# JeremyWesthead/deacon-server

Measured on AMD Instinct MI355X. Metric: Mbp/s filtered (k=31,w=15 vs panhuman-1-sized index), decisions bit-exact vs CPU, higher is better.
Workload: dtype u64

## Files before the change

### deacon-server_amd/_native.py

```python
import ctypes as C
import os
import re
import subprocess

_PKG = os.path.dirname(os.path.abspath(__file__))
LIB_PATH = os.environ.get("DCN_LIB_PATH") or os.path.join(_PKG, "lib", "libdeacon_hip.so")
HEADER_PATH = os.path.join(os.path.dirname(_PKG), "include", "deacon_hip.h")

DCN_OK = 0
DCN_ERR_ARG = -1
DCN_ERR_HIP = -2
DCN_ERR_NOMEM = -3
DCN_ERR_IO = -4
DCN_ERR_FORMAT = -5
DCN_ERR_CAPACITY = -6
DCN_ERR_INTERNAL = -7
N_STATS = 6
N_STAGES = 5
STAGE_NAMES = ("pack", "plan", "scan", "distinct", "finish")
STAT_NAMES = ("total_seqs", "filtered_seqs", "total_bp", "output_bp", "filtered_bp", "output_seq_counter")


class DeaconHipError(RuntimeError):
    def __init__(self, code, message):
# ... 21 lines not shown
        ("prefix_length", C.c_uint64),
    ]


class TrackParams(C.Structure):
    _fields_ = [
        ("bin_bases", C.c_uint32),
        ("member_mask", C.c_uint32),
        ("depth_cap", C.c_uint32),
        ("reserved", C.c_uint32),
        ("prefix_length", C.c_uint64),
    ]


class TrackBin(C.Structure):
    _fields_ = [
        ("n_positions", C.c_uint32),
        ("n_keys", C.c_uint32),
        ("n_observed", C.c_uint32),
        ("max_depth", C.c_uint32),
        ("sum_depth", C.c_uint64),
    ]


class PlaceParams(C.Structure):
    _fields_ = [
        ("band_bases", C.c_uint32),
        ("min_votes", C.c_uint32),
        ("prefix_length", C.c_uint64),
        ("reserved", C.c_uint32 * 2),
    ]


class Placement(C.Structure):
    _fields_ = [
        ("record", C.c_uint32),
        ("reverse", C.c_uint32),
        ("votes", C.c_uint32),
        ("n_anchors", C.c_uint32),
        ("n_positions", C.c_uint32),
        ("read_start", C.c_uint32),
        ("read_end", C.c_uint32),
        ("reserved", C.c_uint32),
        ("ref_start", C.c_uint64),
        ("ref_end", C.c_uint64),
    ]


class PlaceSplitParams(C.Structure):
    _fields_ = [
        ("band_bases", C.c_uint32),
        ("min_votes", C.c_uint32),
        ("prefix_length", C.c_uint64),
        ("max_placements", C.c_uint32),
        ("reserved", C.c_uint32 * 3),
    ]


class SplitPlacement(C.Structure):
    _fields_ = Placement._fields_ + [
        ("rank", C.c_uint32),
        ("n_placed", C.c_uint32),
        ("rival_votes", C.c_uint32),
        ("mapq", C.c_uint32),
    ]


PLACE_SPLIT_MAX = 8


class PlacePairParams(C.Structure):
    _fields_ = [
        ("band_bases", C.c_uint32),
        ("min_votes", C.c_uint32),
        ("prefix_length", C.c_uint64),
        ("max_placements", C.c_uint32),
        ("max_insert", C.c_uint32),
        ("hist_bin_bases", C.c_uint32),
        ("reserved", C.c_uint32 * 3),
    ]


class PairPlacement(C.Structure):
    _fields_ = SplitPlacement._fields_ + [
        ("flags", C.c_uint32),
        ("pair_votes", C.c_uint32),
        ("tlen", C.c_int64),
    ]


PAIR_HIST_BINS = 256


def build(force=False, jobs=6):
    csrc = os.path.join(_PKG, "csrc")
    cmd = ["make", "-C", csrc, f"-j{jobs}"]
    if force:
        cmd.append("-B")
    subprocess.check_call(cmd, stdout=subprocess.DEVNULL)
    return LIB_PATH


def declared_symbols():
    text = open(HEADER_PATH).read()
    text = re.sub(r"/\*.*?\*/", "", text, flags=re.S)
    return sorted(set(re.findall(r"\b(dcn_[a-z0-9_]+)\s*\(", text)))


_u8p, _u32p, _u64p = C.POINTER(C.c_uint8), C.POINTER(C.c_uint32), C.POINTER(C.c_uint64)
_vp = C.c_void_p

_SIGNATURES = {
    "dcn_abi_version": (C.c_int, [_u32p, _u32p]),
    "dcn_version": (C.c_char_p, []),
    "dcn_last_error": (C.c_char_p, []),
    "dcn_device_count": (C.c_int, [C.POINTER(C.c_int)]),
    "dcn_set_minimizer_variant": (C.c_int, [C.c_uint32, C.c_uint32, C.c_uint32]),
    "dcn_get_minimizer_variant": (C.c_int, [_u32p, _u32p, _u32p]),
    "dcn_index_from_keys": (C.c_int, [_vp, C.c_uint64, C.c_uint8, C.c_uint8, C.c_int, C.POINTER(_vp)]),
    "dcn_index_from_file": (C.c_int, [C.c_char_p, C.c_int, C.POINTER(_vp)]),
    "dcn_index_build": (C.c_int, [_vp, _vp, C.c_uint32, C.c_uint8, C.c_uint8, C.c_float, C.c_uint64, C.c_int,
                                  C.POINTER(_vp)]),
    "dcn_index_keys": (C.c_int, [_vp, _vp, C.c_uint64, _u64p]),
    "dcn_index_union": (C.c_int, [C.POINTER(_vp), C.c_uint32, C.POINTER(_vp)]),
    "dcn_index_diff": (C.c_int, [_vp, _vp, C.POINTER(_vp)]),
    "dcn_index_intersect": (C.c_int, [C.POINTER(_vp), C.c_uint32, C.POINTER(_vp)]),
    "dcn_index_write_file": (C.c_int, [_vp, C.c_char_p]),
    "dcn_index_header": (C.c_int, [_vp, _u8p, _u8p, _u64p]),
    "dcn_index_contains": (C.c_int, [_vp, _vp, C.c_uint64, _vp]),
    "dcn_index_contains_device": (C.c_int, [_vp, _vp, C.c_uint64, _vp, _vp]),
    "dcn_index_probe_ceiling": (C.c_int, [_vp, _vp, C.c_uint64, C.c_uint32, C.POINTER(C.c_double)]),
    "dcn_index_destroy": (None, [_vp]),
    "dcn_ctx_create": (C.c_int, [_vp, C.c_uint64, C.c_uint32, C.POINTER(_vp)]),
    "dcn_ctx_destroy": (None, [_vp]),
    "dcn_filter_batch": (C.c_int, [_vp, _vp, _vp, _vp, C.c_uint32, C.POINTER(Params), _vp, _vp, _vp]),
    "dcn_filter_batch_submit": (C.c_int, [_vp, _vp, _vp, _vp, C.c_uint32, C.POINTER(Params), _vp, _vp, _vp, _u64p]),
    "dcn_filter_batch_wait": (C.c_int, [_vp, C.c_uint64]),
    "dcn_filter_batch_packed": (C.c_int, [_vp, _vp, _vp, _vp, _vp, C.c_uint32, C.POINTER(Params), _vp, _vp, _vp]),
    "dcn_filter_batch_packed_submit": (C.c_int, [_vp, _vp, _vp, _vp, _vp, C.c_uint32, C.POINTER(Params), _vp, _vp, _vp,
                                                 _u64p]),
    "dcn_pack_ascii": (C.c_int, [_vp, C.c_uint64, _vp, _vp, _u32p]),
    "dcn_stats_allreduce": (C.c_int, [C.POINTER(_vp), C.c_int, _u64p]),
    "dcn_comm_available": (C.c_int, []),
    "dcn_comm_unique_id": (C.c_int, [_vp]),
    "dcn_comm_create": (C.c_int, [_vp, C.c_int, C.c_int, C.c_int, C.POINTER(_vp)]),
    "dcn_stats_allreduce_rccl": (C.c_int, [_vp, C.POINTER(_vp), C.c_int, _u64p]),
    "dcn_comm_destroy": (None, [_vp]),
    "dcn_index_device": (C.c_int, [_vp, C.POINTER(C.c_int)]),
    "dcn_index_memory": (C.c_int, [_vp, C.POINTER(C.c_uint64)]),
    "dcn_index_clone": (C.c_int, [_vp, C.c_int, C.POINTER(_vp)]),
    "dcn_filter_batch_device": (C.c_int, [_vp, _vp, _vp, _vp, C.c_uint32, C.c_uint64, C.c_uint32,
                                          C.POINTER(Params), _vp, _vp, _vp]),
    "dcn_ctx_synchronize": (C.c_int, [_vp]),
    "dcn_ctx_reserve_records": (C.c_int, [_vp, C.c_uint64]),
    "dcn_ctx_stream": (_vp, [_vp]),
    "dcn_host_alloc": (C.c_int, [C.c_uint64, C.POINTER(_vp)]),
    "dcn_host_free": (None, [_vp]),
    "dcn_minimizer_hashes_batch": (C.c_int, [_vp, _vp, _vp, C.c_uint32, C.c_uint64, _vp, _vp, _vp, C.c_uint64]),
    "dcn_should_keep_hashes": (C.c_int, [_vp, _vp, _vp, C.c_uint32, C.POINTER(Params), _vp, _vp, _vp]),
    "dcn_ctx_stats": (C.c_int, [_vp, _u64p]),
    "dcn_ctx_reset_stats": (C.c_int, [_vp]),
    "dcn_ctx_set_profiling": (C.c_int, [_vp, C.c_int]),
    "dcn_ctx_profile": (C.c_int, [_vp, C.POINTER(C.c_double), _u64p]),
    "dcn_index_set_create": (C.c_int, [C.POINTER(_vp), C.c_uint32, C.POINTER(_vp)]),
    "dcn_index_set_destroy": (None, [_vp]),
    "dcn_index_set_info": (C.c_int, [_vp, _u32p, _u8p, _u8p, _u64p, _u64p]),
    "dcn_classify_batch": (C.c_int, [_vp, _vp, _vp, _vp, _vp, C.c_uint32, C.POINTER(Params), _vp, _vp, _vp]),
    "dcn_classify_batch_device": (C.c_int, [_vp, _vp, _vp, _vp, _vp, C.c_uint32, C.c_uint64, C.c_uint32,
                                            C.POINTER(Params), _vp, _vp, _vp]),
    "dcn_index_set_coverage_enable": (C.c_int, [_vp, C.c_int]),
    "dcn_index_set_coverage_reset": (C.c_int, [_vp]),
    "dcn_index_set_coverage": (C.c_int, [_vp, _vp, _vp]),
    "dcn_index_set_coverage_keys": (C.c_int, [_vp, C.c_uint32, _vp, C.c_uint64, _u64p]),
    "dcn_index_set_depth_enable": (C.c_int, [_vp, C.c_int]),
    "dcn_index_set_depth_reset": (C.c_int, [_vp]),
    "dcn_index_set_depth_stats": (C.c_int, [_vp, _vp, _vp, _vp]),
    "dcn_index_set_depth_hist": (C.c_int, [_vp, C.c_uint32, C.c_uint32, _vp]),
    "dcn_index_set_depth_keys": (C.c_int, [_vp, C.c_uint32, _vp, _vp, C.c_uint64, _u64p]),
    "dcn_index_set_select": (C.c_int, [_vp, C.c_uint32, C.c_uint32, C.c_uint32, C.c_uint32, C.c_uint32, _u64p,
                                       C.POINTER(_vp)]),
    "dcn_index_set_overlap": (C.c_int, [_vp, _vp, _vp, _vp]),
    "dcn_index_builder_create": (C.c_int, [C.c_uint8, C.c_uint8, C.c_float, C.c_uint64, C.c_int, C.POINTER(_vp)]),
    "dcn_index_builder_add": (C.c_int, [_vp, _vp, _vp, C.c_uint32]),
    "dcn_index_builder_info": (C.c_int, [_vp, _u64p, _u64p, _u64p, _u64p]),
    "dcn_index_builder_hist": (C.c_int, [_vp, C.c_uint32, _vp]),
    "dcn_index_builder_counts": (C.c_int, [_vp, _vp, _vp, C.c_uint64, _u64p]),
    "dcn_index_builder_finish": (C.c_int, [_vp, C.c_uint32, C.c_uint32, _u64p, C.POINTER(_vp)]),
    "dcn_index_builder_destroy": (None, [_vp]),
    "dcn_locate_batch": (C.c_int, [_vp, _vp, _vp, _vp, C.c_uint32, _vp, _vp, _vp, C.c_uint64]),
    "dcn_depth_track_batch": (C.c_int, [_vp, _vp, _vp, _vp, C.c_uint32, _vp, _vp, _vp, C.c_uint64]),
    "dcn_anchor_map_create": (C.c_int, [_vp, C.POINTER(_vp)]),
    "dcn_anchor_map_add": (C.c_int, [_vp, _vp, _vp, _vp, C.c_uint32, _u32p]),
    "dcn_anchor_map_info": (C.c_int, [_vp, _u32p, _u64p, _u64p, _u64p]),
    "dcn_anchor_map_anchors": (C.c_int, [_vp, _vp, _vp, _vp, C.c_uint64, _u64p]),
    "dcn_place_batch": (C.c_int, [_vp, _vp, _vp, _vp, C.c_uint32, _vp, _vp]),
    "dcn_place_split_batch": (C.c_int, [_vp, _vp, _vp, _vp, C.c_uint32, _vp, _vp, _vp, C.c_uint64, _vp]),
    "dcn_place_pair_batch": (C.c_int, [_vp, _vp, _vp, _vp, C.c_uint32, _vp, _vp, _vp]),
}

_lib = None
ABI = (1, 11)


def lib():
    global _lib
    if _lib is not None:
        return _lib
    if not os.path.exists(LIB_PATH):
        raise ImportError(
            f"{LIB_PATH} is missing: build it with __graft_entry__.build() "
            "(make -C deacon-server_amd/csrc). There is no CPU fallback.")
    L = C.CDLL(LIB_PATH)
    for name, (res, args) in _SIGNATURES.items():
        f = getattr(L, name)
        f.restype = res
        f.argtypes = args
    major, minor = C.c_uint32(), C.c_uint32()
    if L.dcn_abi_version(C.byref(major), C.byref(minor)) != 0 or (major.value, minor.value >= ABI[1]) != (ABI[0], True):
        raise ImportError(f"{LIB_PATH} has ABI {major.value}.{minor.value}; these bindings were written against {ABI[0]}.{ABI[1]} "
                          "(include/deacon_hip.h: DCN_ABI_MAJOR / DCN_ABI_MINOR)")
    _lib = L
    return L


def check(rc):
    if rc != DCN_OK:
        msg = lib().dcn_last_error()
        raise DeaconHipError(rc, msg.decode("utf-8", "replace") if msg else "")
    return rc
```

### deacon-server_amd/csrc/ctx.hip

```cpp
#include "dcn_ctx.h"
#include "dcn_host_pool.h"

#include <atomic>
#include <cstdlib>
#include <cstring>
#include <mutex>
#include <new>

using dcn_host::HostPool;

uint32_t dcn_cu_count() {
    int dev = 0, cus = 256;
    if (hipGetDevice(&dev) == hipSuccess) (void)hipDeviceGetAttribute(&cus, hipDeviceAttributeMultiprocessorCount, dev);
    return (uint32_t)std::max(cus, 1);
}

namespace dcn_impl {

int alloc_records(dcn_ctx *c, uint64_t n_records) {
    n_records = (n_records + 63) / 64 * 64;
    if (n_records > (1ull << 29)) return dcn_fail(DCN_ERR_CAPACITY, "more than 2^29 hit records in global sets per batch: use smaller batches");
    if (c->d_set_slots) hipFree(c->d_set_slots);
    c->d_set_slots = nullptr;
    c->rec_capacity = 0;
// ... 5 lines not shown
void free_slot_buffers(dcn_slot &sl) {
    if (sl.owns_buffers) {
        void *dev[] = {sl.d_ascii, sl.d_packed, sl.d_invmask, sl.d_offsets, sl.d_unit_id, sl.d_keep, sl.d_hits, sl.d_total};
        for (void *p : dev)
            if (p) hipFree(p);
    }
    if (sl.d_report) hipFree(sl.d_report);
    if (sl.d_off32) hipFree(sl.d_off32);
    if (sl.d_mask_pairs) hipFree(sl.d_mask_pairs);
    void *host[] = {sl.h_keep, sl.h_hits, sl.h_total, sl.h_report, sl.h_off32, sl.h_mask_pairs};
    for (void *p : host)
        if (p) hipHostFree(p);
    if (sl.done) hipEventDestroy(sl.done);
    for (hipEvent_t e : sl.ev_h2d) hipEventDestroy(e);
    for (hipEvent_t e : sl.ev_comp) hipEventDestroy(e);
    sl = dcn_slot();
}

static void free_ctx(dcn_ctx *c) {
    if (!c) return;
    hipSetDevice(c->device);
    if (c->stream) hipStreamSynchronize(c->stream);
    if (c->copy_stream) hipStreamSynchronize(c->copy_stream);
    if (c->d2h_stream) hipStreamSynchronize(c->d2h_stream);
    if (c->pack_stream) {
        hipStreamSynchronize(c->pack_stream);
        hipStreamDestroy(c->pack_stream);
    }
    for (int i = 0; i < 2; ++i) {
        if (c->pack_done[i]) hipEventDestroy(c->pack_done[i]);
        if (c->buf_free[i]) hipEventDestroy(c->buf_free[i]);
    }
    if (c->plan_done) hipEventDestroy(c->plan_done);
    if (c->d_packed_b) hipFree(c->d_packed_b);
    if (c->d_invmask_b) hipFree(c->d_invmask_b);
    if (c->d_pack_status) hipFree(c->d_pack_status);
    for (auto &sl : c->slots) free_slot_buffers(sl);
    void *dev[] = {c->d_ascii, c->d_offsets, c->d_unit_id, c->d_packed, c->d_invmask,
                   c->d_read_tiles, c->d_read_tile_first, c->d_unit_first_read, c->d_unit_tile_first, c->d_unit_tile_count, c->d_tiles,
                   c->d_keep, c->d_unit_state, c->d_hits, c->d_total, c->d_unit_scratch, c->d_caps,
                   c->d_set_off, c->d_tile_hits, c->d_pending, c->d_big, c->d_rec_hash, c->d_set_slots, c->d_status, c->d_report, c->d_dump_hash,
                   c->d_dump_pos, c->d_dump_count, c->d_dump_valid, c->d_tile_read_pos,
                   c->d_cls_big, c->d_cls_n_big, c->d_cls_match, c->d_cls_hits, c->d_cls_total,
                   c->d_loc_bits, c->d_loc_labels, c->d_loc_counts, c->d_loc_big, c->d_loc_n_big, c->d_loc_block_sums,
                   c->d_loc_seg_offsets, c->d_loc_segs, c->d_trk_bin_offsets, c->d_trk_piece_offsets, c->d_trk_bins,
                   c->d_plc_words, c->d_plc_abits, c->d_plc_big, c->d_plc_n_big, c->d_plc_out,
                   c->d_pls_rbits, c->d_pls_n_rounds, c->d_pls_read_counts, c->d_pls_counts, c->d_pls_block_sums,
                   c->d_pls_offsets, c->d_pls_rounds, c->d_pls_out, c->d_ppr_out, c->d_ppr_hist};
    for (void *p : dev)
        if (p && !((char *)p >= c->d_slab && (char *)p < c->d_slab + c->slab_bytes)) hipFree(p);
    if (c->d_slab) hipFree(c->d_slab);
    for (int i = 0; i < dcn_ctx::N_STAGE; ++i) {
        if (c->h_stage[i]) hipHostFree(c->h_stage[i]);
        if (c->stage_free[i]) hipEventDestroy(c->stage_free[i]);
    }
    for (int i = 0; i < dcn_ctx::N_EV; ++i) {
        if (c->ev_h2d[i]) hipEventDestroy(c->ev_h2d[i]);
        if (c->ev_comp[i]) hipEventDestroy(c->ev_comp[i]);
    }
    if (c->h_report) hipHostFree(c->h_report);
    for (int i = 0; i < dcn_ctx::PROF_RING; ++i)
        for (int j = 0; j <= DCN_N_STAGES; ++j)
            if (c->prof_ev[i][j]) hipEventDestroy(c->prof_ev[i][j]);
    if (c->copy_done) hipEventDestroy(c->copy_done);
    if (c->stream) hipStreamDestroy(c->stream);
    if (c->copy_stream) hipStreamDestroy(c->copy_stream);
    if (c->d2h_stream) hipStreamDestroy(c->d2h_stream);
    delete c;
}

static int prof_harvest(dcn_ctx *c, int only_slot = -1) {
    for (int i = 0; i < dcn_ctx::PROF_RING; ++i) {
        if (!c->prof_used[i] || (only_slot >= 0 && i != only_slot)) continue;
        const int first = c->prof_scan_only[i] ? DCN_STAGE_SCAN : 0, last = c->prof_scan_only[i] ? DCN_STAGE_SCAN : DCN_N_STAGES - 1;
        DCN_HIP(hipEventSynchronize(c->prof_ev[i][last + 1]));
        for (int j = first; j <= last; ++j) {
            float ms = 0.f;
            DCN_HIP(hipEventElapsedTime(&ms, c->prof_ev[i][j], c->prof_ev[i][j + 1]));
            c->prof_ms[j] += ms;
        }
        c->prof_batches++;
        c->prof_used[i] = false;
    }
    return DCN_OK;
}

int prof_begin(dcn_ctx *c, int *slot) {
    *slot = -1;
    if (!c->profiling) return DCN_OK;
    int i = c->prof_next;
    c->prof_next = (i + 1) % dcn_ctx::PROF_RING;
    if (c->prof_used[i]) DCN_TRY(prof_harvest(c, i));
    for (int j = 0; j <= DCN_N_STAGES; ++j)
        if (!c->prof_ev[i][j]) DCN_HIP(hipEventCreate(&c->prof_ev[i][j]));
    c->prof_scan_only[i] = c->profiling == 2;
    if (c->profiling == 1) DCN_HIP(hipEventRecord(c->prof_ev[i][0], c->stream));
    *slot = i;
    return DCN_OK;
}

int check_params(const dcn_params *p) {
    if (!p) return dcn_fail(DCN_ERR_ARG, "params is NULL");
    if (p->reserved != 0) return dcn_fail(DCN_ERR_ARG, "params.reserved must be 0");
    if (p->deplete > 1) return dcn_fail(DCN_ERR_ARG, "params.deplete must be 0 or 1");
    return DCN_OK;
}

static bool ensure_pack_ahead(dcn_ctx *c) {
    if (c->pack_ahead_state != 0) return c->pack_ahead_state > 0;
    c->pack_ahead_state = -1;
    if (!getenv("DCN_PACK_AHEAD") || getenv("DCN_NO_PACK_AHEAD")) return false;
    int prio_low = 0, prio_high = 0;
    (void)hipDeviceGetStreamPriorityRange(&prio_low, &prio_high);
    bool ok = hipStreamCreateWithPriority(&c->pack_stream, hipStreamNonBlocking, prio_high) == hipSuccess;
    ok = ok && hipEventCreateWithFlags(&c->plan_done, hipEventDisableTiming) == hipSuccess;
    for (int i = 0; ok && i < 2; ++i)
        ok = hipEventCreateWithFlags(&c->pack_done[i], hipEventDisableTiming) == hipSuccess &&
             hipEventCreateWithFlags(&c->buf_free[i], hipEventDisableTiming) == hipSuccess;
    ok = ok && hipMalloc((void **)&c->d_packed_b, packed_words(c->max_bases) * sizeof(uint32_t)) == hipSuccess &&
         hipMalloc((void **)&c->d_invmask_b, mask_words(c->max_bases) * sizeof(uint32_t)) == hipSuccess &&
         hipMalloc((void **)&c->d_pack_status, 2 * sizeof(dcn_status)) == hipSuccess;
    if (ok) {
        ok = hipMemset(c->d_packed_b, 0, packed_words(c->max_bases) * sizeof(uint32_t)) == hipSuccess &&
             hipMemset(c->d_invmask_b, 0, mask_words(c->max_bases) * sizeof(uint32_t)) == hipSuccess &&
             hipDeviceSynchronize() == hipSuccess;
    }
    if (!ok) {
        (void)hipGetLastError();
        if (c->d_packed_b) hipFree(c->d_packed_b);
        if (c->d_invmask_b) hipFree(c->d_invmask_b);
        if (c->d_pack_status) hipFree(c->d_pack_status);
        c->d_packed_b = c->d_invmask_b = nullptr;
        c->d_pack_status = nullptr;
        return false;
    }
    c->pack_ahead_state = 1;
    return true;
}

static dcn_scan_args scan_args(const dcn_ctx *c, const dcn_index *index, uint32_t *packed, uint32_t *invmask, uint64_t stream_bases);

int enqueue_batch(dcn_ctx *c, const BatchView &v, const dcn_params *params, bool pack_ahead) {
    hipStream_t st = c->stream;
    const dcn_index *idx = c->index;
    if (c->scratch_dirty) DCN_HIP(hipMemsetAsync(c->d_unit_scratch, 0, (uint64_t)c->max_reads * 4 * sizeof(uint32_t), st));
    c->scratch_dirty = true;
    DCN_HIP(hipMemsetAsync(c->d_status, 0, sizeof(dcn_status), st));

    int prof_slot = -1;
    DCN_TRY(prof_begin(c, &prof_slot));
    uint32_t *packed = v.d_packed + DCN_FRONT_PAD, *invmask = v.d_invmask + DCN_FRONT_PAD;
    int ahead_buf = -1;
    const uint32_t *newline_flag = nullptr;
    if (v.d_ascii && pack_ahead && c->profiling != 1 && ensure_pack_ahead(c)) {
        ahead_buf = c->pack_buf;
        c->pack_buf ^= 1;
        if (ahead_buf == 1) {
            packed = c->d_packed_b + DCN_FRONT_PAD;
            invmask = c->d_invmask_b + DCN_FRONT_PAD;
        }
        dcn_status *ps = c->d_pack_status + ahead_buf;
        DCN_HIP(hipStreamWaitEvent(c->pack_stream, c->buf_free[ahead_buf], 0));
        if (!getenv("DCN_PACK_AHEAD_EARLY")) DCN_HIP(hipStreamWaitEvent(c->pack_stream, c->plan_done, 0));
        DCN_HIP(hipMemsetAsync(ps, 0, sizeof(dcn_status), c->pack_stream));
        DCN_TRY(dcn_launch_pack_beside(v.d_ascii, v.b0, v.b1, packed, invmask, ps, c->pack_stream));
        DCN_HIP(hipEventRecord(c->pack_done[ahead_buf], c->pack_stream));
        DCN_HIP(hipStreamWaitEvent(st, c->pack_done[ahead_buf], 0));
        newline_flag = &ps->any_newline;
    } else if (v.d_ascii) {
        DCN_TRY(dcn_launch_pack(v.d_ascii, v.b0, v.b1, packed, invmask, c->d_status, st));
    }
    DCN_PROF_MARK(DCN_STAGE_PACK);

    const uint32_t n_reads = v.n_reads, n_units = v.n_units;
    dcn_plan_args pa = plan_args(c, idx, v.d_ascii, v.d_offsets, v.d_unit_id, n_reads, n_units, params->prefix_length);
    pa.unit_base = v.unit_base;
    pa.unit_state = c->d_unit_state;
    pa.unit_scratch = c->d_unit_scratch;
    pa.scratch_stride = c->max_reads;
    pa.newline_flag = newline_flag;
    pa.stream_bases = v.stream_bases;
    pa.check_offsets = 1;
    pa.max_tiles = c->max_tiles;
    DCN_TRY(dcn_launch_plan(pa, st));
    if (pack_ahead && c->pack_ahead_state == 1) DCN_HIP(hipEventRecord(c->plan_done, st));
    DCN_PROF_MARK(DCN_STAGE_PLAN);

    const UnitScratch us = unit_scratch(c);
    dcn_scan_args sa = scan_args(c, idx, packed, invmask, v.stream_bases);
    sa.unit_tile_first = c->d_unit_tile_first;
    sa.unit_tile_count = c->d_unit_tile_count;
    sa.abs_threshold = params->abs_threshold;
    sa.rel_threshold = params->rel_threshold;
    sa.deplete = params->deplete;
    sa.early_out_max_items = 0;
    static const bool no_early_out = getenv("DCN_NO_EARLY_OUT") != nullptr, no_early_out_pairs = getenv("DCN_NO_EARLY_OUT_PAIRS") != nullptr;
    if (!v.d_hits && !v.d_total && params->abs_threshold >= 1 && params->abs_threshold <= 4 && !no_early_out) {
        uint32_t lo = 0, hi = 65535;
        while (lo < hi) {
            uint32_t mid = (lo + hi + 1) / 2;
            if (dcn_required_hits(params->abs_threshold, params->rel_threshold, mid) == params->abs_threshold) lo = mid;
            else hi = mid - 1;
        }
        sa.early_out_max_items = lo;
        sa.early_out_pairs = no_early_out_pairs ? 0u : 1u;
    }
    sa.keep = v.d_keep;
    sa.hits = v.d_hits;
    sa.total = v.d_total;
    sa.unit_state = c->d_unit_state;
    sa.g_total = us.g_total;
    sa.g_hitcnt = us.g_hitcnt;
    sa.g_zero = us.g_zero;
    sa.rec_hash = c->d_rec_hash;
    sa.rec_shift = c->rec_shift;
    sa.tile_windows = c->tile_windows;
    sa.tile_hits = c->d_tile_hits;
    sa.pending = c->d_pending;
    sa.status = c->d_status;
    DCN_TRY(dcn_launch_scan(sa, tile_bound(c, n_reads, v.b1 - v.b0), false, st));
    DCN_PROF_MARK(DCN_STAGE_SCAN);

    const bool decisions_only = !v.d_hits && !v.d_total && !getenv("DCN_NO_EARLY_OUT");
    const dcn_distinct_args da = distinct_args(c, n_units, params, c->d_rec_hash, c->rec_shift, decisions_only ? us.g_total : nullptr);
    DCN_TRY(dcn_launch_distinct(da, st));
    DCN_PROF_MARK(DCN_STAGE_DISTINCT);

    const dcn_finish_args fa = finish_args(c, n_units, params, v.d_unit_id ? c->d_unit_first_read : nullptr, v.d_offsets, v.d_keep,
                                           v.d_hits, v.d_total, v.d_report);
    DCN_TRY(dcn_launch_finish(fa, st));
    c->scratch_dirty = false;
    if (pack_ahead && c->pack_ahead_state == 1) DCN_HIP(hipEventRecord(c->buf_free[ahead_buf >= 0 ? ahead_buf : 0], st));
    DCN_PROF_MARK(DCN_STAGE_FINISH);
    if (prof_slot >= 0) c->prof_used[prof_slot] = true;
    return DCN_OK;
}

int grow_run_slots(dcn_ctx *c) {
    if (c->rec_shift == 0) return DCN_OK;
    const bool in_slab = c->d_rec_hash && (char *)c->d_rec_hash >= c->d_slab && (char *)c->d_rec_hash < c->d_slab + c->slab_bytes;
    if (c->d_rec_hash && !in_slab) hipFree(c->d_rec_hash);
    c->d_rec_hash = nullptr;
    const uint32_t old_shift = c->rec_shift;
    c->rec_shift = 0;
    int rc = dev_alloc(&c->d_rec_hash, c->max_bases + 128, "rec_hash (one slot per window)");
    if (rc != DCN_OK) {
        c->rec_shift = old_shift;
        int rc2 = dev_alloc(&c->d_rec_hash, (c->max_bases >> old_shift) + 256, "rec_hash");
        return rc2 != DCN_OK ? rc2 : rc;
    }
    static std::atomic<bool> said{false};
    if (!said.exchange(true) && getenv("DCN_QUIET") == nullptr)
        std::fprintf(stderr, "deacon-hip: a unit's hits outgrew its run of the record array; this context now keeps one slot per window "
                             "(%.2f GB instead of %.2f GB of device memory)\n", (c->max_bases + 128) * 8e-9,
                     ((c->max_bases >> old_shift) + 256) * 8e-9);
    return DCN_OK;
}

int overflow_error(const dcn_ctx *c, uint64_t need) {
    return dcn_fail(DCN_ERR_CAPACITY, "hit-record scratch overflow: need " + std::to_string(need) +
                                          " records, have " + std::to_string(c->rec_capacity) +
                                          " (dcn_ctx_reserve_records)");
}

int sync_and_check(dcn_ctx *c, uint64_t *needed_records) {
    DCN_HIP(hipStreamSynchronize(c->stream));
    if (needed_records) *needed_records = 0;
    if (c->profiling) DCN_TRY(prof_harvest(c));
    if (!c->batch_pending) return DCN_OK;
    c->batch_pending = false;
    DCN_HIP(hipMemcpy(c->h_report, c->d_report, sizeof(dcn_batch_report), hipMemcpyDeviceToHost));
    if (c->h_report->bounds) {
        DCN_HIP(hipMemsetAsync(c->d_report, 0, offsetof(dcn_batch_report, stats), c->stream));
        return dcn_fail(DCN_ERR_INTERNAL, "scan kernel: index out of range in phase B (DCN_DEBUG_BOUNDS build)");
    }
    if (c->h_report->bad_offsets) {
        DCN_HIP(hipMemsetAsync(c->d_report, 0, offsetof(dcn_batch_report, stats), c->stream));
        return dcn_fail(DCN_ERR_ARG, "d_offsets of a batch since the last synchronize were not non-decreasing within [0, n_bases] when the "
                                     "device read them (were they written, and ordered before the context's stream, when "
                                     "dcn_filter_batch_device was called?): the outputs and counters of those batches are undefined");
    }
    if (c->h_report->overflow) {
        const uint64_t need = c->h_report->need;
        const bool runs = (c->h_report->overflow & 2u) != 0, sets = (c->h_report->overflow & 1u) != 0;
        DCN_HIP(hipMemsetAsync(c->d_report, 0, offsetof(dcn_batch_report, stats), c->stream));
        if (runs) DCN_TRY(grow_run_slots(c));
        if (needed_records) *needed_records = sets ? need : 0;
        if (!sets)
            return dcn_fail(DCN_ERR_CAPACITY, "a unit had more hits in one wave than its run of the record array holds; the context "
                                              "now keeps one slot per window: enqueue the batches since the last synchronize again");
        return overflow_error(c, need);
    }
    return DCN_OK;
}

bool is_pinned_host(const void *p) {
    if (!p) return false;
    hipPointerAttribute_t attr;
    if (hipPointerGetAttributes(&attr, p) != hipSuccess) {
        (void)hipGetLastError();
        return false;
    }
    return attr.type == hipMemoryTypeHost;
}

template <typename Fill>
static int staged_h2d_fill(dcn_ctx *c, void *d_dst, uint64_t bytes, uint64_t piece_align, Fill fill) {
    uint8_t *dst = (uint8_t *)d_dst;
    const uint64_t piece = c->stage_bytes / piece_align * piece_align;
    for (uint64_t off = 0; off < bytes; off += piece) {
        const int which = c->stage_next;
        c->stage_next = (which + 1) % dcn_ctx::N_STAGE;
        const uint64_t m = std::min<uint64_t>(piece, bytes - off);
        DCN_HIP(hipEventSynchronize(c->stage_free[which]));
        fill(c->h_stage[which], off, m);
        DCN_HIP(hipMemcpyAsync(dst + off, c->h_stage[which], m, hipMemcpyHostToDevice, c->copy_stream));
        DCN_HIP(hipEventRecord(c->stage_free[which], c->copy_stream));
    }
    return DCN_OK;
}

int staged_h2d(dcn_ctx *c, void *d_dst, const void *h_src, uint64_t bytes, int pinned) {
    if (bytes == 0) return DCN_OK;
    if (pinned < 0) pinned = is_pinned_host(h_src) ? 1 : 0;
    if (pinned) {
        DCN_HIP(hipMemcpyAsync(d_dst, h_src, bytes, hipMemcpyHostToDevice, c->copy_stream));
        return DCN_OK;
    }
    const uint8_t *src = (const uint8_t *)h_src;
    return staged_h2d_fill(c, d_dst, bytes, 64, [&](uint8_t *stage, uint64_t first, uint64_t n) {
        HostPool::get().copy(stage, src + first, n);
    });
}


int slots_busy(const dcn_ctx *c) {
    int n = 0;
    for (const auto &sl : c->slots) n += sl.busy ? 1 : 0;
    return n;
}

static std::mutex g_ctx_devices_mu;
static int g_ctx_per_device[64] = {0};
static void note_ctx_device(int device, int delta) {
    int n_devices = 0;
    {
        std::lock_guard<std::mutex> g(g_ctx_devices_mu);
        if (device >= 0 && device < 64) g_ctx_per_device[device] += delta;
        for (int d = 0; d < 64; ++d) n_devices += g_ctx_per_device[d] > 0;
    }
    if (delta > 0) HostPool::get().ensure_devices(n_devices);
}

int check_idle(const dcn_ctx *c) {
    if (slots_busy(c) || c->batch_pending) return dcn_fail(DCN_ERR_ARG, "batches are in flight on this context: wait for them first");
    return DCN_OK;
}

int check_ctx_matches(const dcn_ctx *c, const dcn_index *other, const char *noun) {
    const dcn_index *ix = c->index;
    const std::string n = noun;
    if (ix->k != other->k || ix->w != other->w)
        return dcn_fail(DCN_ERR_ARG, "the context's index (k=" + std::to_string((int)ix->k) + ", w=" + std::to_string((int)ix->w) +
                                         ") and " + n + " (k=" + std::to_string((int)other->k) + ", w=" + std::to_string((int)other->w) +
                                         ") differ");
    if (ix->device != other->device) return dcn_fail(DCN_ERR_ARG, "the context and " + n + " live on different devices");
    if (ix->variant != other->variant)
        return dcn_fail(DCN_ERR_ARG, "the context's index and " + n + " were created under different minimizer rules");
    return check_idle(c);
}

int check_device_batch(const dcn_ctx *c, uint32_t n_reads, uint64_t n_bases, uint32_t n_units, const uint32_t *d_unit_id) {
    if (n_reads > c->max_reads) return dcn_fail(DCN_ERR_CAPACITY, "n_reads exceeds the context's max_batch_reads");
    if (n_bases > c->max_bases) return dcn_fail(DCN_ERR_CAPACITY, "n_bases exceeds the context's max_batch_bases");
    if (n_units == 0 || n_units > n_reads || (!d_unit_id && n_units != n_reads))
        return dcn_fail(DCN_ERR_ARG, "n_units inconsistent with n_reads / d_unit_id");
    return DCN_OK;
}

int check_offsets_walk(const uint64_t *offsets, uint32_t n, const char *noun, const char *too_long) {
    if (offsets[0] != 0) return dcn_fail(DCN_ERR_ARG, std::string(noun) + "[0] must be 0");
    for (uint32_t r = 0; r < n; ++r) {
        if (offsets[r + 1] < offsets[r]) return dcn_fail(DCN_ERR_ARG, std::string(noun) + " must be non-decreasing");
        if (offsets[r + 1] - offsets[r] > 0xFFFFFFF0ull) return dcn_fail(DCN_ERR_ARG, too_long);
    }
    return DCN_OK;
}

int validate_host_batch(const dcn_ctx *c, const uint64_t *offsets, uint32_t n_reads) {
    if (n_reads > c->max_reads) return dcn_fail(DCN_ERR_CAPACITY, "n_reads exceeds the context's max_batch_reads");
    DCN_TRY(check_idle(c));
    DCN_TRY(check_offsets_walk(offsets, n_reads, "offsets", "read longer than 2^32 bases"));
    if (offsets[n_reads] > c->max_bases) return dcn_fail(DCN_ERR_CAPACITY, "batch exceeds the context's max_batch_bases");
    return DCN_OK;
}

int ensure_dump_buffers(dcn_ctx *c) {
    if (c->d_dump_hash) return DCN_OK;
    DCN_TRY(dev_alloc(&c->d_dump_hash, c->max_bases + 2, "dump_hash"));
    DCN_TRY(dev_alloc(&c->d_dump_pos, c->max_bases + 2, "dump_pos"));
    DCN_TRY(dev_alloc(&c->d_dump_valid, c->max_bases + 2, "dump_valid"));
    DCN_TRY(dev_alloc(&c->d_dump_count, c->max_tiles, "dump_count"));
    return DCN_OK;
}

int ensure_position_bitmap(dcn_ctx *c) {
    if (c->d_loc_bits) return DCN_OK;
    return dev_alloc(&c->d_loc_bits, (c->max_bases + 31) / 32 + 1, "position bitmap");
}

int ensure_position_words(dcn_ctx *c) {
    if (c->d_loc_labels) return DCN_OK;
    return dev_alloc(&c->d_loc_labels, c->max_bases + 2, "position words");
}

UnitScratch unit_scratch(const dcn_ctx *c) {
    uint32_t *const s = c->d_unit_scratch;
    const uint64_t n = c->max_reads;
    return {s, s + n, s + 2 * n, s + 3 * n};
}

int stage_done(dcn_ctx *c) {
    DCN_HIP(hipEventRecord(c->copy_done, c->copy_stream));
    DCN_HIP(hipStreamWaitEvent(c->stream, c->copy_done, 0));
// ... 64 lines not shown
    v.n_tiles = &c->d_status->n_tiles;
    v.hash = c->d_dump_hash;
    v.valid = c->d_dump_valid;
    v.pos = c->d_dump_pos;
    v.count = c->d_dump_count;
    v.max_tiles = max_tiles;
    v.n_bases = n_bases;
    return v;
}

int dump_front_end(dcn_ctx *c, const dcn_index *index, const uint8_t *d_ascii, const uint64_t *d_offsets,
                   const uint32_t *d_unit_id, uint32_t n_reads, uint32_t n_units, uint64_t n_bases, uint64_t prefix_length,
                   bool plan_checks_offsets, int *prof_slot_out, dcn_dump_view *view) {
    hipStream_t st = c->stream;
    int prof_slot = -1;
    DCN_TRY(prof_begin(c, &prof_slot));
    *prof_slot_out = prof_slot;
    DCN_TRY(dcn_launch_pack(d_ascii, 0, n_bases, c->d_packed + DCN_FRONT_PAD, c->d_invmask + DCN_FRONT_PAD, c->d_status, st));
    DCN_PROF_MARK(DCN_STAGE_PACK);
    dcn_plan_args pa = plan_args(c, index, d_ascii, d_offsets, d_unit_id, n_reads, n_units, prefix_length);
    pa.read_tiles = c->d_read_tiles;
    pa.read_tile_first = c->d_read_tile_first;
    if (plan_checks_offsets) {
        pa.stream_bases = n_bases;
        pa.check_offsets = 1;
        pa.max_tiles = c->max_tiles;
    }
    DCN_TRY(dcn_launch_plan(pa, st));
    DCN_PROF_MARK(DCN_STAGE_PLAN);
    dcn_scan_args sa = dump_scan_args(c, index, n_bases);
    sa.dump_abs = 1;
    const uint32_t max_tiles = tile_bound(c, n_reads, n_bases);
    DCN_TRY(dcn_launch_scan(sa, max_tiles, true, st));
    DCN_PROF_MARK(DCN_STAGE_SCAN);
    *view = dump_view(c, max_tiles, n_bases);
    return DCN_OK;
}

int record_run_end(dcn_ctx *c, int prof_slot) {
    if (prof_slot >= 0) c->prof_used[prof_slot] = true;
    if (c->pack_ahead_state == 1) {
        DCN_HIP(hipEventRecord(c->plan_done, c->stream));
        for (int i = 0; i < 2; ++i) DCN_HIP(hipEventRecord(c->buf_free[i], c->stream));
    }
    return DCN_OK;
}

int finish_run(dcn_ctx *c, int prof_slot) {
    DCN_TRY(record_run_end(c, prof_slot));
    return sync_and_check(c, nullptr);
}

dcn_distinct_args distinct_args(const dcn_ctx *c, uint32_t n_units, const dcn_params *params, const uint64_t *rec_hash,
                                uint32_t rec_shift, uint32_t *g_total_or_null) {
    const UnitScratch us = unit_scratch(c);
    dcn_distinct_args da = {};
    da.tiles = c->d_tiles;
    da.n_tiles = &c->d_status->n_tiles;
    da.unit_tile_first = c->d_unit_tile_first;
    da.unit_tile_count = c->d_unit_tile_count;
    da.unit_state = c->d_unit_state;
    da.tile_hits = c->d_tile_hits;
    da.pending = c->d_pending;
    da.rec_hash = rec_hash;
    da.rec_shift = rec_shift;
    da.g_hitcnt = us.g_hitcnt;
    da.g_distinct = us.g_distinct;
    da.set_off = c->d_set_off;
    da.set_slots = c->d_set_slots;
    da.set_capacity = 4 * c->rec_capacity + 64;
    da.n_units = n_units;
    da.status = c->d_status;
    da.caps = c->d_caps;
    da.big = c->d_big;
    da.g_total = g_total_or_null;
    da.abs_threshold = params->abs_threshold;
    da.rel_threshold = params->rel_threshold;
    return da;
}

dcn_finish_args finish_args(const dcn_ctx *c, uint32_t n_units, const dcn_params *params, const uint32_t *unit_first_read,
                            const uint64_t *offsets, uint8_t *keep, uint32_t *hits, uint32_t *total, dcn_batch_report *report) {
    const UnitScratch us = unit_scratch(c);
    dcn_finish_args fa = {};
    fa.n_units = n_units;
    fa.unit_first_read = unit_first_read;
    fa.offsets = offsets;
    fa.unit_state = c->d_unit_state;
    fa.g_total = us.g_total;
    fa.g_hitcnt = us.g_hitcnt;
    fa.g_distinct = us.g_distinct;
    fa.g_zero = us.g_zero;
    fa.abs_threshold = params->abs_threshold;
    fa.rel_threshold = params->rel_threshold;
    fa.deplete = params->deplete;
    fa.keep = keep;
    fa.hits = hits;
    fa.total = total;
    fa.report = report;
    fa.status = c->d_status;
    return fa;
}

}

using namespace dcn_impl;

extern "C" int dcn_ctx_create(const dcn_index *index, uint64_t max_batch_bases, uint32_t max_batch_reads,
                              dcn_ctx **out) {
    if (!out) return dcn_fail(DCN_ERR_ARG, "out is NULL");
    *out = nullptr;
    if (!index) return dcn_fail(DCN_ERR_ARG, "index is NULL");
    if (max_batch_bases == 0 || max_batch_reads == 0) return dcn_fail(DCN_ERR_ARG, "batch limits must be > 0");
    if (max_batch_reads > 0xFFFFFF00u) return dcn_fail(DCN_ERR_ARG, "max_batch_reads too large");
    dcn_ctx *c = new (std::nothrow) dcn_ctx();
    if (!c) return dcn_fail(DCN_ERR_NOMEM, "host allocation failed");
    c->index = index;
    c->device = index->device;
    c->max_bases = max_batch_bases;
    c->max_reads = max_batch_reads;
    if (const char *tw = getenv("DCN_TILE_WINDOWS")) {
        long v = strtol(tw, nullptr, 10);
        if (v >= 16 && v <= (long)DCN_MAX_TILE_WINDOWS) c->tile_windows = (uint32_t)v;
    }
    uint64_t mt = (uint64_t)max_batch_reads + max_batch_bases / c->tile_windows + 1;
    if (mt > 0xFFFFFF00ull) {
        delete c;
        return dcn_fail(DCN_ERR_ARG, "batch limits imply more than 2^32 tiles");
    }
    c->max_tiles = (uint32_t)mt;
    c->chunk_bases = 64ull << 20;
    if (const char *cb = getenv("DCN_CHUNK_BASES")) {
        long long v = atoll(cb);
        if (v >= 1024) c->chunk_bases = (uint64_t)v;
    }
    int rc = DCN_OK;
    auto fail = [&](int code) {
        free_ctx(c);
        return code;
    };
    if (hipSetDevice(c->device) != hipSuccess) return fail(dcn_fail(DCN_ERR_HIP, "hipSetDevice failed"));
    bool ok = hipStreamCreateWithFlags(&c->stream, hipStreamNonBlocking) == hipSuccess &&
              hipStreamCreateWithFlags(&c->copy_stream, hipStreamNonBlocking) == hipSuccess &&
              hipStreamCreateWithFlags(&c->d2h_stream, hipStreamNonBlocking) == hipSuccess &&
              hipEventCreateWithFlags(&c->copy_done, hipEventDisableTiming) == hipSuccess;
    for (int i = 0; ok && i < dcn_ctx::N_STAGE; ++i)
        ok = hipEventCreateWithFlags(&c->stage_free[i], hipEventDisableTiming) == hipSuccess;
    for (int i = 0; ok && i < dcn_ctx::N_EV; ++i)
        ok = hipEventCreateWithFlags(&c->ev_h2d[i], hipEventDisableTiming) == hipSuccess &&
             hipEventCreateWithFlags(&c->ev_comp[i], hipEventDisableTiming) == hipSuccess;
    if (!ok) return fail(dcn_fail(DCN_ERR_HIP, "stream/event creation failed"));
    c->rec_shift = 2;
    if (index->w <= 7) c->rec_shift = 0;
    if (const char *rs = getenv("DCN_REC_SHIFT")) c->rec_shift = (uint32_t)std::min(3, std::max(0, atoi(rs)));
    uint64_t MR = max_batch_reads;
    const bool slab = getenv("DCN_CTX_SLAB") != nullptr;
    uint64_t slab_off = 0;
    for (int pass = slab ? 0 : 1; pass < 2; ++pass) {
        if (slab && pass == 1) {
            c->slab_bytes = slab_off;
            if (hipMalloc((void **)&c->d_slab, c->slab_bytes) != hipSuccess) {
                c->d_slab = nullptr;
                c->slab_bytes = 0;
                return fail(dcn_fail(DCN_ERR_NOMEM, "hipMalloc of the context slab failed"));
            }
            slab_off = 0;
        }
#define A(ptr, count, what)                                                                                   \
    if (slab) {                                                                                               \
        if (pass == 1) c->ptr = reinterpret_cast<decltype(c->ptr)>(c->d_slab + slab_off);                     \
        slab_off += (std::max<uint64_t>((count), 1) * sizeof(*c->ptr) + (2u << 20) - 1) / (2u << 20) * (2u << 20); \
    } else if ((rc = dev_alloc(&c->ptr, (count), what)) != DCN_OK)                                            \
        return fail(rc)
    A(d_ascii, max_batch_bases + 64, "ascii");
    A(d_offsets, MR + 1, "offsets");
    A(d_unit_id, MR, "unit_id");
    A(d_packed, packed_words(max_batch_bases), "packed");
    A(d_invmask, mask_words(max_batch_bases), "invmask");
    A(d_read_tiles, MR, "read_tiles");
    A(d_read_tile_first, MR + 1, "read_tile_first");
    A(d_unit_first_read, MR + 1, "unit_first_read");
    A(d_unit_tile_first, MR + 1, "unit_tile_first");
    A(d_unit_tile_count, MR + 1, "unit_tile_count");
    A(d_tiles, mt, "tiles");
    A(d_keep, MR, "keep");
    A(d_unit_state, MR, "unit_state");
    A(d_hits, MR, "hits");
    A(d_total, MR, "total");
    A(d_unit_scratch, MR * 4, "unit_scratch");
    A(d_caps, MR, "caps");
    A(d_set_off, MR + 1, "set_off");
    A(d_tile_hits, mt, "tile_hits");
    A(d_pending, MR, "pending");
    A(d_big, MR + mt / 64 + 1, "big");
    A(d_rec_hash, (max_batch_bases >> c->rec_shift) + 256, "rec_hash");
    A(d_status, 1, "status");
    A(d_report, 1, "report");
#undef A
    }
    uint64_t recs = std::min<uint64_t>(std::max<uint64_t>(max_batch_bases / 16, 1u << 16), 1ull << 29);
    if (const char *rc_env = getenv("DCN_RECORD_CAPACITY")) recs = std::min<uint64_t>(std::max<uint64_t>(strtoull(rc_env, nullptr, 10), 64), 1ull << 29);
    if ((rc = alloc_records(c, recs)) != DCN_OK) return fail(rc);
    c->stage_bytes = std::min<uint64_t>(std::max<uint64_t>(max_batch_bases + 64, 4096), 32ull << 20);
    if (const char *sb = getenv("DCN_STAGE_BYTES"))
        c->stage_bytes = std::min<uint64_t>(std::max<uint64_t>(strtoull(sb, nullptr, 10), 4096), 32ull << 20);
    for (int i = 0; i < dcn_ctx::N_STAGE; ++i)
        if (hipHostMalloc((void **)&c->h_stage[i], c->stage_bytes, hipHostMallocDefault) != hipSuccess)
            return fail(dcn_fail(DCN_ERR_NOMEM, "pinned staging allocation failed"));
    if (hipHostMalloc((void **)&c->h_report, sizeof(dcn_batch_report), hipHostMallocDefault) != hipSuccess)
        return fail(dcn_fail(DCN_ERR_NOMEM, "pinned status allocation failed"));
    if (hipMemset(c->d_packed, 0, packed_words(max_batch_bases) * sizeof(uint32_t)) != hipSuccess ||
        hipMemset(c->d_invmask, 0, mask_words(max_batch_bases) * sizeof(uint32_t)) != hipSuccess ||
        hipMemset(c->d_status, 0, sizeof(dcn_status)) != hipSuccess ||
        hipMemset(c->d_unit_scratch, 0, (uint64_t)max_batch_reads * 4 * sizeof(uint32_t)) != hipSuccess ||
        hipMemset(c->d_report, 0, sizeof(dcn_batch_report)) != hipSuccess ||
        hipDeviceSynchronize() != hipSuccess)
        return fail(dcn_fail(DCN_ERR_HIP, "hipMemset failed"));
    note_ctx_device(c->device, +1);
    *out = c;
    return DCN_OK;
}

extern "C" void dcn_ctx_destroy(dcn_ctx *ctx) {
    if (ctx) note_ctx_device(ctx->device, -1);
    free_ctx(ctx);
}

extern "C" void *dcn_ctx_stream(dcn_ctx *ctx) { return ctx ? (void *)ctx->stream : nullptr; }

extern "C" int dcn_ctx_reserve_records(dcn_ctx *ctx, uint64_t n_records) {
    if (!ctx) return dcn_fail(DCN_ERR_ARG, "ctx is NULL");
    if (slots_busy(ctx)) return dcn_fail(DCN_ERR_ARG, "host batches are in flight: wait for them first");
    DCN_HIP(hipSetDevice(ctx->device));
    DCN_HIP(hipStreamSynchronize(ctx->stream));
    if (n_records <= ctx->rec_capacity) return DCN_OK;
    return alloc_records(ctx, n_records);
}

extern "C" int dcn_ctx_synchronize(dcn_ctx *ctx) {
    if (!ctx) return dcn_fail(DCN_ERR_ARG, "ctx is NULL");
    DCN_HIP(hipSetDevice(ctx->device));
    return sync_and_check(ctx, nullptr);
}

extern "C" int dcn_filter_batch_device(dcn_ctx *ctx, const uint8_t *d_bases, const uint64_t *d_offsets,
                                       const uint32_t *d_unit_id, uint32_t n_reads, uint64_t n_bases,
                                       uint32_t n_units, const dcn_params *params, uint8_t *d_keep, uint32_t *d_hits,
                                       uint32_t *d_total) {
    if (!ctx) return dcn_fail(DCN_ERR_ARG, "ctx is NULL");
    DCN_TRY(check_params(params));
    if (n_reads == 0) return DCN_OK;
    if (!d_bases || !d_offsets || !d_keep) return dcn_fail(DCN_ERR_ARG, "d_bases/d_offsets/d_keep is NULL");
    DCN_TRY(check_device_batch(ctx, n_reads, n_bases, n_units, d_unit_id));
    if (ctx->slots[0].busy) return dcn_fail(DCN_ERR_ARG, "a host batch is in flight on this context: wait for it first");
    DCN_HIP(hipSetDevice(ctx->device));
    BatchView v;
    v.d_ascii = d_bases;
    v.d_packed = ctx->d_packed;
    v.d_invmask = ctx->d_invmask;
    v.d_offsets = d_offsets;
    v.d_unit_id = d_unit_id;
    v.n_reads = n_reads;
    v.n_units = n_units;
    v.b0 = 0;
    v.b1 = n_bases;
    v.stream_bases = n_bases;
    v.d_keep = d_keep;
    v.d_hits = d_hits;
    v.d_total = d_total;
    v.d_report = ctx->d_report;
    DCN_TRY(enqueue_batch(ctx, v, params, true));
    ctx->batch_pending = true;
    return DCN_OK;
}

extern "C" int dcn_ctx_set_profiling(dcn_ctx *ctx, int enable) {
    if (!ctx) return dcn_fail(DCN_ERR_ARG, "ctx is NULL");
    DCN_HIP(hipSetDevice(ctx->device));
    DCN_HIP(hipStreamSynchronize(ctx->stream));
    for (int i = 0; i < dcn_ctx::PROF_RING; ++i) ctx->prof_used[i] = false;
    for (int j = 0; j < DCN_N_STAGES; ++j) ctx->prof_ms[j] = 0.0;
    ctx->prof_batches = 0;
    ctx->profiling = enable == 2 ? 2 : (enable != 0 ? 1 : 0);
    return DCN_OK;
}

extern "C" int dcn_ctx_profile(dcn_ctx *ctx, double stage_ms[DCN_N_STAGES], uint64_t *n_batches) {
    if (!ctx || !stage_ms) return dcn_fail(DCN_ERR_ARG, "ctx/stage_ms is NULL");
    if (ctx->profiling) {
        DCN_HIP(hipSetDevice(ctx->device));
        DCN_TRY(prof_harvest(ctx));
    }
    for (int j = 0; j < DCN_N_STAGES; ++j) stage_ms[j] = ctx->prof_ms[j];
    if (n_batches) *n_batches = ctx->prof_batches;
    return DCN_OK;
}

extern "C" int dcn_ctx_stats(dcn_ctx *ctx, uint64_t counters[DCN_N_STATS]) {
    if (!ctx || !counters) return dcn_fail(DCN_ERR_ARG, "ctx/counters is NULL");
    DCN_HIP(hipSetDevice(ctx->device));
    DCN_HIP(hipStreamSynchronize(ctx->stream));
    DCN_HIP(hipMemcpy(ctx->h_report, ctx->d_report, sizeof(dcn_batch_report), hipMemcpyDeviceToHost));
    for (int i = 0; i < DCN_N_STATS; ++i) counters[i] = ctx->h_report->stats[i] + ctx->host_stats[i];
    return DCN_OK;
}

extern "C" int dcn_ctx_reset_stats(dcn_ctx *ctx) {
    if (!ctx) return dcn_fail(DCN_ERR_ARG, "ctx is NULL");
    DCN_HIP(hipSetDevice(ctx->device));
    DCN_HIP(hipStreamSynchronize(ctx->stream));
    DCN_HIP(hipMemsetAsync(ctx->d_report->stats, 0, sizeof(unsigned long long) * DCN_N_STATS, ctx->stream));
    DCN_HIP(hipStreamSynchronize(ctx->stream));
    for (int i = 0; i < DCN_N_STATS; ++i) ctx->host_stats[i] = 0;
    return DCN_OK;
}

extern "C" int dcn_stats_allreduce(dcn_ctx *const *ctxs, int n_ctx, uint64_t counters[DCN_N_STATS]) {
    if (!counters || (n_ctx > 0 && !ctxs) || n_ctx < 0) return dcn_fail(DCN_ERR_ARG, "ctxs/counters is NULL");
    for (int i = 0; i < DCN_N_STATS; ++i) counters[i] = 0;
    for (int j = 0; j < n_ctx; ++j) {
        uint64_t one[DCN_N_STATS];
        DCN_TRY(dcn_ctx_stats(ctxs[j], one));
        for (int i = 0; i < DCN_N_STATS; ++i) counters[i] += one[i];
    }
    return DCN_OK;
}
```

### deacon-server_amd/csrc/dcn_ctx.h

```cpp
#pragma once

#include "dcn_dump_sweep.h"
#include "dcn_internal.h"
#include "dcn_plan.h"

#include <algorithm>
#include <functional>
#include <vector>

struct dcn_split_round;

struct dcn_mask_range {
    uint64_t g0 = 0, g1 = 0, pairs_off = 0;
    uint32_t n = 0;
};

struct dcn_chunk {
    uint32_t r0 = 0, r1 = 0, u0 = 0, u1 = 0;
    uint64_t b0 = 0, b1 = 0;
    uint64_t max_len = 0;
    std::vector<dcn_mask_range> mask_ranges;
};

struct dcn_slot {
    bool allocated = false, busy = false, owns_buffers = false;
    uint64_t ticket = 0;
    uint8_t *d_ascii = nullptr;
    uint32_t *d_packed = nullptr, *d_invmask = nullptr;
    uint64_t *d_offsets = nullptr;
    uint32_t *d_off32 = nullptr, *h_off32 = nullptr;
    bool off32 = false;
    bool lean = false;
    uint2 *d_mask_pairs = nullptr, *h_mask_pairs = nullptr;
    uint64_t mask_pairs_cap = 0, mask_pairs_used = 0;
    uint32_t *d_unit_id = nullptr;
    uint8_t *d_keep = nullptr;
    uint32_t *d_hits = nullptr, *d_total = nullptr;
    dcn_batch_report *d_report = nullptr;
    uint8_t *h_keep = nullptr;
    uint32_t *h_hits = nullptr, *h_total = nullptr;
    dcn_batch_report *h_report = nullptr;
    hipEvent_t done = nullptr;
    std::vector<hipEvent_t> ev_h2d, ev_comp;
    dcn_params params = {};
    bool device_pack = false;
    bool has_units = false, counts = false;
    uint32_t n_reads = 0, n_units = 0;
    uint64_t n_bases = 0;
    uint8_t *u_keep = nullptr;
    uint32_t *u_hits = nullptr, *u_total = nullptr;
    bool keep_direct = false, hits_direct = false, total_direct = false;
    std::vector<dcn_chunk> chunks;
};

struct dcn_ctx {
    const dcn_index *index = nullptr;
    int device = 0;
    hipStream_t stream = nullptr, copy_stream = nullptr, d2h_stream = nullptr;
    hipStream_t pack_stream = nullptr;
    uint32_t *d_packed_b = nullptr, *d_invmask_b = nullptr;
    dcn_status *d_pack_status = nullptr;
    hipEvent_t pack_done[2] = {}, buf_free[2] = {}, plan_done = nullptr;
    int pack_buf = 0, pack_ahead_state = 0;
    static constexpr int N_STAGE = 3, N_EV = 8, N_SLOTS = 2;
    hipEvent_t copy_done = nullptr, stage_free[N_STAGE] = {};
    hipEvent_t ev_h2d[N_EV] = {}, ev_comp[N_EV] = {};
    int ev_next = 0, stage_next = 0;
    uint64_t max_bases = 0;
    uint32_t max_reads = 0;
    uint32_t tile_windows = 256;
    uint32_t max_tiles = 0;
    uint64_t chunk_bases = 0;
    uint8_t *d_ascii = nullptr;
    uint64_t *d_offsets = nullptr;
    uint32_t *d_unit_id = nullptr;
    uint32_t *d_packed = nullptr, *d_invmask = nullptr;
    uint32_t *d_read_tiles = nullptr, *d_read_tile_first = nullptr;
    uint32_t *d_unit_first_read = nullptr, *d_unit_tile_first = nullptr, *d_unit_tile_count = nullptr;
    dcn_tile *d_tiles = nullptr;
    uint8_t *d_keep = nullptr, *d_unit_state = nullptr;
    uint32_t *d_hits = nullptr, *d_total = nullptr;
    uint32_t *d_unit_scratch = nullptr;
    bool scratch_dirty = false;
    uint32_t *d_caps = nullptr, *d_set_off = nullptr;
    uint64_t *d_rec_hash = nullptr;
    uint32_t rec_shift = 0;
    char *d_slab = nullptr;
    uint64_t slab_bytes = 0;
    uint32_t *d_tile_hits = nullptr, *d_pending = nullptr;
    uint2 *d_big = nullptr;
    uint64_t rec_capacity = 0;
    uint64_t *d_set_slots = nullptr;
    dcn_status *d_status = nullptr;
    dcn_batch_report *d_report = nullptr;
    dcn_batch_report *h_report = nullptr;
    uint64_t host_stats[DCN_N_STATS] = {};
    uint8_t *h_stage[N_STAGE] = {};
    uint64_t stage_bytes = 0;
    dcn_slot slots[N_SLOTS];
    uint64_t next_ticket = 1;
    uint64_t *d_dump_hash = nullptr;
    uint32_t *d_dump_pos = nullptr, *d_dump_count = nullptr, *d_tile_read_pos = nullptr;
    uint8_t *d_dump_valid = nullptr;
    uint32_t *d_cls_big = nullptr, *d_cls_n_big = nullptr;
    uint32_t *d_cls_match = nullptr, *d_cls_hits = nullptr, *d_cls_total = nullptr;
    uint32_t cls_hits_members = 0;
    uint32_t *d_loc_bits = nullptr, *d_loc_labels = nullptr;
    uint32_t *d_loc_counts = nullptr, *d_loc_big = nullptr, *d_loc_n_big = nullptr;
    unsigned long long *d_loc_block_sums = nullptr;
    uint64_t *d_loc_seg_offsets = nullptr;
    dcn_segment *d_loc_segs = nullptr;
    uint64_t loc_seg_cap = 0;
    uint64_t *d_trk_bin_offsets = nullptr, *d_trk_piece_offsets = nullptr;
    dcn_track_bin *d_trk_bins = nullptr;
    uint64_t trk_bin_cap = 0;
    uint64_t *d_plc_words = nullptr;
    uint32_t *d_plc_abits = nullptr, *d_plc_big = nullptr, *d_plc_n_big = nullptr;
    dcn_placement *d_plc_out = nullptr;
    uint32_t *d_pls_rbits = nullptr, *d_pls_n_rounds = nullptr, *d_pls_read_counts = nullptr, *d_pls_counts = nullptr;
    unsigned long long *d_pls_block_sums = nullptr;
    uint64_t *d_pls_offsets = nullptr;
    dcn_split_round *d_pls_rounds = nullptr;
    dcn_split_placement *d_pls_out = nullptr;
    uint64_t pls_round_cap = 0, pls_out_cap = 0;
    dcn_pair_placement *d_ppr_out = nullptr;
    unsigned long long *d_ppr_hist = nullptr;
    bool batch_pending = false;
    bool lean = false;
    static constexpr int PROF_RING = 64;
    int profiling = 0;
    hipEvent_t prof_ev[PROF_RING][DCN_N_STAGES + 1] = {};
    bool prof_used[PROF_RING] = {}, prof_scan_only[PROF_RING] = {};
    int prof_next = 0;
    double prof_ms[DCN_N_STAGES] = {};
    uint64_t prof_batches = 0;
};

bool dcn_host_pack_is_wide();
bool dcn_host_pack_groups(const uint8_t *ascii, uint64_t n_bases, uint64_t g0, uint64_t g1, uint32_t *packed,
                          uint32_t *mask);

#define DCN_TRY(expr)              \
    do {                           \
        int _rc = (expr);          \
        if (_rc != DCN_OK) return _rc; \
    } while (0)

#define DCN_PROF_MARK(stage)                                                                                      \
    do {                                                                                                          \
        if (prof_slot >= 0 && (c->profiling == 1 || (stage) == DCN_STAGE_PLAN || (stage) == DCN_STAGE_SCAN))      \
            DCN_HIP(hipEventRecord(c->prof_ev[prof_slot][(stage) + 1], st));                                      \
    } while (0)

#pragma GCC visibility push(hidden)
namespace dcn_impl {

template <typename T>
int dev_alloc(T **p, uint64_t count, const char *what) {
    hipError_t e = hipMalloc((void **)p, std::max<uint64_t>(count, 1) * sizeof(T));
    if (e != hipSuccess) {
        *p = nullptr;
        return dcn_fail(DCN_ERR_NOMEM, std::string("hipMalloc ") + what + ": " + hipGetErrorString(e));
    }
    return DCN_OK;
}

template <typename T>
int dev_alloc_zeroed(T **p, uint64_t count, const char *what) {
    *p = nullptr;
    T *d = nullptr;
    hipError_t e = hipMalloc((void **)&d, count * sizeof(T));
    if (e == hipSuccess) e = hipMemset(d, 0, count * sizeof(T));
    if (e == hipSuccess) e = hipDeviceSynchronize();
    if (e != hipSuccess) {
        if (d) hipFree(d);
        return dcn_hip_fail(e, what);
    }
    *p = d;
    return DCN_OK;
}

struct DevMem {
    void *p = nullptr;
    ~DevMem() {
        if (p) hipFree(p);
    }
    int alloc(uint64_t bytes, bool zero, const char *what) {
        hipError_t e = hipMalloc(&p, std::max<uint64_t>(bytes, 8));
        if (e == hipSuccess && zero) e = hipMemset(p, 0, std::max<uint64_t>(bytes, 8));
        return e == hipSuccess ? DCN_OK : dcn_hip_fail(e, what);
    }
    int clear(const char *what) {
        const hipError_t e = hipMemset(p, 0, 8);
        return e == hipSuccess ? DCN_OK : dcn_hip_fail(e, what);
    }
    int read(void *h, uint64_t bytes, const char *what) const {
        const hipError_t e = hipMemcpy(h, p, bytes, hipMemcpyDeviceToHost);
        return e == hipSuccess ? DCN_OK : dcn_hip_fail(e, what);
    }
    template <typename T>
    T *as() const {
        return (T *)p;
    }
};

inline int read_count(const DevMem &d_n, const char *what, unsigned long long *n) { return d_n.read(n, sizeof(*n), what); }

inline uint64_t packed_words(uint64_t max_bases) { return DCN_FRONT_PAD + 2 * ((max_bases + 31) / 32) + DCN_TAIL_PAD; }
inline uint64_t mask_words(uint64_t max_bases) { return DCN_FRONT_PAD + (max_bases + 31) / 32 + DCN_TAIL_PAD; }

struct BatchView {
    const uint8_t *d_ascii = nullptr;
    uint32_t *d_packed = nullptr, *d_invmask = nullptr;
    const uint64_t *d_offsets = nullptr;
    const uint32_t *d_unit_id = nullptr;
    uint32_t unit_base = 0;
    uint32_t n_reads = 0, n_units = 0;
    uint64_t b0 = 0, b1 = 0;
    uint64_t stream_bases = 0;
    uint8_t *d_keep = nullptr;
    uint32_t *d_hits = nullptr, *d_total = nullptr;
    dcn_batch_report *d_report = nullptr;
};

int same_params(const dcn_index *a, const dcn_index *b);
int check_kw(uint8_t k, uint8_t w);

constexpr uint32_t DCN_BUILD_MAX_PIECES = 1u << 16;
uint64_t build_chunk_bases();
using build_sweep_fn = std::function<int(uint64_t nb, bool continues)>;
struct build_times {
    double front_end_s = 0, staging_s = 0, growth_s = 0, finish_s = 0, finish_table_s = 0;
};
double build_now();
int build_timing_begin(dcn_ctx *c);
int build_times_print(const char *which, dcn_ctx *c, const build_times &t);
int build_run_chunks(dcn_ctx *c, const dcn_index *idx, const uint8_t *bases, const uint64_t *offsets, uint32_t n_seqs,
                     uint64_t chunk_bases, const build_sweep_fn &sweep, build_times *times = nullptr);

int check_set(const dcn_index *set);

int alloc_records(dcn_ctx *c, uint64_t n_records);
void free_slot_buffers(dcn_slot &sl);
int prof_begin(dcn_ctx *c, int *slot);
int check_params(const dcn_params *p);
int enqueue_batch(dcn_ctx *c, const BatchView &v, const dcn_params *params, bool pack_ahead = false);
// ... 42 lines not shown
```

### deacon-server_amd/csrc/dcn_internal.h

```cpp
#pragma once

#include <hip/hip_runtime.h>
#include <stdint.h>

#include <string>

#include "../../include/deacon_hip.h"

void dcn_set_error(const std::string &msg);
int dcn_fail(int code, const std::string &msg);

#define DCN_HIP(expr)                                                                              \
    do {                                                                                           \
        hipError_t _e = (expr);                                                                    \
        if (_e != hipSuccess)                                                                      \
            return dcn_fail(_e == hipErrorOutOfMemory ? DCN_ERR_NOMEM : DCN_ERR_HIP,               \
                            std::string(#expr) + ": " + hipGetErrorString(_e));                    \
    } while (0)

inline int dcn_hip_fail(hipError_t e, const char *what) {
    return dcn_fail(e == hipErrorOutOfMemory ? DCN_ERR_NOMEM : DCN_ERR_HIP, std::string(what) + ": " + hipGetErrorString(e));
}

template <typename F>
int dcn_device_tally(uint64_t count, unsigned long long *h, const char *what, F sweep) {
    unsigned long long *d = nullptr;
    hipError_t e = hipMalloc((void **)&d, count * sizeof(unsigned long long));
    if (e != hipSuccess) return dcn_hip_fail(e, what);
    int rc = DCN_OK;
    e = hipMemset(d, 0, count * sizeof(unsigned long long));
    if (e == hipSuccess) rc = sweep(d);
    if (e == hipSuccess && rc == DCN_OK) e = hipMemcpy(h, d, count * sizeof(unsigned long long), hipMemcpyDeviceToHost);
    hipFree(d);
    if (rc != DCN_OK) return rc;
    return e == hipSuccess ? DCN_OK : dcn_hip_fail(e, what);
}

uint32_t dcn_cu_count();

void dcn_host_parallel_copy(void *dst, const void *src, size_t n);

#ifndef DCN_GROUP_SLOTS
#define DCN_GROUP_SLOTS 2
#endif
constexpr int DCN_SLOTS_PER_KEY = DCN_GROUP_SLOTS == 2 ? 4 : 2;
constexpr int DCN_SLOTS_PER_KEY_ROOMY = 2 * DCN_SLOTS_PER_KEY;
constexpr uint64_t DCN_ROOMY_MAX_GROUPS = 1ull << 31;

struct dcn_table_view {
    const uint64_t *slots;
    uint32_t group_shift;
    uint32_t group_mask;
    uint32_t has_zero;
};

constexpr uint32_t DCN_VARIANT_DEFAULT = (1u << 16) | (16u << 8) | 0u;
uint32_t dcn_current_variant();

struct dcn_index {
    uint32_t variant = dcn_current_variant();
    int device = 0;
    uint8_t k = 0, w = 0;
    uint64_t n_keys = 0;
    uint64_t n_groups = 0;
    uint64_t *d_slots = nullptr;
    bool has_zero = false;
    uint32_t *d_labels = nullptr;
    uint32_t n_members = 0;
    uint32_t zero_label = 0;
    uint32_t *d_cov = nullptr;
    uint64_t cov_words = 0;
    uint64_t cov_keys[32] = {};
    uint32_t *d_depth = nullptr;
    uint64_t depth_words = 0;
    uint64_t *d_anchor = nullptr;
    uint32_t anchor_records = 0;
    dcn_table_view view() const {
        dcn_table_view v;
        v.slots = d_slots;
        uint32_t bits = 0;
        while ((1ull << bits) < n_groups) ++bits;
        v.group_shift = 32 - bits;
        v.group_mask = (uint32_t)(n_groups - 1);
        v.has_zero = has_zero ? 1u : 0u;
        return v;
    }
};

__host__ __device__ inline uint32_t dcn_group_of(uint64_t key, uint32_t group_shift, uint32_t group_mask) {
    uint32_t lo = (uint32_t)key, hi = (uint32_t)(key >> 32);
    uint32_t x = (lo ^ ((hi << 15) | (hi >> 17))) * 0x9E3779B1u;
    return group_shift >= 32 ? 0u : ((x >> group_shift) & group_mask);
}

constexpr int DCN_WAVE = 64;
constexpr int DCN_LCAP = 40;
constexpr uint32_t DCN_FRONT_PAD = 64;
constexpr uint32_t DCN_TAIL_PAD = 256;
constexpr uint32_t DCN_MAX_TILE_WINDOWS = 2048;

struct dcn_tile {
    uint64_t scan_start;
    uint32_t unit;
    uint32_t nwf;
    __host__ __device__ uint32_t n_windows() const { return nwf & 0x3FFFFFFFu; }
    __host__ __device__ uint32_t carry() const { return nwf >> 31; }
    __host__ __device__ bool whole_unit() const { return (nwf >> 30) & 1u; }
};
static_assert(sizeof(dcn_tile) == 16, "tile descriptor");

struct dcn_status {
    uint32_t rec_overflow;
    uint32_t n_tiles;
    uint32_t any_records;
    uint32_t n_big;
    uint32_t any_scattered;
    uint32_t n_pending;
    uint32_t any_newline;
    uint32_t bounds;
    uint32_t run_overflow;
    uint32_t bad_offsets;
    unsigned long long set_cursor;
};

struct dcn_batch_report {
    uint32_t overflow;
    uint32_t bounds;
    uint32_t bad_offsets;
    uint32_t reserved_;
    unsigned long long need;
    unsigned long long stats[DCN_N_STATS];
};

struct dcn_scan_args {
    const uint32_t *packed;
    const uint32_t *invmask;
    const dcn_tile *tiles;
    const uint32_t *tile_read_pos;
    const uint32_t *n_tiles;
    uint32_t *unit_tile_first;
    uint32_t *unit_tile_count;
    dcn_table_view table;
    uint32_t k, w;
    uint64_t stream_bases;
    uint64_t abs_threshold;
    double rel_threshold;
    uint32_t deplete;
    uint32_t early_out_max_items;
    uint32_t early_out_pairs;
    uint8_t *keep;
    uint32_t *hits, *total;
    uint8_t *unit_state;
    uint32_t *g_total;
    uint32_t *g_hitcnt;
    uint32_t *g_zero;
    uint64_t *rec_hash;
    uint32_t rec_shift;
    uint32_t tile_windows;
    uint32_t *tile_hits;
    uint32_t *pending;
    dcn_status *status;
    uint64_t *dump_hash;
    uint32_t *dump_pos;
    uint8_t *dump_valid;
    uint32_t *dump_count;
    uint32_t dump_abs;
    uint32_t variant;
    uint32_t nt_rot;
    uint32_t cmp_mask;
    uint32_t nt_combine_xor;
};

int dcn_launch_pack(const uint8_t *d_ascii, uint64_t base_begin, uint64_t base_end, uint32_t *d_packed,
                    uint32_t *d_invmask, dcn_status *status, hipStream_t stream, bool index_side = false,
                    uint32_t block_threads = 256);
int dcn_launch_pack_beside(const uint8_t *d_ascii, uint64_t base_begin, uint64_t base_end, uint32_t *d_packed, uint32_t *d_invmask,
                           dcn_status *status, hipStream_t stream);
int dcn_launch_scan(const dcn_scan_args &args, uint32_t max_tiles, bool dump, hipStream_t stream);

int dcn_table_build(dcn_index *idx, const uint64_t *host_keys, uint64_t n);
int dcn_table_contains(const dcn_index *idx, const uint64_t *host_keys, uint64_t n, uint8_t *out);
int dcn_table_contains_device(const dcn_index *idx, const uint64_t *d_keys, uint64_t n, uint8_t *d_out,
                              hipStream_t stream);
int dcn_table_probe_ceiling(const dcn_index *idx, const uint64_t *d_keys, uint64_t n, uint32_t reps, double *best,
                            hipStream_t stream);
int dcn_table_insert_varint9(dcn_index *idx, const uint64_t *d_raw, uint64_t n, unsigned long long *d_new,
                             uint32_t *d_zero, uint32_t *d_bad, hipStream_t stream);
uint64_t dcn_table_groups_for(uint64_t n_keys);
int dcn_table_alloc(dcn_index *idx, uint64_t n_keys_capacity);
int dcn_table_reserve(dcn_index *idx, uint64_t n_keys_capacity);
int dcn_table_insert_dump(dcn_index *idx, const uint64_t *d_hash, const uint8_t *d_valid, const uint32_t *d_abs_pos,
                          uint64_t n_slots, const uint8_t *d_ascii, float entropy_threshold, hipStream_t stream);
int dcn_table_count_valid(const uint8_t *d_valid, uint64_t n, uint64_t *count, hipStream_t stream);
int dcn_table_export(const dcn_index *idx, uint64_t *host_out, uint64_t capacity, uint64_t *n_out);
int dcn_table_merge(dcn_index *dst, const dcn_index *src, const dcn_index *minus);
hipError_t dcn_table_malloc(uint64_t **p, uint64_t bytes);
int dcn_table_clone_by_keys(const dcn_index *src, dcn_index *dst);


__host__ __device__ inline uint64_t dcn_required_hits(uint64_t abs_threshold, double rel_threshold,
                                                      uint64_t total) {
    uint64_t rel_required = 0;
    if (total != 0) {
        double r = round(rel_threshold * (double)total);
        if (!(r > 0.0)) rel_required = 0;
        else if (r >= 18446744073709551616.0) rel_required = ~0ull;
        else rel_required = (uint64_t)r;
        if (rel_required < 1) rel_required = 1;
    }
    return abs_threshold > rel_required ? abs_threshold : rel_required;
}

__host__ __device__ inline bool dcn_decide(uint64_t hits, uint64_t total, uint64_t abs_threshold,
                                           double rel_threshold, uint32_t deplete) {
    uint64_t required = dcn_required_hits(abs_threshold, rel_threshold, total);
    return deplete ? (hits < required) : (hits >= required);
}
```

### deacon-server_amd/csrc/pack.hip

```cpp
#include "dcn_internal.h"

#include <algorithm>

namespace {

__device__ inline uint32_t pack4(uint32_t x) {
    uint32_t y = (x >> 1) & 0x03030303u;
    return (y * ((1u << 24) | (1u << 18) | (1u << 12) | (1u << 6))) >> 24;
}

__device__ inline uint32_t pack4_index_side(uint32_t x) {
    uint32_t out = 0;
#pragma unroll
    for (int j = 0; j < 4; ++j) {
        uint32_t c = ((x >> (8 * j)) & 0xFFu) | 0x20u;
        bool is_a = (c == 'a') | (c == 'w');
        bool is_t = (c == 't');
        bool is_g = (c == 'g') | (c == 'r') | (c == 's') | (c == 'k') | (c == 'd') | (c == 'v');
        uint32_t code = is_a ? 0u : is_t ? 2u : is_g ? 3u : 1u;
        out |= code << (2 * j);
    }
    return out;
}

__device__ inline uint32_t invalid4(uint32_t x) {
    const uint32_t y = x | 0x20202020u;
    const uint32_t T = (y >> 2) & ~(y >> 1) & 0x01010101u;
    const uint32_t expect = 0x60606060u | (T << 4) | (T ^ 0x01010101u);
    const uint32_t diff = (y & 0xF9F9F9F9u) ^ expect;
    const uint32_t nz = ((diff & 0x7F7F7F7Fu) + 0x7F7F7F7Fu) | diff;
    return (((nz >> 7) & 0x01010101u) * 0x01020408u) >> 24;
}

template <bool ALIGNED, bool INDEX_SIDE>
__global__ __launch_bounds__(256) void pack_kernel(const uint8_t *__restrict__ ascii, uint64_t n_bases,
                                                   uint32_t *__restrict__ packed,
                                                   uint32_t *__restrict__ invmask, uint64_t g_first, uint64_t n_chunks,
                                                   dcn_status *status) {
    uint64_t stride = (uint64_t)gridDim.x * blockDim.x;
    uint32_t nl = 0;
    for (uint64_t t = g_first + (uint64_t)blockIdx.x * blockDim.x + threadIdx.x; t < g_first + n_chunks; t += stride) {
        uint64_t base = t * 32;
        uint32_t w[8];
        if (ALIGNED && base + 32 <= n_bases) {
            const uint4 *p = reinterpret_cast<const uint4 *>(ascii + base);
            uint4 a = p[0], b = p[1];
            w[0] = a.x; w[1] = a.y; w[2] = a.z; w[3] = a.w;
            w[4] = b.x; w[5] = b.y; w[6] = b.z; w[7] = b.w;
        } else {
#pragma unroll
            for (int q = 0; q < 8; ++q) {
                uint32_t v = 0;
#pragma unroll
                for (int j = 0; j < 4; ++j) {
                    uint64_t i = base + 4 * q + j;
                    uint32_t c = i < n_bases ? ascii[i] : (uint32_t)'A';
                    v |= c << (8 * j);
                }
                w[q] = v;
            }
        }
        uint32_t p0 = 0, p1 = 0, m = 0;
#pragma unroll
        for (int q = 0; q < 4; ++q) {
            p0 |= (INDEX_SIDE ? pack4_index_side(w[q]) : pack4(w[q])) << (8 * q);
            p1 |= (INDEX_SIDE ? pack4_index_side(w[q + 4]) : pack4(w[q + 4])) << (8 * q);
        }
#pragma unroll
        for (int q = 0; q < 8; ++q) m |= invalid4(w[q]) << (4 * q);
        if (!INDEX_SIDE && m) {
#pragma unroll
            for (int q = 0; q < 8; ++q) {
                uint32_t z = w[q] ^ 0x0A0A0A0Au;
                nl |= (z - 0x01010101u) & ~z & 0x80808080u;
            }
        }
        packed[2 * t] = p0;
        packed[2 * t + 1] = p1;
        invmask[t] = m;
    }
    if (!INDEX_SIDE && nl && status) status->any_newline = 1;
}


__global__ __launch_bounds__(64) __attribute__((amdgpu_num_vgpr(32))) void pack16_kernel(
    const uint8_t *__restrict__ ascii, uint32_t *__restrict__ packed, uint32_t *__restrict__ invmask, uint32_t h_first,
    uint32_t h_end, dcn_status *status) {
    const uint32_t stride = gridDim.x * 64u;
    uint32_t nl = 0;
    uint16_t *mask16 = reinterpret_cast<uint16_t *>(invmask);
    for (uint32_t t = h_first + blockIdx.x * 64u + threadIdx.x; t < h_end; t += stride) {
        const uint4 a = *reinterpret_cast<const uint4 *>(ascii + (uint64_t)t * 16);
        const uint32_t p = pack4(a.x) | (pack4(a.y) << 8) | (pack4(a.z) << 16) | (pack4(a.w) << 24);
        const uint32_t m = invalid4(a.x) | (invalid4(a.y) << 4) | (invalid4(a.z) << 8) | (invalid4(a.w) << 12);
        if (m) {
            uint32_t z = a.x ^ 0x0A0A0A0Au;
            nl |= (z - 0x01010101u) & ~z & 0x80808080u;
            z = a.y ^ 0x0A0A0A0Au;
            nl |= (z - 0x01010101u) & ~z & 0x80808080u;
            z = a.z ^ 0x0A0A0A0Au;
            nl |= (z - 0x01010101u) & ~z & 0x80808080u;
            z = a.w ^ 0x0A0A0A0Au;
            nl |= (z - 0x01010101u) & ~z & 0x80808080u;
        }
        packed[t] = p;
        mask16[t] = (uint16_t)m;
    }
    if (nl && status) status->any_newline = 1;
}

}

int dcn_launch_pack_beside(const uint8_t *d_ascii, uint64_t base_begin, uint64_t base_end, uint32_t *d_packed, uint32_t *d_invmask,
                           dcn_status *status, hipStream_t stream) {
    if (base_end <= base_begin) return DCN_OK;
    const uint64_t whole_end = base_end / 32 * 32;
    if ((reinterpret_cast<uintptr_t>(d_ascii) & 15) != 0 || (base_begin & 31) != 0 || whole_end / 16 > 0xFFFFFFFFull || whole_end <= base_begin)
        return dcn_launch_pack(d_ascii, base_begin, base_end, d_packed, d_invmask, status, stream, false, 64);
    const uint32_t h_first = (uint32_t)(base_begin / 16), h_end = (uint32_t)(whole_end / 16);
    const uint32_t blocks = (uint32_t)std::min<uint64_t>(((uint64_t)(h_end - h_first) + 63) / 64, 256ull * 4 * 16);
    hipLaunchKernelGGL(pack16_kernel, dim3(blocks), dim3(64), 0, stream, d_ascii, d_packed, d_invmask, h_first, h_end, status);
    DCN_HIP(hipGetLastError());
    if (whole_end < base_end) return dcn_launch_pack(d_ascii, whole_end, base_end, d_packed, d_invmask, status, stream, false, 64);
    return DCN_OK;
}

int dcn_launch_pack(const uint8_t *d_ascii, uint64_t base_begin, uint64_t base_end, uint32_t *d_packed,
                    uint32_t *d_invmask, dcn_status *status, hipStream_t stream, bool index_side, uint32_t block_threads) {
    if (base_end <= base_begin) return DCN_OK;
    const uint64_t g_first = base_begin / 32, n_bases = base_end;
    uint64_t n_chunks = (base_end + 31) / 32 - g_first;
    const uint32_t bt = block_threads == 64 ? 64u : 256u;
    uint32_t blocks = (uint32_t)((n_chunks + bt - 1) / bt);
    if (blocks > 256 * 32 * (256 / bt)) blocks = 256 * 32 * (256 / bt);
    bool aligned = (reinterpret_cast<uintptr_t>(d_ascii) & 15) == 0;
#define DCN_PACK(AL, IX) \
    hipLaunchKernelGGL((pack_kernel<AL, IX>), dim3(blocks), dim3(bt), 0, stream, d_ascii, n_bases, d_packed, d_invmask, g_first, n_chunks, status)
    if (index_side) {
        if (aligned) DCN_PACK(true, true);
        else DCN_PACK(false, true);
    } else {
        if (aligned) DCN_PACK(true, false);
        else DCN_PACK(false, false);
    }
#undef DCN_PACK
    DCN_HIP(hipGetLastError());
    return DCN_OK;
}
```

### deacon-server_amd/csrc/plan.hip

```cpp
#include "dcn_internal.h"
#include "dcn_plan.h"
#include "dcn_probe.h"

#include <algorithm>

namespace {

__device__ inline uint32_t effective_windows(const uint8_t *ascii, uint64_t off, uint64_t len, uint64_t prefix,
                                             uint32_t k, uint32_t l) {
    if (len < k) return 0;
    uint64_t n = (prefix > 0 && len > prefix) ? prefix : len;
    if (ascii && n > 0 && ascii[off + n - 1] == '\n') n -= 1;
    return n >= l ? (uint32_t)(n - l + 1) : 0;
}

__device__ inline void write_tile(const dcn_plan_args &a, uint32_t first, uint32_t j, uint64_t off, uint32_t nwin,
                                  uint32_t unit, bool whole_unit = false) {
    uint32_t wstart = j * a.tile_windows;
    uint32_t carry = j > 0 ? 1u : 0u;
    if (a.check_offsets && first + j >= a.max_tiles) {
        a.status->bad_offsets = 1;
        return;
    }
    dcn_tile t;
    t.scan_start = off + wstart - carry;
    t.unit = unit;
    t.nwf = min(a.tile_windows, nwin - wstart) | (carry << 31) | (whole_unit ? 1u << 30 : 0u);
    a.tiles[first + j] = t;
    if (a.tile_read_pos) a.tile_read_pos[first + j] = wstart - carry;
}

template <uint32_t PLAN_CH>
__global__ __launch_bounds__(256) void plan_kernel(dcn_plan_args a) {
    constexpr uint32_t PLAN_READS = 256 * PLAN_CH;
    constexpr uint32_t OWN = 4;
    __shared__ uint32_t s_tiles[PLAN_READS];
    __shared__ uint32_t s_first[PLAN_READS];
    __shared__ uint32_t s_wave[4], s_wave1[4];
    __shared__ uint32_t s_base;
    __shared__ uint32_t long_reads[PLAN_READS];
    __shared__ uint32_t n_long;
    const uint32_t tid = threadIdx.x;
    const uint32_t block_first = blockIdx.x * PLAN_READS;
    const uint32_t block_end = min(a.n_reads, block_first + PLAN_READS);
    if (tid == 0) n_long = 0;
    const uint8_t *ascii = (a.ascii && (a.newline_flag ? *a.newline_flag : a.status->any_newline)) ? a.ascii : nullptr;
    uint32_t nwin[PLAN_CH], nt[PLAN_CH], loc[PLAN_CH];
    const bool two_classes = a.unit_id == nullptr;
    uint32_t carry = 0;
    uint32_t carry1 = 0;
#pragma unroll
    for (uint32_t c = 0; c < PLAN_CH; ++c) {
        const uint32_t r = block_first + c * 256 + tid;
        nwin[c] = 0;
        nt[c] = 0;
        if (r < a.n_reads) {
            uint64_t off = a.offsets[r], end = a.offsets[r + 1];
            if (a.check_offsets && (end < off || end > a.stream_bases)) {
                a.status->bad_offsets = 1;
                end = off = 0;
            }
            nwin[c] = effective_windows(ascii, off, end - off, a.prefix_length, a.k, a.k + a.w - 1);
            nt[c] = (nwin[c] + a.tile_windows - 1) / a.tile_windows;
        }
        const bool single = two_classes && nt[c] == 1;
        const uint32_t own = single ? 0u : nt[c], own1 = single ? 1u : 0u;
        uint32_t inc = own, inc1 = own1;
#pragma unroll
        for (int d = 1; d < 64; d <<= 1) {
            uint32_t o = __shfl_up(inc, d, 64), o1 = __shfl_up(inc1, d, 64);
            if ((int)(tid & 63) >= d) {
                inc += o;
                inc1 += o1;
            }
        }
        __syncthreads();
        if ((tid & 63) == 63) {
            s_wave[tid >> 6] = inc;
            s_wave1[tid >> 6] = inc1;
        }
        __syncthreads();
        uint32_t wave_base = 0, chunk_total = 0, wave_base1 = 0, chunk_total1 = 0;
#pragma unroll
        for (uint32_t i = 0; i < 4; ++i) {
            if (i < (tid >> 6)) {
                wave_base += s_wave[i];
                wave_base1 += s_wave1[i];
            }
            chunk_total += s_wave[i];
            chunk_total1 += s_wave1[i];
        }
        loc[c] = single ? (0x80000000u | (carry1 + wave_base1 + inc1 - 1u)) : (carry + wave_base + inc - own);
        carry += chunk_total;
        carry1 += chunk_total1;
        s_tiles[c * 256 + tid] = nt[c];
    }
    if (tid == 0) s_base = (carry + carry1) ? atomicAdd(a.tile_cursor, carry + carry1) : 0u;
    __syncthreads();
#pragma unroll
    for (uint32_t c = 0; c < PLAN_CH; ++c) {
        if (loc[c] & 0x80000000u) loc[c] = carry + (loc[c] & 0x7FFFFFFFu);
        s_first[c * 256 + tid] = s_base + loc[c];
    }
    __syncthreads();
#pragma unroll
    for (uint32_t c = 0; c < PLAN_CH; ++c) {
        const uint32_t r = block_first + c * 256 + tid;
        if (r >= a.n_reads) continue;
        const uint32_t first = s_base + loc[c];
        if (a.read_tiles) {
            a.read_tiles[r] = nt[c];
            a.read_tile_first[r] = first;
        }
        uint32_t u = r;
        bool unit_head = true;
        if (a.unit_id) {
            u = a.unit_id[r] - a.unit_base;
            if (a.check_offsets) {
                const uint32_t prev = r ? a.unit_id[r - 1] : a.unit_base - 1u;
                if (u >= a.n_units || a.unit_id[r] - prev > 1u || (r == a.n_reads - 1 && u != a.n_units - 1)) {
                    a.status->bad_offsets = 1;
                    if (u >= a.n_units) u = 0;
                }
            }
            unit_head = r == 0 || a.unit_id[r - 1] != a.unit_id[r];
            if (unit_head) a.unit_first_read[u] = r;
            if (r == a.n_reads - 1) a.unit_first_read[a.n_units] = a.n_reads;
        }
        if (unit_head) {
            uint32_t count = nt[c];
            if (a.unit_id) {
                uint32_t q = r + 1;
                while (q < a.n_reads && a.unit_id[q] - a.unit_base == u) {
                    if (q >= block_end) {
                        count = 0xFFFFFFFFu;
                        break;
                    }
                    count += s_tiles[q - block_first];
                    ++q;
                }
            }
            if (a.unit_id || nt[c] != 1) {
                a.unit_tile_first[u] = first;
                a.unit_tile_count[u] = count;
            }
            if (a.unit_state) a.unit_state[u] = 0;
        }
        const uint64_t off = a.offsets[r];
        for (uint32_t j = 0; j < min(nt[c], OWN); ++j) write_tile(a, first, j, off, nwin[c], u, !a.unit_id && nt[c] == 1);
        if (nt[c] > OWN) long_reads[atomicAdd(&n_long, 1u)] = c * 256 + tid;
    }
    __syncthreads();
    for (uint32_t q = 0; q < n_long; ++q) {
        const uint32_t li = long_reads[q], lr = block_first + li;
        const uint32_t lnt = s_tiles[li], lfirst = s_first[li];
        uint32_t lu = a.unit_id ? a.unit_id[lr] - a.unit_base : lr;
        if (a.check_offsets && lu >= a.n_units) lu = 0;
        const uint64_t loff = a.offsets[lr];
        const uint32_t lnwin = effective_windows(ascii, loff, a.offsets[lr + 1] - loff, a.prefix_length, a.k, a.k + a.w - 1);
        for (uint32_t j = OWN + tid; j < lnt; j += blockDim.x) write_tile(a, lfirst, j, loff, lnwin, lu);
    }
}

#ifndef DCN_LDS_SET_LOG2
#define DCN_LDS_SET_LOG2 11
#endif
constexpr uint32_t DCN_LDS_SET_SLOTS = 1u << DCN_LDS_SET_LOG2;
constexpr uint32_t DCN_LDS_SET_MAX = DCN_LDS_SET_SLOTS * 7 / 10 - 33;
constexpr uint32_t DCN_LDS_WALK_MAX_TILES = 1024;

__device__ inline uint32_t set_slot_of(uint64_t h, uint32_t cap) {
    uint32_t lo = (uint32_t)h, hi = (uint32_t)(h >> 32);
    return ((lo ^ ((hi << 13) | (hi >> 19))) * 0x85EBCA6Bu) & (cap - 1);
}

__global__ __launch_bounds__(64) void unit_distinct_kernel(dcn_distinct_args a) {
    __shared__ unsigned long long set[DCN_LDS_SET_SLOTS];
    if (a.status->run_overflow) return;
    const uint32_t NP = a.status->n_pending;
    const uint32_t lane = threadIdx.x;
    uint32_t nu = 0, nfirst = 0, ncount = 0, nH = 0, ntot = 0;
    auto fetch = [&](uint32_t i) {
        if (i < NP) {
            nu = a.pending[i];
            nfirst = a.unit_tile_first[nu];
            ncount = a.unit_tile_count[nu];
            nH = a.g_hitcnt[nu];
            ntot = a.g_total ? a.g_total[nu] : 0u;
        }
    };
    fetch(blockIdx.x);
    for (uint32_t i = blockIdx.x; i < NP; i += gridDim.x) {
        const uint32_t u = nu, first = nfirst, count = ncount, H = nH, tot = ntot;
        fetch(i + gridDim.x);
        if (H == 0) {
            if (lane == 0) a.caps[u] = 0;
            continue;
        }
        uint32_t enough = 0xFFFFFFFFu;
        if (a.g_total) {
            const uint64_t req = dcn_required_hits(a.abs_threshold, a.rel_threshold, tot);
            if ((uint64_t)H < req) {
                if (lane == 0) {
                    a.g_distinct[u] = 0;
                    a.caps[u] = 0;
                }
                continue;
            }
            enough = req > 0xFFFFFFFEull ? 0xFFFFFFFEu : (uint32_t)req;
        }
        const uint32_t Hset = H < enough ? H : enough;
        if (count == 0xFFFFFFFFu || Hset > DCN_LDS_SET_MAX || count > DCN_LDS_WALK_MAX_TILES) {
            uint32_t cap = 64;
            while (cap < 2u * H && cap < (1u << 31)) cap <<= 1;
            unsigned long long off = 0;
            if (lane == 0) off = atomicAdd(&a.status->set_cursor, (unsigned long long)cap);
            off = (unsigned long long)__shfl((long long)off, 0, 64);
            const bool fits = off + cap <= a.set_capacity;
            const uint32_t n_items = count == 0xFFFFFFFFu ? 0u : (count + 63) / 64;
            uint32_t item0 = 0;
            if (lane == 0) {
                a.set_off[u] = (uint32_t)off;
                a.caps[u] = fits ? cap : 0u;
                if (!fits) a.status->rec_overflow = 1;
                else if (n_items) item0 = atomicAdd(&a.status->n_big, n_items);
                if (fits && count == 0xFFFFFFFFu) a.status->any_scattered = 1;
            }
            item0 = __shfl(item0, 0, 64);
            if (fits)
                for (uint32_t q = lane; q < n_items; q += 64) a.big[item0 + q] = make_uint2(u, 64 * q);
            continue;
        }
        const uint32_t most = enough == 0xFFFFFFFFu ? Hset : (Hset + 256u < H ? Hset + 256u : H);
        uint32_t cap = 64;
        while (cap < 2u * most && cap < DCN_LDS_SET_SLOTS) cap <<= 1;
        auto tile_run = [&](uint32_t t, uint32_t &n, uint64_t &slot0) {
            n = 0;
            slot0 = 0;
            if (t < count) {
                n = a.tile_hits[first + t];
                const dcn_tile tl = a.tiles[first + t];
                slot0 = (tl.scan_start + tl.carry()) >> a.rec_shift;
            }
        };
        uint32_t n;
        uint64_t slot0;
        tile_run(lane, n, slot0);
        for (uint32_t q = lane; q < cap; q += 64) set[q] = 0;
        __syncthreads();
        uint32_t distinct = 0;
        for (uint32_t t0 = 0; t0 < count && distinct < enough; t0 += 64) {
            if (t0) tile_run(t0 + lane, n, slot0);
            unsigned long long runs = __ballot(n != 0);
            while (runs && distinct < enough) {
                const int r = __ffsll((long long)runs) - 1;
                runs &= runs - 1;
                const uint32_t rn = __shfl(n, r, 64);
                const uint64_t rs = (uint64_t)__shfl((long long)slot0, r, 64);
                for (uint32_t j0 = 0; j0 < rn && distinct < enough; j0 += 256) {
                    uint64_t h[4];
#pragma unroll
                    for (int q = 0; q < 4; ++q) {
                        const uint32_t j = j0 + q * 64 + lane;
                        h[q] = j < rn ? a.rec_hash[rs + j] : 0ull;
                    }
#pragma unroll
                    for (int q = 0; q < 4; ++q) {
                        bool fresh = false;
                        if (h[q] != 0) {
                            uint32_t sl = set_slot_of(h[q], cap);
                            for (;;) {
                                unsigned long long old = atomicCAS(&set[sl], 0ull, (unsigned long long)h[q]);
                                if (old == 0) {
                                    fresh = true;
                                    break;
                                }
                                if (old == h[q]) break;
                                sl = (sl + 1) & (cap - 1);
                            }
                        }
                        distinct += (uint32_t)__popcll(__ballot(fresh));
                    }
                }
            }
        }
        __syncthreads();
        if (lane == 0) {
            a.g_distinct[u] = distinct;
            a.caps[u] = 0;
        }
    }
}

__device__ inline uint32_t insert_run(const uint64_t *rec_hash, uint64_t slot0, uint32_t n, unsigned long long *region,
                                      uint32_t cap, uint32_t lane) {
    uint32_t fresh_n = 0;
    for (uint32_t j0 = 0; j0 < n; j0 += 256) {
        uint64_t h[4];
        uint32_t sl[4];
        unsigned long long old[4];
#pragma unroll
        for (int q = 0; q < 4; ++q) {
            const uint32_t j = j0 + q * 64 + lane;
            h[q] = j < n ? rec_hash[slot0 + j] : 0ull;
        }
#pragma unroll
        for (int q = 0; q < 4; ++q) {
            sl[q] = set_slot_of(h[q], cap);
            old[q] = h[q] ? atomicCAS(&region[sl[q]], 0ull, (unsigned long long)h[q]) : h[q];
        }
#pragma unroll
        for (int q = 0; q < 4; ++q) {
            bool fresh = false;
            if (h[q] != 0) {
                unsigned long long o = old[q];
                for (;;) {
                    if (o == 0) {
                        fresh = true;
                        break;
                    }
                    if (o == h[q]) break;
                    sl[q] = (sl[q] + 1) & (cap - 1);
                    o = atomicCAS(&region[sl[q]], 0ull, (unsigned long long)h[q]);
                }
            }
            fresh_n += (uint32_t)__popcll(__ballot(fresh));
        }
    }
    return fresh_n;
}

__global__ __launch_bounds__(256) void distinct_clear_kernel(uint64_t *set_slots, uint64_t capacity, const dcn_status *status) {
    if (status->set_cursor == 0 || status->rec_overflow || status->run_overflow) return;
    uint64_t total = status->set_cursor;
    if (total > capacity) total = capacity;
    uint64_t stride = (uint64_t)gridDim.x * blockDim.x;
    for (uint64_t i = (uint64_t)blockIdx.x * blockDim.x + threadIdx.x; i < total; i += stride) set_slots[i] = 0;
}

__global__ __launch_bounds__(256) void big_insert_kernel(dcn_distinct_args a) {
    if (a.status->set_cursor == 0 || a.status->rec_overflow || a.status->run_overflow) return;
    const uint32_t NB = a.status->n_big;
    const uint32_t lane = threadIdx.x & 63;
    const uint32_t gwave = (blockIdx.x * blockDim.x + threadIdx.x) >> 6, n_waves = (gridDim.x * blockDim.x) >> 6;
    for (uint32_t bi = gwave; bi < NB; bi += n_waves) {
        const uint2 item = a.big[bi];
        const uint32_t u = item.x;
        const uint32_t first = a.unit_tile_first[u], count = a.unit_tile_count[u];
        const uint32_t cap = a.caps[u];
        unsigned long long *region = (unsigned long long *)(a.set_slots + a.set_off[u]);
        const uint32_t t = item.y + lane;
        uint32_t n = 0;
        uint64_t slot0 = 0;
        if (t < count) {
            n = a.tile_hits[first + t];
            const dcn_tile tl = a.tiles[first + t];
            slot0 = (tl.scan_start + tl.carry()) >> a.rec_shift;
        }
        uint32_t fresh_n = 0;
        unsigned long long runs = __ballot(n != 0);
        while (runs) {
            const int r = __ffsll((long long)runs) - 1;
            runs &= runs - 1;
            fresh_n += insert_run(a.rec_hash, (uint64_t)__shfl((long long)slot0, r, 64), __shfl(n, r, 64), region, cap, lane);
        }
        if (lane == 0 && fresh_n) atomicAdd(&a.g_distinct[u], fresh_n);
    }
    if (a.status->any_scattered == 0) return;
    const uint32_t NT = *a.n_tiles;
    for (uint32_t t = gwave; t < NT; t += n_waves) {
        const dcn_tile tl = a.tiles[t];
        if (a.unit_state[tl.unit] || a.unit_tile_count[tl.unit] != 0xFFFFFFFFu) continue;
        const uint32_t cap = a.caps[tl.unit];
        const uint32_t n = a.tile_hits[t];
        if (!cap || !n) continue;
        const uint32_t fresh_n = insert_run(a.rec_hash, (tl.scan_start + tl.carry()) >> a.rec_shift, n,
                                            (unsigned long long *)(a.set_slots + a.set_off[tl.unit]), cap, lane);
        if (lane == 0 && fresh_n) atomicAdd(&a.g_distinct[tl.unit], fresh_n);
    }
}

__global__ __launch_bounds__(256) void finish_kernel(dcn_finish_args a) {
    unsigned long long st[DCN_N_STATS] = {0, 0, 0, 0, 0, 0};
    const uint32_t stride = gridDim.x * blockDim.x;
    for (uint32_t u0 = blockIdx.x * blockDim.x + threadIdx.x; u0 < a.n_units; u0 += 4 * stride) {
        uint8_t state[4], kept[4];
        uint32_t r0[4], r1[4];
        uint64_t o0[4], o1[4];
#pragma unroll
        for (int q = 0; q < 4; ++q) {
            const uint32_t u = u0 + q * stride;
            state[q] = 2;
            if (u < a.n_units) {
                state[q] = a.unit_state[u];
                kept[q] = a.keep[u];
                r0[q] = a.unit_first_read ? a.unit_first_read[u] : u;
                r1[q] = a.unit_first_read ? a.unit_first_read[u + 1] : u + 1;
            }
        }
#pragma unroll
        for (int q = 0; q < 4; ++q) {
            o0[q] = o1[q] = 0;
            if (state[q] != 2 && a.offsets && !a.status->bad_offsets) {
                o0[q] = a.offsets[r0[q]];
                o1[q] = a.offsets[r1[q]];
            }
        }
#pragma unroll
        for (int q = 0; q < 4; ++q) {
            if (state[q] == 2) continue;
            const uint32_t u = u0 + q * stride;
            bool keep;
            if (state[q]) {
                keep = kept[q] != 0;
            } else {
                uint32_t tot = a.g_total[u], hc = a.g_distinct[u] + (a.g_zero[u] ? 1u : 0u);
                a.g_total[u] = 0;
                a.g_hitcnt[u] = 0;
                a.g_distinct[u] = 0;
                a.g_zero[u] = 0;
                keep = dcn_decide(hc, tot, a.abs_threshold, a.rel_threshold, a.deplete);
                a.keep[u] = keep ? 1 : 0;
                if (a.hits) a.hits[u] = hc;
                if (a.total) a.total[u] = tot;
            }
            if (a.offsets) {
                unsigned long long nseq = r1[q] - r0[q], bp = o1[q] - o0[q];
                st[DCN_STAT_TOTAL_SEQS] += nseq;
                st[DCN_STAT_TOTAL_BP] += bp;
                if (keep) {
                    st[DCN_STAT_OUTPUT_BP] += bp;
                    st[DCN_STAT_OUTPUT_SEQ_COUNTER] += nseq;
                } else {
                    st[DCN_STAT_FILTERED_SEQS] += nseq;
                    st[DCN_STAT_FILTERED_BP] += bp;
                }
            }
        }
    }
    if (a.status->bounds && blockIdx.x == 0 && threadIdx.x == 0) a.report->bounds = a.status->bounds;
    if (a.status->bad_offsets) {
        if (blockIdx.x == 0 && threadIdx.x == 0) a.report->bad_offsets = 1;
        return;
    }
    if (a.status->rec_overflow || a.status->run_overflow) {
        if (blockIdx.x == 0 && threadIdx.x == 0) {
            atomicOr(&a.report->overflow, (a.status->rec_overflow ? 1u : 0u) | (a.status->run_overflow ? 2u : 0u));
            if (a.status->rec_overflow) atomicMax(&a.report->need, (a.status->set_cursor + 3) / 4);
        }
        return;
    }
    if (!a.offsets) return;
    __shared__ unsigned long long red[DCN_N_STATS][4];
    int lane = threadIdx.x & 63, wave = threadIdx.x >> 6;
#pragma unroll
    for (int c = 0; c < DCN_N_STATS; ++c) {
        unsigned long long v = st[c];
#pragma unroll
        for (int d = 32; d >= 1; d >>= 1) v += __shfl_xor(v, d, 64);
        if (lane == 0) red[c][wave] = v;
    }
    __syncthreads();
    if (threadIdx.x < DCN_N_STATS) {
        unsigned long long v = red[threadIdx.x][0] + red[threadIdx.x][1] + red[threadIdx.x][2] + red[threadIdx.x][3];
        if (v) atomicAdd(&a.report->stats[threadIdx.x], v);
    }
}

__global__ __launch_bounds__(256) void probe_hashes_kernel(dcn_probe_hashes_args a) {
    uint64_t stride = (uint64_t)gridDim.x * blockDim.x;
    for (uint64_t i = (uint64_t)blockIdx.x * blockDim.x + threadIdx.x; i < a.n_hashes; i += stride) {
        uint64_t h = a.hashes[i];
        if (h == 0) {
            if (a.table.has_zero) {
                uint32_t lo = 0, hi = a.n_units - 1;
                while (lo < hi) {
                    uint32_t mid = lo + (hi - lo + 1) / 2;
                    if (a.hash_offsets[mid] <= i) lo = mid;
                    else hi = mid - 1;
                }
                a.g_zero[lo] = 1;
            }
        } else if (!dcn_table_contains_dev(a.table, h)) {
            a.hashes[i] = 0;
        }
    }
}

__global__ __launch_bounds__(256) void hash_units_kernel(dcn_probe_hashes_args a) {
    uint32_t u = blockIdx.x * blockDim.x + threadIdx.x;
    if (u == 0) {
        *a.n_tiles = a.n_units;
        a.status->any_records = 1;
        a.status->n_pending = a.n_units;
    }
    if (u >= a.n_units) return;
    const uint64_t n = a.hash_offsets[u + 1] - a.hash_offsets[u];
    dcn_tile t;
    t.scan_start = a.hash_offsets[u];
    t.unit = u;
    t.nwf = (uint32_t)n & 0x3FFFFFFFu;
    a.tiles[u] = t;
    a.tile_hits[u] = (uint32_t)n;
    a.unit_tile_first[u] = u;
    a.unit_tile_count[u] = 1;
    a.unit_state[u] = 0;
    a.pending[u] = u;
    a.g_total[u] = (uint32_t)n;
    a.g_hitcnt[u] = (uint32_t)n;
    a.g_distinct[u] = 0;
    a.g_zero[u] = 0;
}

inline uint32_t blocks_for(uint64_t n, uint32_t cap = 256 * 16) {
    uint64_t b = (n + 255) / 256;
    if (b < 1) b = 1;
    return (uint32_t)(b > cap ? cap : b);
}

}

int dcn_launch_plan(const dcn_plan_args &a, hipStream_t stream) {
    if (a.n_reads >= (1u << 19))
        hipLaunchKernelGGL(plan_kernel<8>, dim3((a.n_reads + 2047) / 2048), dim3(256), 0, stream, a);
    else
        hipLaunchKernelGGL(plan_kernel<1>, dim3((a.n_reads + 255) / 256), dim3(256), 0, stream, a);
    DCN_HIP(hipGetLastError());
    return DCN_OK;
}

int dcn_launch_distinct(const dcn_distinct_args &a, hipStream_t stream) {
    hipLaunchKernelGGL(unit_distinct_kernel, dim3(std::max(1u, std::min(a.n_units, 256u * 10u))), dim3(64), 0, stream, a);
    hipLaunchKernelGGL(distinct_clear_kernel, dim3(1024), dim3(256), 0, stream, a.set_slots, a.set_capacity, a.status);
    hipLaunchKernelGGL(big_insert_kernel, dim3(2048), dim3(256), 0, stream, a);
    DCN_HIP(hipGetLastError());
    return DCN_OK;
}

int dcn_launch_finish(const dcn_finish_args &a, hipStream_t stream) {
    hipLaunchKernelGGL(finish_kernel, dim3(blocks_for(a.n_units, 1024)), dim3(256), 0, stream, a);
    DCN_HIP(hipGetLastError());
    return DCN_OK;
}

int dcn_launch_probe_hashes(const dcn_probe_hashes_args &a, hipStream_t stream) {
    hipLaunchKernelGGL(hash_units_kernel, dim3((a.n_units + 255) / 256), dim3(256), 0, stream, a);
    if (a.n_hashes)
        hipLaunchKernelGGL(probe_hashes_kernel, dim3(blocks_for(a.n_hashes)), dim3(256), 0, stream, a);
    DCN_HIP(hipGetLastError());
    return DCN_OK;
}
```

### deacon-server_amd/csrc/scan.hip

```cpp
#include "dcn_internal.h"
#include "dcn_probe.h"

#include <atomic>

namespace {

__device__ __constant__ uint32_t NT_F[4] = {0x95c60474u, 0x62a02b4cu, 0x82572324u, 0x4be24456u};

__device__ inline uint32_t rotl32(uint32_t x, uint32_t r) { return __funnelshift_l(x, x, r); }

#ifndef DCN_WAVE_OPS_SHFL
#define DCN_WAVE_OPS_SHFL 0
#endif
template <bool MAX>
__device__ inline uint32_t wave_scan_dpp(uint32_t v) {
    auto op = [](uint32_t x, uint32_t y) { return MAX ? max(x, y) : x + y; };
    v = op(v, (uint32_t)__builtin_amdgcn_update_dpp(0, (int)v, 0x111, 0xf, 0xf, false));
    v = op(v, (uint32_t)__builtin_amdgcn_update_dpp(0, (int)v, 0x112, 0xf, 0xf, false));
    v = op(v, (uint32_t)__builtin_amdgcn_update_dpp(0, (int)v, 0x114, 0xf, 0xf, false));
    v = op(v, (uint32_t)__builtin_amdgcn_update_dpp(0, (int)v, 0x118, 0xf, 0xf, false));
    v = op(v, (uint32_t)__builtin_amdgcn_update_dpp(0, (int)v, 0x142, 0xa, 0xf, false));
    v = op(v, (uint32_t)__builtin_amdgcn_update_dpp(0, (int)v, 0x143, 0xc, 0xf, false));
    return v;
}

__device__ inline uint32_t wave_inclusive_scan_u32(uint32_t v, int lane) {
#if DCN_WAVE_OPS_SHFL
#pragma unroll
    for (int d = 1; d < 64; d <<= 1) {
        uint32_t o = __shfl_up(v, d, 64);
        if (lane >= d) v += o;
    }
    return v;
#else
    (void)lane;
    return wave_scan_dpp<false>(v);
#endif
}

__device__ inline uint32_t wave_max_u32(uint32_t v) {
#if DCN_WAVE_OPS_SHFL
#pragma unroll
    for (int d = 32; d >= 1; d >>= 1) v = max(v, __shfl_xor(v, d, 64));
    return v;
#else
    return (uint32_t)__builtin_amdgcn_readlane((int)wave_scan_dpp<true>(v), 63);
#endif
}

__device__ inline uint32_t wave_last_u32(uint32_t incl) {
#if DCN_WAVE_OPS_SHFL
    return __shfl(incl, 63, 64);
#else
    return (uint32_t)__builtin_amdgcn_readlane((int)incl, 63);
#endif
}

#ifndef DCN_LIST_BY_LANE
#define DCN_LIST_BY_LANE 1
#endif
#if DCN_LIST_BY_LANE
#define DCN_LIST_AT(lane_, entry_) list[lane_][entry_]
#else
#define DCN_LIST_AT(lane_, entry_) list[entry_][lane_]
#endif
constexpr int DCN_LSTRIDE = 42;
static_assert(DCN_LSTRIDE >= DCN_LCAP && (DCN_LSTRIDE / 2) % 2 == 1 && DCN_LSTRIDE % 2 == 0, "odd dword stride");
constexpr int DCN_RCAP = 256;

struct WaveShared {
    uint4 tab[16];
#if DCN_LIST_BY_LANE
    uint16_t list[DCN_WAVE][DCN_LSTRIDE];
#else
    uint16_t list[DCN_LCAP + 2][DCN_WAVE];
#endif
    uint64_t ring_hash[DCN_RCAP];
    uint32_t total[DCN_WAVE];
    uint32_t hits[DCN_WAVE];
    uint32_t items[DCN_WAVE];
    uint16_t hraw[DCN_WAVE];
    uint32_t ucap[DCN_WAVE];
    uint32_t unit_of[DCN_WAVE];
    uint16_t start[DCN_WAVE + 2];
    uint32_t uhits[DCN_WAVE];
    uint64_t run_base[DCN_WAVE];
    uint8_t local[DCN_WAVE];
    uint8_t lok[DCN_WAVE];
};

#ifndef DCN_EXP
#define DCN_EXP 0
#endif
#ifndef DCN_MIN_WAVES
#define DCN_MIN_WAVES 4
#endif
#ifndef DCN_FAST_EXTRA_ROUNDS
#define DCN_FAST_EXTRA_ROUNDS 4
#endif
#ifndef DCN_MIN_WAVES_FAST
#define DCN_MIN_WAVES_FAST 4
#endif

template <bool B>
struct BoolTag {
    static constexpr bool value = B;
};
template <int N>
struct IntTag {
    static constexpr int value = N;
};
#ifndef DCN_EXPORT_UNIFORM
#define DCN_EXPORT_UNIFORM 0
#endif
#ifndef DCN_PIPE_B
#define DCN_PIPE_B 0
#endif
#ifndef DCN_U_FINAL
#define DCN_U_FINAL 1
#endif

template <int W, bool K128, bool DUMP, bool FAST, bool VAR = false>
__global__ __launch_bounds__(DCN_WAVE, FAST ? DCN_MIN_WAVES_FAST : DCN_MIN_WAVES) void scan_kernel(dcn_scan_args a) {
    static_assert(!VAR || (W == 0 && !FAST), "the variant path is the generic-w counting / dump kernel");
    __shared__ WaveShared sh;
    extern __shared__ __align__(16) uint2 dyn_ring[];

    const int lane = threadIdx.x;
    const uint32_t NT = a.status->bad_offsets ? 0u : *a.n_tiles;
    const uint32_t wave_first = blockIdx.x * DCN_WAVE;
    if (wave_first >= NT) return;
    const uint32_t k = a.k;
    const uint32_t w = W > 0 ? (uint32_t)W : a.w;
    const uint32_t l = k + w - 1;

    const uint32_t tile_idx = wave_first + lane;
    const bool have_tile = tile_idx < NT;
    dcn_tile t = a.tiles[have_tile ? tile_idx : NT - 1];
    if (!have_tile) t.nwf = 0;
    const uint32_t carry = t.carry();
    const uint32_t nwc = t.n_windows() ? t.n_windows() + carry : 0;
    const uint32_t tile_read_pos = (DUMP && have_tile && a.tile_read_pos) ? a.tile_read_pos[tile_idx] : 0u;
    const uint32_t unit_prev = __shfl_up(t.unit, 1, 64);
    const uint64_t start_prev = (uint64_t)__shfl_up((long long)t.scan_start, 1, 64);
    const bool head = lane == 0 || t.unit != unit_prev || t.scan_start < start_prev;
    const unsigned long long head_mask = __ballot(head);
    const uint32_t uslot = (uint32_t)__popcll(head_mask & ((2ull << lane) - 1)) - 1;
    sh.total[lane] = 0;
    sh.hits[lane] = 0;
    sh.items[lane] = 0;
    sh.hraw[lane] = 0;
    sh.lok[lane] = 0;
    sh.uhits[lane] = 0;
    sh.ucap[lane] = 0;
    if (head) {
        sh.unit_of[uslot] = t.unit;
        sh.run_base[uslot] = (t.scan_start + carry) >> a.rec_shift;
        bool loc = false;
        if (!DUMP) {
            if (t.whole_unit()) {
                loc = true;
            } else {
                uint32_t first = a.unit_tile_first[t.unit], count = a.unit_tile_count[t.unit];
                loc = count != 0xFFFFFFFFu && first >= wave_first && first + count <= wave_first + DCN_WAVE;
            }
        }
        sh.local[uslot] = loc ? 1 : 0;
    }
    const uint32_t ROT = VAR ? a.nt_rot : 1u;
    const uint32_t ROTR = (32u - ROT) & 31u;
    if (lane < 16) {
        uint32_t in = lane & 3, out = lane >> 2;
        uint4 e;
        e.x = NT_F[in];
        e.y = rotl32(NT_F[in ^ 2], (ROT * (k - 1)) & 31);
        e.z = rotl32(NT_F[out], (ROT * k) & 31);
        e.w = rotl32(NT_F[out ^ 2], ROTR);
        sh.tab[lane] = e;
    }
    __syncthreads();
    if (!DUMP) {
        const uint32_t head_lane = 63u - (uint32_t)__clzll(head_mask & ((2ull << lane) - 1));
        const uint64_t first_win = (uint64_t)__shfl((long long)(t.scan_start + carry), head_lane, 64);
        const uint32_t slack = t.n_windows() < a.tile_windows ? l - 1 : 0u;
        if (have_tile && t.n_windows()) atomicMax(&sh.ucap[uslot], (uint32_t)(t.scan_start + carry + t.n_windows() + slack - first_win));
        __syncthreads();
        if (head) sh.ucap[uslot] = (uint32_t)(((first_win + sh.ucap[uslot]) >> a.rec_shift) - (first_win >> a.rec_shift));
        __syncthreads();
    }

    const uint32_t *packed = a.packed;
    const int64_t s = (int64_t)t.scan_start;

    uint32_t fw = 0, rc = 0, tg = 0;
    {
        const int64_t q_in = s >> 4;
        const uint32_t sh_in = (uint32_t)(s & 15) * 2;
        uint32_t cur = 0;
        for (uint32_t tt = 0; tt + 1 < k; ++tt) {
            if ((tt & 15) == 0) cur = __funnelshift_r(packed[q_in + (tt >> 4)], packed[q_in + (tt >> 4) + 1], sh_in);
            uint32_t c = (cur >> (2 * (tt & 15))) & 3;
            uint4 e = sh.tab[c];
            fw = rotl32(fw, VAR ? ROT : 1u) ^ e.x;
            rc = rotl32(rc, VAR ? ROTR : 31u) ^ e.y;
            tg += c >> 1;
        }
    }
    uint32_t zprev = 0, wprev = 0;

    uint32_t cnt = 0;
    uint32_t emitted_before = 0;
    bool first_pending = carry;
    uint32_t prev = 0xFFFFFFFFu;
    uint32_t n_ring = 0;
    bool go_global = false;
    bool any_rec = false;
    const uint32_t nk = nwc ? nwc + w - 1 : 0;
    const uint32_t jmax = wave_max_u32(nk);

    auto flush = [&](auto u_tag, bool final_flush) {
        constexpr int U = decltype(u_tag)::value;
#ifdef DCN_PHASEB_PRIO
        __builtin_amdgcn_s_setprio(DCN_PHASEB_PRIO);
#endif
        const uint32_t skip0 = (first_pending && cnt > 0) ? 1u : 0u;
        const uint32_t us_skip = uslot | (skip0 << 8);
        const uint32_t cnt_eff = cnt - skip0;
        uint32_t incl = wave_inclusive_scan_u32(cnt_eff, lane);
        uint32_t M = wave_last_u32(incl);
        sh.start[lane] = (uint16_t)(incl - cnt_eff);
        if (lane == 63) sh.start[64] = (uint16_t)M;
        if (!DUMP && cnt_eff) atomicAdd(&sh.items[uslot], cnt_eff);
        if (!final_flush) go_global = true;
        __syncthreads();
        if (!DUMP && head) {
            bool ok = sh.local[uslot] && !go_global && sh.items[uslot] <= (uint32_t)(DCN_RCAP - DCN_WAVE);
            sh.lok[uslot] = ok ? 1 : 0;
        }
        __syncthreads();
        constexpr int NPW = K128 ? 5 : 3;
        constexpr int NMW = K128 ? 3 : 2;
        constexpr bool PIPE = DCN_PIPE_B && U == 1;
        struct Item {
            bool act;
            uint32_t lo, idx, rel, o_uslot;
            uint64_t p;
            uint32_t mw[NMW], pw[NPW];
        };
        auto fetch = [&](uint32_t E, Item &it) {
            const uint32_t e = E + lane;
            it.act = e < M;
            uint32_t l_ = 0, h_ = 63;
#pragma unroll
            for (int step = 0; step < 6; ++step) {
                const uint32_t mid = (l_ + h_ + 1) >> 1;
                const bool le = sh.start[mid] <= e;
                l_ = le ? mid : l_;
                h_ = le ? h_ : mid - 1;
            }
            it.lo = l_;
            it.idx = it.act ? e - sh.start[l_] : 0;
            const uint32_t o_pk = __shfl(us_skip, l_, 64);
            const uint32_t o_skip = o_pk >> 8;
#ifdef DCN_DEBUG_BOUNDS
            if (it.act && (l_ > 63u || it.idx + o_skip >= (uint32_t)DCN_LCAP + 2u)) {
                a.status->bounds = 1;
                it.act = false;
                it.idx = 0;
            }
#endif
            it.rel = sh.DCN_LIST_AT(l_, it.idx + o_skip);
            const long long o_s = __shfl((long long)s, l_, 64);
            it.o_uslot = o_pk & 0xFFu;
            it.p = (uint64_t)(o_s + it.rel);
#ifdef DCN_DEBUG_BOUNDS
            if (it.act && it.p + k > a.stream_bases) {
                a.status->bounds = 2;
                it.act = false;
                it.p = 0;
            }
#endif
            if (it.act) {
                const uint32_t *mp = a.invmask + (it.p >> 5);
                const uint32_t *pp = packed + (it.p >> 4);
#pragma unroll
                for (int q = 0; q < NMW; ++q) it.mw[q] = mp[q];
#pragma unroll
                for (int q = 0; q < NPW; ++q) it.pw[q] = pp[q];
            }
        };
        Item cur, nxt;
        if (PIPE && M) fetch(0, cur);
        for (uint32_t E = 0; E < ((DCN_EXP & 2) ? 0u : M); E += DCN_WAVE * U) {
            bool act[U];
            uint32_t lo[U], hi[U];
#pragma unroll
            for (int u = 0; u < U; ++u) {
                act[u] = E + u * DCN_WAVE + lane < M;
                lo[u] = 0;
                hi[u] = 63;
            }
            if (!PIPE) {
#pragma unroll
            for (int it = 0; it < 6; ++it) {
#pragma unroll
                for (int u = 0; u < U; ++u) {
                    uint32_t e = E + u * DCN_WAVE + lane;
                    uint32_t mid = (lo[u] + hi[u] + 1) >> 1;
                    bool le = sh.start[mid] <= e;
                    lo[u] = le ? mid : lo[u];
                    hi[u] = le ? hi[u] : mid - 1;
                }
            }
            }
            uint64_t p[U];
            uint32_t o_uslot[U], idx[U], rel[U];
            uint32_t mw[U][NMW], pw[U][NPW];
            if (PIPE) {
                act[0] = cur.act;
                lo[0] = cur.lo;
                idx[0] = cur.idx;
                rel[0] = cur.rel;
                o_uslot[0] = cur.o_uslot;
                p[0] = cur.p;
#pragma unroll
                for (int q = 0; q < NMW; ++q) mw[0][q] = cur.mw[q];
#pragma unroll
                for (int q = 0; q < NPW; ++q) pw[0][q] = cur.pw[q];
            }
#pragma unroll
            for (int u = 0; u < (PIPE ? 0 : U); ++u) {
                uint32_t e = E + u * DCN_WAVE + lane;
                idx[u] = act[u] ? e - sh.start[lo[u]] : 0;
                const uint32_t o_pk = __shfl(us_skip, lo[u], 64);
                const uint32_t o_skip = o_pk >> 8;
#ifdef DCN_DEBUG_BOUNDS
                if (act[u] && (lo[u] > 63u || idx[u] + o_skip >= (uint32_t)DCN_LCAP + 2u)) {
                    a.status->bounds = 1;
                    act[u] = false;
                    idx[u] = 0;
                }
#endif
                rel[u] = sh.DCN_LIST_AT(lo[u], idx[u] + o_skip);
                long long o_s = __shfl((long long)s, lo[u], 64);
                o_uslot[u] = o_pk & 0xFFu;
                p[u] = (uint64_t)(o_s + rel[u]);
#ifdef DCN_DEBUG_BOUNDS
                if (act[u] && p[u] + k > a.stream_bases) {
                    a.status->bounds = 2;
                    act[u] = false;
                    p[u] = 0;
                }
#endif
            }
#pragma unroll
            for (int u = 0; u < (PIPE ? 0 : U); ++u) {
                if (act[u]) {
                    const uint32_t *mp = a.invmask + (p[u] >> 5);
                    const uint32_t *pp = packed + (p[u] >> 4);
#pragma unroll
                    for (int q = 0; q < NMW; ++q) mw[u][q] = (DCN_EXP & 16) ? 0u : mp[q];
#pragma unroll
                    for (int q = 0; q < NPW; ++q) pw[u][q] = pp[q];
                }
            }
            bool valid[U];
            uint64_t hash[U];
#pragma unroll
            for (int u = 0; u < U; ++u) {
                valid[u] = false;
                hash[u] = 0;
                if (act[u]) {
                    uint32_t msh = (uint32_t)(p[u] & 31);
                    if constexpr (K128) {
                        uint64_t mbits = ((uint64_t)__funnelshift_r(mw[u][1], mw[u][NMW - 1], msh) << 32) |
                                         __funnelshift_r(mw[u][0], mw[u][1], msh);
                        valid[u] = (mbits & ((~0ull) >> (64 - k))) == 0;
                    } else {
                        valid[u] = (__funnelshift_r(mw[u][0], mw[u][1], msh) & (0xFFFFFFFFu >> (32 - k))) == 0;
                    }
                    uint32_t psh = (uint32_t)(p[u] & 15) * 2;
                    uint64_t lo64 = ((uint64_t)__funnelshift_r(pw[u][1], pw[u][2], psh) << 32) |
                                    __funnelshift_r(pw[u][0], pw[u][1], psh);
                    if constexpr (K128) {
                        uint64_t hi64 = ((uint64_t)__funnelshift_r(pw[u][3], pw[u][NPW - 1], psh) << 32) |
                                        __funnelshift_r(pw[u][2], pw[u][3], psh);
                        hash[u] = dcn_kmer_hash128_bits(lo64, hi64, k);
                    } else {
                        hash[u] = dcn_kmer_hash64_bits(lo64, k);
                    }
                }
            }
            if (DUMP) {
#pragma unroll
                for (int u = 0; u < U; ++u) {
                    uint32_t o_eb = __shfl(emitted_before, lo[u], 64);
                    uint32_t o_rp = __shfl(tile_read_pos, lo[u], 64);
                    uint32_t o_carry = __shfl(carry, lo[u], 64);
                    long long o_s = __shfl((long long)s, lo[u], 64);
                    if (act[u]) {
                        uint64_t slot = (uint64_t)o_s + o_carry + o_eb + idx[u];
                        a.dump_hash[slot] = valid[u] ? hash[u] : 0;
                        a.dump_pos[slot] = a.dump_abs ? (uint32_t)p[u] : o_rp + rel[u];
                        a.dump_valid[slot] = valid[u] ? 1 : 0;
                    }
                }
                if (PIPE) {
                    if (E + DCN_WAVE < M) fetch(E + DCN_WAVE, nxt);
                    cur = nxt;
                }
                continue;
            }
            uint32_t grp[U];
            dcn_group g[U];
#pragma unroll
            for (int u = 0; u < U; ++u) {
                grp[u] = dcn_group_of(hash[u], a.table.group_shift, a.table.group_mask);
                if (valid[u] && !(DCN_EXP & 1)) g[u] = dcn_load_group(a.table, grp[u]);
            }
            if (PIPE && E + DCN_WAVE < M) fetch(E + DCN_WAVE, nxt);
            bool hit[U];
#pragma unroll
            for (int u = 0; u < U; ++u) {
                hit[u] = false;
                if (valid[u]) {
                    if (DCN_EXP & 1) {
                        hit[u] = (hash[u] & 1) != 0;
                    } else if (hash[u] == 0) {
                        hit[u] = a.table.has_zero != 0;
                    } else {
                        int r = dcn_group_resolve(g[u], hash[u]);
                        while (r < 0) {
                            grp[u] = (grp[u] + 1) & a.table.group_mask;
                            r = dcn_group_resolve(dcn_load_group(a.table, grp[u]), hash[u]);
                        }
                        hit[u] = r == 1;
                    }
                } else if (act[u]) {
                    atomicSub(&sh.total[o_uslot[u]], 1u);
                }
            }
#pragma unroll
            for (int u = 0; u < U; ++u) {
                const bool lok = hit[u] && sh.lok[o_uslot[u]];
                const unsigned long long hb = __ballot(lok);
                if (hb) {
                    const unsigned long long lt = (1ull << lane) - 1;
                    const uint32_t nh = (uint32_t)__popcll(hb);
                    const uint32_t rank = (uint32_t)__popcll(hb & lt);
                    const uint32_t x = n_ring + rank;
                    if (lok) sh.ring_hash[x & (DCN_RCAP - 1)] = hash[u];
                    const unsigned long long below = hb & lt;
                    const uint32_t prev_lane = below ? 63u - (uint32_t)__clzll(below) : (uint32_t)lane;
                    const uint32_t prev_us = __shfl(o_uslot[u], prev_lane, 64);
                    const bool run_head = lok && (below == 0 || prev_us != o_uslot[u]);
                    const unsigned long long hm_all = __ballot(run_head);
                    const unsigned long long hm = hm_all & (lt | (1ull << lane));
                    const uint32_t head_lane = hm ? 63u - (uint32_t)__clzll(hm) : 0u;
                    const uint32_t rank_head = (uint32_t)__popcll(hb & ((1ull << head_lane) - 1));
                    const uint32_t run = lok ? sh.hraw[o_uslot[u]] + (rank - rank_head) : 0u;
                    __syncthreads();
                    bool dup = false;
                    for (uint32_t d0 = 0; __any(d0 < ((DCN_EXP & 8) ? 0u : run)); d0 += 4) {
                        uint64_t v0 = sh.ring_hash[(x - d0 - 1) & (DCN_RCAP - 1)];
                        uint64_t v1 = sh.ring_hash[(x - d0 - 2) & (DCN_RCAP - 1)];
                        uint64_t v2 = sh.ring_hash[(x - d0 - 3) & (DCN_RCAP - 1)];
                        uint64_t v3 = sh.ring_hash[(x - d0 - 4) & (DCN_RCAP - 1)];
                        dup |= (d0 + 0 < run && v0 == hash[u]) | (d0 + 1 < run && v1 == hash[u]) |
                               (d0 + 2 < run && v2 == hash[u]) | (d0 + 3 < run && v3 == hash[u]);
                    }
                    const unsigned long long db = __ballot(dup);
                    if (run_head) {
                        const unsigned long long later = hm_all & ~((2ull << lane) - 1);
                        const unsigned long long upto = later ? ((1ull << (__ffsll((long long)later) - 1)) - 1) : ~0ull;
                        const unsigned long long rm = hb & upto & ~lt;
                        sh.hraw[o_uslot[u]] += (uint32_t)__popcll(rm);
                        sh.hits[o_uslot[u]] += (uint32_t)__popcll(rm & ~db);
                    }
                    n_ring += nh;
                    __syncthreads();
                }
                {
                    const bool rec = hit[u] && !lok;
                    const unsigned long long rb = (DCN_EXP & 256) ? 0ull : __ballot(rec);
#if DCN_EXPORT_UNIFORM
                    const uint32_t us0 = rb ? (uint32_t)__builtin_amdgcn_readlane((int)o_uslot[u], __ffsll((long long)rb) - 1) : 0u;
                    const bool one_unit = rb && __ballot(rec && o_uslot[u] != us0) == 0;
                    if (one_unit) {
                        const unsigned long long lt = (1ull << lane) - 1;
                        any_rec = true;
                        const uint32_t base = sh.uhits[us0];
                        if (rec) {
                            const uint32_t at = base + (uint32_t)__popcll(rb & lt);
                            if (at < sh.ucap[us0]) {
                                if (!(DCN_EXP & 512)) a.rec_hash[sh.run_base[us0] + at] = hash[u];
                            } else {
                                a.status->run_overflow = 1;
                            }
                            if (hash[u] == 0) a.g_zero[sh.unit_of[us0]] = 1;
                            if ((rb & lt) == 0) sh.uhits[us0] = base + (uint32_t)__popcll(rb);
                        }
                    } else
#endif
                    if (rb) {
                        const unsigned long long lt = (1ull << lane) - 1;
                        const unsigned long long below = rb & lt;
                        const uint32_t prev_lane = below ? 63u - (uint32_t)__clzll(below) : (uint32_t)lane;
                        const uint32_t prev_us = __shfl(o_uslot[u], prev_lane, 64);
                        const bool run_head = rec && (below == 0 || prev_us != o_uslot[u]);
                        const unsigned long long hm_all = __ballot(run_head);
                        const unsigned long long hm = hm_all & (lt | (1ull << lane));
                        const uint32_t head_lane = hm ? 63u - (uint32_t)__clzll(hm) : 0u;
                        const uint32_t rank = (uint32_t)__popcll(below) - (uint32_t)__popcll(rb & ((1ull << head_lane) - 1));
                        any_rec = true;
                        if (rec) {
                            const uint32_t at = sh.uhits[o_uslot[u]] + rank;
                            if (at < sh.ucap[o_uslot[u]]) {
                                if (!(DCN_EXP & 512)) a.rec_hash[sh.run_base[o_uslot[u]] + at] = hash[u];
                            } else {
                                a.status->run_overflow = 1;
                            }
                            if (hash[u] == 0) a.g_zero[sh.unit_of[o_uslot[u]]] = 1;
                        }
                        if (run_head) {
                            const unsigned long long later = hm_all & ~((2ull << lane) - 1);
                            const unsigned long long upto = later ? ((1ull << (__ffsll((long long)later) - 1)) - 1) : ~0ull;
                            sh.uhits[o_uslot[u]] += (uint32_t)__popcll(rb & upto & ~lt);
                        }
                    }
                }
            }
            if (PIPE) cur = nxt;
        }
        if (!DUMP && cnt_eff) atomicAdd(&sh.total[uslot], cnt_eff);
        emitted_before += cnt_eff;
        if (skip0) first_pending = false;
        cnt = 0;
        __syncthreads();
#ifdef DCN_PHASEB_PRIO
        __builtin_amdgcn_s_setprio(0);
#endif
    };

    constexpr uint32_t STEP = W > 0 ? (uint32_t)W : 8u;
    static_assert(STEP < DCN_LCAP && STEP <= 16, "a block's bits must fit one word and the list must outlast a block");
    uint32_t ringL[STEP], ringR[STEP];
    uint32_t pl = 0xFFFFFFFFu, pr = 0;
    if (W > 0) {
#pragma unroll
        for (uint32_t r = 0; r < STEP; ++r) {
            ringL[r] = 0xFFFFFFFFu;
            ringR[r] = 0;
        }
    } else if (VAR) {
        for (uint32_t r = 0; r < w; ++r)
            reinterpret_cast<ulonglong2 *>(dyn_ring)[r * DCN_WAVE + lane] = make_ulonglong2(~0ull, 0ull);
    } else {
        for (uint32_t r = 0; r < w; ++r) dyn_ring[r * DCN_WAVE + lane] = make_uint2(0xFFFFFFFFu, 0u);
    }
    uint32_t gslot = 0;
    uint32_t keymask = 0xFFFF0000u;
    asm volatile("" : "+v"(keymask));
    const uint32_t lhalf = l >> 1;

    int64_t b_in = 2 * (s + (int64_t)(k - 1)), b_k = 2 * s, b_l = 2 * (s - (int64_t)(w - 1));
    int64_t wi_in = b_in >> 5, wi_k = b_k >> 5, wi_l = b_l >> 5;
    uint32_t so_in = (uint32_t)(b_in & 31), so_k = (uint32_t)(b_k & 31), so_l = (uint32_t)(b_l & 31);
    uint32_t ra_in = packed[wi_in], rb_in = packed[wi_in + 1];
    uint32_t ra_k = packed[wi_k], rb_k = packed[wi_k + 1];
    uint32_t ra_l = packed[wi_l], rb_l = packed[wi_l + 1];
    uint32_t w_in = __funnelshift_r(ra_in, rb_in, so_in);
    uint32_t w_k = __funnelshift_r(ra_k, rb_k, so_k);
    uint32_t w_l = __funnelshift_r(ra_l, rb_l, so_l);
    auto advance_streams = [&]() {
        so_in += 2 * STEP; wi_in += so_in >> 5; so_in &= 31;
        so_k += 2 * STEP; wi_k += so_k >> 5; so_k &= 31;
        so_l += 2 * STEP; wi_l += so_l >> 5; so_l &= 31;
        if (DCN_EXP & 128) {
            ra_in = rb_in ^ 0x5A5A5A5Au; rb_in = ra_k + 0x1234567u; ra_k = rb_l; rb_k = ra_l ^ ra_in; ra_l = rb_k; rb_l = rb_in;
            return;
        }
        ra_in = packed[wi_in]; rb_in = packed[wi_in + 1];
        if (DCN_EXP & 64) {
            ra_k = ra_in; rb_k = rb_in; ra_l = ra_in; rb_l = rb_in;
        } else {
            ra_k = packed[wi_k]; rb_k = packed[wi_k + 1];
            ra_l = packed[wi_l]; rb_l = packed[wi_l + 1];
        }
    };
    advance_streams();
    {
        if (W > 0) {
            uint32_t m = (w - 1) >= 16 ? 0xAAAAAAAAu : (0xAAAAAAAAu & ((1u << (2 * (w - 1))) - 1u));
            tg += __popc(w_l & m);
        } else {
            for (uint32_t b = 1; b < w; ++b) {
                int64_t p = s - (int64_t)b;
                tg += (packed[p >> 4] >> (2 * (uint32_t)(p & 15) + 1)) & 1u;
            }
        }
    }
    uint4 e_nx = sh.tab[(w_in & 3) | ((w_k & 3) << 2)];

    auto block = [&](auto first_tag, const uint32_t jb) {
        constexpr bool FIRST = decltype(first_tag)::value;
        const uint32_t te = (w_in & 0x33333333u) | ((w_k & 0x33333333u) << 2);
        const uint32_t to = ((w_in >> 2) & 0x33333333u) | (w_k & 0xCCCCCCCCu);
        uint32_t nw_in = 0, nw_k = 0, nw_l = 0;
#pragma unroll
        for (uint32_t r = 0; r < STEP; ++r) {
            const uint32_t j = jb + r;
            const uint4 e = e_nx;
            if (r + 1 < STEP) {
                const uint32_t tsel = ((r + 1) & 1) ? to : te;
                const uint32_t n = (r + 1) >> 1;
                const uint32_t addr16 = n == 0 ? ((tsel << 4) & 0xF0u) : ((tsel >> (4 * n - 4)) & 0xF0u);
                e_nx = *reinterpret_cast<const uint4 *>(reinterpret_cast<const char *>(sh.tab) + addr16);
            } else {
                nw_in = __funnelshift_r(ra_in, rb_in, so_in);
                nw_k = __funnelshift_r(ra_k, rb_k, so_k);
                nw_l = __funnelshift_r(ra_l, rb_l, so_l);
                e_nx = sh.tab[(nw_in & 3) | ((nw_k & 3) << 2)];
                advance_streams();
            }
            const uint32_t hi_in = (w_in >> (2 * r + 1)) & 1;
            const uint32_t hl = (w_l >> (2 * r + 1)) & 1;
            fw = __builtin_amdgcn_bitop3_b32(rotl32(fw, VAR ? ROT : 1u), zprev, e.x, 0x96);
            rc = __builtin_amdgcn_bitop3_b32(rotl32(rc, VAR ? ROTR : 31u), wprev, e.y, 0x96);
            zprev = e.z;
            wprev = e.w;
            const uint32_t h = (VAR && a.nt_combine_xor) ? (fw ^ rc) : (fw + rc);
            const uint32_t jlow = j & 0xFFFFu;
            const uint32_t lk = __builtin_amdgcn_bitop3_b32(h, keymask, jlow, 0xEA);
            const uint32_t rk = __builtin_amdgcn_bitop3_b32(h, keymask, jlow, 0xAE);
            uint32_t lmin, rmax;
            if constexpr (W > 0) {
                ringL[r] = lk;
                ringR[r] = rk;
                pl = min(pl, lk);
                pr = max(pr, rk);
                if (r == W - 1) {
#pragma unroll
                    for (int qq = W - 2; qq >= 0; --qq) {
                        ringL[qq] = min(ringL[qq], ringL[qq + 1]);
                        ringR[qq] = max(ringR[qq], ringR[qq + 1]);
                    }
                    lmin = ringL[0];
                    rmax = ringR[0];
                    pl = 0xFFFFFFFFu;
                    pr = 0;
                } else {
                    lmin = min(pl, ringL[(r + 1) % STEP]);
                    rmax = max(pr, ringR[(r + 1) % STEP]);
                }
            } else if constexpr (VAR) {
                ulonglong2 *ring64 = reinterpret_cast<ulonglong2 *>(dyn_ring);
                ring64[gslot * DCN_WAVE + lane] = make_ulonglong2(((unsigned long long)(h & a.cmp_mask) << 32) | j,
                                                                  ((unsigned long long)(~h & a.cmp_mask) << 32) | j);
                gslot = gslot + 1 == w ? 0 : gslot + 1;
                unsigned long long lmin64 = ~0ull, rmax64 = 0ull;
                for (uint32_t qq = 0; qq < w; ++qq) {
                    ulonglong2 v = ring64[qq * DCN_WAVE + lane];
                    lmin64 = v.x < lmin64 ? v.x : lmin64;
                    rmax64 = v.y > rmax64 ? v.y : rmax64;
                }
                lmin = (uint32_t)lmin64;
                rmax = (uint32_t)rmax64;
            } else {
                dyn_ring[gslot * DCN_WAVE + lane] = make_uint2(lk, rk);
                gslot = gslot + 1 == w ? 0 : gslot + 1;
                lmin = 0xFFFFFFFFu;
                rmax = 0;
                for (uint32_t qq = 0; qq < w; ++qq) {
                    uint2 v = dyn_ring[qq * DCN_WAVE + lane];
                    lmin = min(lmin, v.x);
                    rmax = max(rmax, v.y);
                }
            }
            tg += hi_in;
            if constexpr (W > 0) {
                if (!FIRST || r == STEP - 1) {
                    const uint32_t sel = ((tg > lhalf) ? lmin : rmax) & 0xFFFFu;
                    const bool emit = FIRST ? (nwc > 0) : ((j - (w - 1) < nwc) && sel != prev);
                    if (!(DCN_EXP & 4)) sh.DCN_LIST_AT(lane, cnt) = (uint16_t)sel;
                    cnt += emit ? 1u : 0u;
                    prev = sel;
                }
            } else {
                const uint32_t sel = ((tg > lhalf) ? lmin : rmax) & 0xFFFFu;
                const uint32_t i = j - (w - 1);
                const bool in_range = i < nwc;
                const bool emit = in_range && sel != prev;
                sh.DCN_LIST_AT(lane, cnt) = (uint16_t)sel;
                cnt += emit ? 1u : 0u;
                prev = in_range ? sel : prev;
            }
            tg -= hl;
        }
        w_in = nw_in;
        w_k = nw_k;
        w_l = nw_l;
    };

    if (jmax > 0) {
        block(BoolTag<true>{}, 0);
        if (__any(cnt > DCN_LCAP - STEP)) flush(IntTag<1>{}, false);
        for (uint32_t jb = STEP; jb < jmax; jb += STEP) {
            block(BoolTag<false>{}, jb);
            if (__any(cnt > DCN_LCAP - STEP)) flush(IntTag<1>{}, false);
        }
    }
    if (FAST && !DUMP && !go_global) {
        const uint32_t skip0 = (first_pending && cnt > 0) ? 1u : 0u;
        const uint32_t cnt_eff = cnt - skip0;
        const unsigned long long tile_mask = __ballot(have_tile);
        const unsigned long long up1 = lane < 63 ? 1ull << (lane + 1) : 0ull, down1 = lane > 0 ? 1ull << (lane - 1) : 0ull;
        const bool prev_head = (head_mask & down1) != 0;
        const bool next_mate = (tile_mask & up1) != 0 && (head_mask & up1) == 0;
        const uint32_t uh = head ? (uint32_t)lane : (uint32_t)lane - 1u;
        const uint32_t partner = head ? (next_mate ? (uint32_t)lane + 1u : (uint32_t)lane) : (uint32_t)lane - 1u;
        const uint32_t partner_cnt = __shfl(cnt_eff, partner, 64);
        const uint32_t cnt_unit = cnt_eff + (partner != (uint32_t)lane ? partner_cnt : 0u);
        const bool own = !have_tile || ((head || (prev_head && a.early_out_pairs)) && sh.local[uslot] && cnt_unit <= a.early_out_max_items);
        if (__all(own)) {
            const uint32_t need = (uint32_t)a.abs_threshold;
            uint64_t seen0 = 0, seen1 = 0, seen2 = 0;
            uint32_t nh = 0;
            auto probe_item = [&](uint64_t p, bool actv, uint64_t &hash) -> bool {
                bool hit = false;
                hash = 0;
                if (actv) {
                    const uint32_t *mp = a.invmask + (p >> 5);
                    const uint32_t *pp = packed + (p >> 4);
                    const uint32_t m0 = mp[0], m1 = mp[1], m2 = K128 ? mp[2] : 0u;
                    uint32_t pw[K128 ? 5 : 3];
#pragma unroll
                    for (int q = 0; q < (K128 ? 5 : 3); ++q) pw[q] = pp[q];
                    const uint32_t msh = (uint32_t)(p & 31);
                    bool valid;
                    if constexpr (K128) {
                        const uint64_t mbits = ((uint64_t)__funnelshift_r(m1, m2, msh) << 32) | __funnelshift_r(m0, m1, msh);
                        valid = (mbits & ((~0ull) >> (64 - k))) == 0;
                    } else {
                        valid = (__funnelshift_r(m0, m1, msh) & (0xFFFFFFFFu >> (32 - k))) == 0;
                    }
                    const uint32_t psh = (uint32_t)(p & 15) * 2;
                    const uint64_t lo64 = ((uint64_t)__funnelshift_r(pw[1], pw[2], psh) << 32) | __funnelshift_r(pw[0], pw[1], psh);
                    if constexpr (K128) {
                        const uint64_t hi64 = ((uint64_t)__funnelshift_r(pw[3], pw[4], psh) << 32) | __funnelshift_r(pw[2], pw[3], psh);
                        hash = dcn_kmer_hash128_bits(lo64, hi64, k);
                    } else {
                        hash = dcn_kmer_hash64_bits(lo64, k);
                    }
                    if (valid) {
                        if (hash == 0) {
                            hit = a.table.has_zero != 0;
                        } else {
                            uint32_t grp = dcn_group_of(hash, a.table.group_shift, a.table.group_mask);
                            int r = dcn_group_resolve(dcn_load_group(a.table, grp), hash);
                            while (r < 0) {
                                grp = (grp + 1) & a.table.group_mask;
                                r = dcn_group_resolve(dcn_load_group(a.table, grp), hash);
                            }
                            hit = r == 1;
                        }
                    }
                }
                return hit;
            };
            auto note_hit = [&](uint64_t hash) {
                const bool dup = (nh > 0 && hash == seen0) | (nh > 1 && hash == seen1) | (nh > 2 && hash == seen2);
                if (!dup) {
                    seen2 = nh == 2 ? hash : seen2;
                    seen1 = nh == 1 ? hash : seen1;
                    seen0 = nh == 0 ? hash : seen0;
                    ++nh;
                }
            };
            const uint32_t maxc = wave_max_u32(cnt_eff);
            const uint32_t R1 = min(need + (uint32_t)DCN_FAST_EXTRA_ROUNDS, maxc);
            for (uint32_t j = 0; j < R1; ++j) {
                const bool actv = j < cnt_eff && nh < need;
                if (!__any(actv)) break;
                uint64_t hash;
                const uint32_t rel = sh.DCN_LIST_AT(lane, (actv ? j : 0u) + skip0);
                const bool hit = probe_item((uint64_t)(s + rel), actv, hash);
                const bool p_hit = __shfl((int)hit, partner, 64) != 0;
                const uint64_t p_hash = (uint64_t)__shfl((long long)hash, partner, 64);
                const bool paired_lane = partner != (uint32_t)lane;
                const bool h1 = head ? hit : p_hit, h2 = head ? (paired_lane && p_hit) : hit;
                const uint64_t v1 = head ? hash : p_hash, v2 = head ? p_hash : hash;
                if (h1 && nh < need) note_hit(v1);
                if (h2 && nh < need) note_hit(v2);
            }
            const uint32_t rem = (nh < need && cnt_eff > R1) ? cnt_eff - R1 : 0u;
            const uint32_t incl = wave_inclusive_scan_u32(rem, lane);
            const uint32_t M = wave_last_u32(incl);
            if (M) {
                sh.start[lane] = (uint16_t)(incl - rem);
                if (lane == 63) sh.start[64] = (uint16_t)M;
                __syncthreads();
                for (uint32_t E = 0; E < M; E += DCN_WAVE) {
                    const uint32_t e = E + lane;
                    const bool act = e < M;
                    uint32_t lo = 0, hi = 63;
#pragma unroll
                    for (int it = 0; it < 6; ++it) {
                        const uint32_t mid = (lo + hi + 1) >> 1;
                        const bool le = sh.start[mid] <= e;
                        lo = le ? mid : lo;
                        hi = le ? hi : mid - 1;
                    }
                    const uint32_t idx = act ? e - sh.start[lo] + R1 : 0u;
                    const uint32_t o_skip = __shfl(skip0, lo, 64);
                    const uint32_t o_nh = __shfl(nh, lo, 64);
                    const long long o_s = __shfl((long long)s, lo, 64);
                    const uint32_t rel = sh.DCN_LIST_AT(lo, idx + o_skip);
                    uint64_t hash;
                    const bool hit = probe_item((uint64_t)(o_s + rel), act && o_nh < need, hash);
                    unsigned long long hb = __ballot(hit);
                    while (hb) {
                        const int src = __ffsll((long long)hb) - 1;
                        hb &= hb - 1;
                        const uint64_t h = (uint64_t)__shfl((long long)hash, src, 64);
                        const uint32_t o = __shfl(lo, src, 64);
                        const uint32_t o_uh = __shfl(uh, o, 64);
                        if (uh == o_uh && nh < need) note_hit(h);
                    }
                }
            }
            if (have_tile && head) {
                a.keep[t.unit] = (a.deplete ? nh < need : nh >= need) ? 1 : 0;
                a.unit_state[t.unit] = 1;
            }
            return;
        }
    }
    flush(IntTag<DCN_U_FINAL>{}, true);
    if (DUMP) {
        if (have_tile) a.dump_count[tile_idx] = emitted_before;
        return;
    }

    if (any_rec && lane == 0) a.status->any_records = 1;
    {
        const bool pending = have_tile && !sh.lok[uslot] && !(DCN_EXP & 1024);
        bool enrol = false;
        if (pending) {
            const uint32_t th = head ? sh.uhits[uslot] : 0u;
            a.tile_hits[tile_idx] = th;
            if (th) enrol = atomicAdd(&a.g_hitcnt[t.unit], th) == 0u;
        }
        const unsigned long long em = __ballot(enrol);
        if (em) {
            uint32_t base = 0;
            if (lane == 0) base = atomicAdd(&a.status->n_pending, (uint32_t)__popcll(em));
            base = __shfl(base, 0, 64);
            if (enrol) {
                a.pending[base + (uint32_t)__popcll(em & ((1ull << lane) - 1))] = t.unit;
                if (t.whole_unit()) {
                    a.unit_tile_first[t.unit] = tile_idx;
                    a.unit_tile_count[t.unit] = 1;
                }
            }
        }
    }

    if (head && have_tile) {
        uint32_t tot = sh.total[uslot];
        if (sh.lok[uslot]) {
            uint32_t hc = sh.hits[uslot];
            a.keep[t.unit] = dcn_decide(hc, tot, a.abs_threshold, a.rel_threshold, a.deplete) ? 1 : 0;
            if (a.hits) a.hits[t.unit] = hc;
            if (a.total) a.total[t.unit] = tot;
            a.unit_state[t.unit] = 1;
        } else if (tot) {
            atomicAdd(&a.g_total[t.unit], tot);
        }
    }
}

template <int W, bool VAR = false>
int launch_w(const dcn_scan_args &args, uint32_t blocks, bool dump, bool k128, size_t dyn, hipStream_t stream) {
#define DCN_LAUNCH(K128_, DUMP_, FAST_)                                                               \
    do {                                                                                              \
        auto kern = scan_kernel<W, K128_, DUMP_, FAST_ && !VAR, VAR>;                                 \
        if (dyn > 0) {                                                                                \
            hipError_t e = hipFuncSetAttribute(reinterpret_cast<const void *>(kern),                  \
                                               hipFuncAttributeMaxDynamicSharedMemorySize, (int)dyn); \
            if (e != hipSuccess) return dcn_fail(DCN_ERR_HIP, std::string("dyn LDS: ") + hipGetErrorString(e)); \
        }                                                                                             \
        hipLaunchKernelGGL(kern, dim3(blocks), dim3(DCN_WAVE), dyn, stream, args);                    \
    } while (0)
    const bool fast = !dump && args.early_out_max_items != 0;
    if (k128) {
        if (dump) DCN_LAUNCH(true, true, false);
        else if (fast) DCN_LAUNCH(true, false, true);
        else DCN_LAUNCH(true, false, false);
    } else {
        if (dump) DCN_LAUNCH(false, true, false);
        else if (fast) DCN_LAUNCH(false, false, true);
        else DCN_LAUNCH(false, false, false);
    }
#undef DCN_LAUNCH
    DCN_HIP(hipGetLastError());
    return DCN_OK;
}

}

namespace {
std::atomic<uint32_t> g_variant{DCN_VARIANT_DEFAULT};
}

uint32_t dcn_current_variant() { return g_variant.load(); }

int dcn_set_minimizer_variant(uint32_t nt_rot, uint32_t cmp_bits, uint32_t combine) {
    if (nt_rot < 1 || nt_rot > 31) return dcn_fail(DCN_ERR_ARG, "minimizer variant: rotation must be 1..31");
    if (cmp_bits != 16 && cmp_bits != 32) return dcn_fail(DCN_ERR_ARG, "minimizer variant: 16 or 32 hash bits are compared");
    if (combine > 1) return dcn_fail(DCN_ERR_ARG, "minimizer variant: combine is 0 (fw + rc) or 1 (fw ^ rc)");
    g_variant.store((nt_rot << 16) | (cmp_bits << 8) | combine);
    return DCN_OK;
}

int dcn_get_minimizer_variant(uint32_t *nt_rot, uint32_t *cmp_bits, uint32_t *combine) {
    const uint32_t v = g_variant.load();
    if (nt_rot) *nt_rot = v >> 16;
    if (cmp_bits) *cmp_bits = (v >> 8) & 0xFF;
    if (combine) *combine = v & 0xFF;
    return DCN_OK;
}

int dcn_launch_scan(const dcn_scan_args &args_in, uint32_t max_tiles, bool dump, hipStream_t stream) {
    if (max_tiles == 0) return DCN_OK;
    uint32_t blocks = (max_tiles + DCN_WAVE - 1) / DCN_WAVE;
    bool k128 = args_in.k > 32;
    const uint32_t v = args_in.variant ? args_in.variant : DCN_VARIANT_DEFAULT;
    if (v != DCN_VARIANT_DEFAULT) {
        dcn_scan_args args = args_in;
        args.nt_rot = v >> 16;
        args.cmp_mask = ((v >> 8) & 0xFF) == 32 ? 0xFFFFFFFFu : 0xFFFF0000u;
        args.nt_combine_xor = v & 0xFF;
        args.early_out_max_items = 0;
        if (args.w > 128) return dcn_fail(DCN_ERR_ARG, "minimizer variant: w <= 128 (two u64 keys per window slot in LDS)");
        size_t dyn = (size_t)args.w * DCN_WAVE * sizeof(ulonglong2);
        return launch_w<0, true>(args, blocks, dump, k128, dyn, stream);
    }
    const dcn_scan_args &args = args_in;
    switch (args.w) {
    case 15: return launch_w<15>(args, blocks, dump, k128, 0, stream);
    case 11: return launch_w<11>(args, blocks, dump, k128, 0, stream);
    case 1: return launch_w<1>(args, blocks, dump, k128, 0, stream);
    default: {
        size_t dyn = (size_t)args.w * DCN_WAVE * sizeof(uint2);
        return launch_w<0>(args, blocks, dump, k128, dyn, stream);
    }
    }
}
```

### deacon-server_amd/filter.py

```python
import ctypes as C
import os

import numpy as np

from . import _native as N
from ._native import DeaconHipError, Params

DEFAULT_KMER_LENGTH = 31
DEFAULT_WINDOW_SIZE = 15


def _ptr(a):
    return a.ctypes.data_as(C.c_void_p) if a is not None else None


def _as_u8(seq):
    if isinstance(seq, np.ndarray):
        return np.ascontiguousarray(seq, dtype=np.uint8)
    if isinstance(seq, str):
        seq = seq.encode()
    return np.frombuffer(bytes(seq), dtype=np.uint8)


def concat_reads(reads):
# ... 586 lines not shown
        super().close()


class Placer(_Context):

    def __init__(self, anchor_map, max_batch_bases=1 << 26, max_batch_reads=1 << 20, band_bases=256, min_votes=2,
                 prefix_length=0):
        self.anchor_map = anchor_map
        self.band_bases = int(band_bases)
        self.min_votes = int(min_votes)
        self.prefix_length = int(prefix_length)
        super().__init__(anchor_map._h, max_batch_bases, max_batch_reads)

    def _params(self):
        return N.PlaceParams(self.band_bases, self.min_votes, self.prefix_length, (C.c_uint32 * 2)(0, 0))

    def place_batch(self, bases, offsets):
        bases, offsets, n_reads = _batch(bases, offsets)
        out = np.zeros(max(n_reads, 1), PLACEMENT_DTYPE)
        p = self._params()
        N.check(N.lib().dcn_place_batch(self._h, self.anchor_map._h, _ptr(bases) if len(bases) else None, _ptr(offsets),
                                        n_reads, C.byref(p), _ptr(out)))
        return out[:n_reads]

    def place(self, reads):
        bases, offsets = concat_reads(list(reads))
        return self.place_batch(bases, offsets)

    def place_split_batch(self, bases, offsets, max_placements=4, capacity=None):
        bases, offsets, n_reads = _batch(bases, offsets)
        cap = n_reads * int(max_placements) if capacity is None else int(capacity)
        place_offsets = np.zeros(n_reads + 1, np.uint64)
        out = np.zeros(max(cap, 1), SPLIT_PLACEMENT_DTYPE)
        counts = np.zeros((max(n_reads, 1), 2), np.uint32)
        p = N.PlaceSplitParams(self.band_bases, self.min_votes, self.prefix_length, int(max_placements), (C.c_uint32 * 3)(0, 0, 0))
        N.check(N.lib().dcn_place_split_batch(self._h, self.anchor_map._h, _ptr(bases) if len(bases) else None, _ptr(offsets),
                                              n_reads, C.byref(p), _ptr(place_offsets), _ptr(out) if cap else None, cap,
                                              _ptr(counts)))
        return place_offsets, out[:int(place_offsets[n_reads])], counts[:n_reads]

    def place_split(self, reads, max_placements=4):
        reads = list(reads)
        bases, offsets = concat_reads(reads)
        po, rows, _ = self.place_split_batch(bases, offsets, max_placements)
        return [rows[int(po[r]):int(po[r + 1])] for r in range(len(reads))]

    def place_pair_batch(self, bases, offsets, max_placements=4, max_insert=1000, hist_bin_bases=8, want_hist=True):
        bases, offsets, n_reads = _batch(bases, offsets)
        out = np.zeros(max(n_reads, 1), PAIR_PLACEMENT_DTYPE)
        hist = np.zeros(N.PAIR_HIST_BINS, np.uint64) if want_hist else None
        p = N.PlacePairParams(self.band_bases, self.min_votes, self.prefix_length, int(max_placements), int(max_insert),
                              int(hist_bin_bases), (C.c_uint32 * 3)(0, 0, 0))
        N.check(N.lib().dcn_place_pair_batch(self._h, self.anchor_map._h, _ptr(bases) if len(bases) else None, _ptr(offsets),
                                             n_reads, C.byref(p), _ptr(out), _ptr(hist) if want_hist else None))
        return out[:n_reads], hist

    def place_pairs(self, reads1, reads2, **kw):
        reads1, reads2 = list(reads1), list(reads2)
        if len(reads1) != len(reads2):
            raise ValueError("place_pairs: the two lists must have one mate each per pair")
        bases, offsets = concat_reads([m for pair in zip(reads1, reads2) for m in pair])
        return self.place_pair_batch(bases, offsets, **kw)


class FilterProcessor(_Context):

    def __init__(self, index, abs_threshold=2, rel_threshold=0.01, prefix_length=0, deplete=False,
                 max_batch_bases=1 << 26, max_batch_reads=1 << 20):
        self.index = index
        self.abs_threshold = int(abs_threshold)
        self.rel_threshold = float(rel_threshold)
        self.prefix_length = int(prefix_length)
        self.deplete = bool(deplete)
        super().__init__(index._h, max_batch_bases, max_batch_reads)

    def _params(self):
        return Params(self.abs_threshold, self.rel_threshold, self.prefix_length, 1 if self.deplete else 0, 0)

    def filter_batch(self, bases, offsets, unit_id=None, counts=True):
        bases, offsets, n_reads = _batch(bases, offsets)
        if unit_id is not None:
            unit_id = np.ascontiguousarray(unit_id, dtype=np.uint32)
            n_units = int(unit_id[-1]) + 1 if n_reads else 0
        else:
            n_units = n_reads
        keep = np.zeros(max(n_units, 1), np.uint8)
        p = self._params()
        if not counts:
            N.check(N.lib().dcn_filter_batch(self._h, _ptr(bases) if len(bases) else None, _ptr(offsets),
                                             _ptr(unit_id), n_reads, C.byref(p), _ptr(keep), None, None))
            return keep[:n_units].astype(bool)
        hits = np.zeros(max(n_units, 1), np.uint32)
        total = np.zeros(max(n_units, 1), np.uint32)
        N.check(N.lib().dcn_filter_batch(self._h, _ptr(bases) if len(bases) else None, _ptr(offsets),
                                         _ptr(unit_id), n_reads, C.byref(p), _ptr(keep), _ptr(hits), _ptr(total)))
        return keep[:n_units].astype(bool), hits[:n_units], total[:n_units]

    def _outputs(self, offsets, unit_id, counts, out):
        n_reads = len(offsets) - 1
        n_units = (int(unit_id[-1]) + 1 if n_reads else 0) if unit_id is not None else n_reads
        if out is not None:
            keep, hits, total = out
        else:
            keep = np.zeros(max(n_units, 1), np.uint8)
            hits = np.zeros(max(n_units, 1), np.uint32) if counts else None
            total = np.zeros(max(n_units, 1), np.uint32) if counts else None
        return n_reads, n_units, keep, hits, total

    def submit(self, bases, offsets, unit_id=None, counts=True, out=None):
        bases, offsets, _ = _batch(bases, offsets)
        if unit_id is not None:
            unit_id = np.ascontiguousarray(unit_id, dtype=np.uint32)
        n_reads, n_units, keep, hits, total = self._outputs(offsets, unit_id, counts, out)
        p = self._params()
        t = C.c_uint64()
        N.check(N.lib().dcn_filter_batch_submit(self._h, _ptr(bases) if len(bases) else None, _ptr(offsets),
                                                _ptr(unit_id), n_reads, C.byref(p), _ptr(keep), _ptr(hits),
                                                _ptr(total), C.byref(t)))
        return PendingBatch(self, t.value, n_units, keep, hits, total, (bases, offsets, unit_id, p))

    def submit_packed(self, packed, invmask, offsets, unit_id=None, counts=True, out=None):
        packed = np.ascontiguousarray(packed, dtype=np.uint32)
        invmask = np.ascontiguousarray(invmask, dtype=np.uint32)
        offsets = np.ascontiguousarray(offsets, dtype=np.uint64)
        if unit_id is not None:
            unit_id = np.ascontiguousarray(unit_id, dtype=np.uint32)
        n_reads, n_units, keep, hits, total = self._outputs(offsets, unit_id, counts, out)
        g = (int(offsets[-1]) + 31) // 32 if n_reads else 0
        if len(packed) < 2 * g or len(invmask) < g:
            raise ValueError("packed / invmask must hold whole 32-base groups of the batch")
        p = self._params()
        t = C.c_uint64()
        N.check(N.lib().dcn_filter_batch_packed_submit(self._h, _ptr(packed), _ptr(invmask), _ptr(offsets),
                                                       _ptr(unit_id), n_reads, C.byref(p), _ptr(keep), _ptr(hits),
                                                       _ptr(total), C.byref(t)))
        return PendingBatch(self, t.value, n_units, keep, hits, total, (packed, invmask, offsets, unit_id, p))

    def filter_batch_packed(self, packed, invmask, offsets, unit_id=None, counts=True):
        return self.submit_packed(packed, invmask, offsets, unit_id, counts).wait()

    def filter_reads(self, reads, paired=False):
        bases, offsets = concat_reads(reads)
        unit_id = (np.arange(len(reads), dtype=np.uint32) // 2) if paired else None
        return self.filter_batch(bases, offsets, unit_id)

    def filter_batch_device(self, d_bases, d_offsets, n_reads, n_bases, d_keep, d_hits=None, d_total=None,
                            d_unit_id=None, n_units=None):
        p = self._params()
        if n_units is None:
            n_units = n_reads
        N.check(N.lib().dcn_filter_batch_device(self._h, d_bases, d_offsets, d_unit_id, n_reads, n_bases, n_units,
                                                C.byref(p), d_keep, d_hits, d_total))

    def reserve_records(self, n_records):
        N.check(N.lib().dcn_ctx_reserve_records(self._h, int(n_records)))

    def should_keep_sequence(self, seq):
        keep, hits, total = self.filter_reads([seq])
        return bool(keep[0]), int(hits[0]), int(total[0])

    def should_keep_pair(self, seq1, seq2):
        keep, hits, total = self.filter_reads([seq1, seq2], paired=True)
        return bool(keep[0]), int(hits[0]), int(total[0])

    def reset_stats(self):
        N.check(N.lib().dcn_ctx_reset_stats(self._h))

    def set_profiling(self, enable=True):
        N.check(N.lib().dcn_ctx_set_profiling(self._h, 2 if enable == 2 else (1 if enable else 0)))

    def summary(self, elapsed_seconds):
        s = self.stats()
        seqs_in, bp_in = s["total_seqs"], s["total_bp"]
        seqs_out, bp_out = seqs_in - s["filtered_seqs"], s["output_bp"]

        def prop(a, b):
            return a / b if b else 0.0

        return {
            "k": self.index.kmer_length, "w": self.index.window_size,
            "abs_threshold": self.abs_threshold, "rel_threshold": self.rel_threshold,
            "prefix_length": self.prefix_length, "deplete": self.deplete,
            "seqs_in": seqs_in, "seqs_out": seqs_out, "seqs_out_proportion": prop(seqs_out, seqs_in),
            "seqs_removed": s["filtered_seqs"], "seqs_removed_proportion": prop(s["filtered_seqs"], seqs_in),
            "bp_in": bp_in, "bp_out": bp_out, "bp_out_proportion": prop(bp_out, bp_in),
            "bp_removed": s["filtered_bp"], "bp_removed_proportion": prop(s["filtered_bp"], bp_in),
            "time": elapsed_seconds,
            "seqs_per_second": int(seqs_in / elapsed_seconds) if elapsed_seconds > 0 else 0,
            "bp_per_second": int(bp_in / elapsed_seconds) if elapsed_seconds > 0 else 0,
        }

    def minimizer_hashes_batch(self, bases, offsets, prefix_length=None):
        bases, offsets, n_reads = _batch(bases, offsets)
        pl = self.prefix_length if prefix_length is None else int(prefix_length)
        out_off = np.zeros(n_reads + 1, np.uint64)
        cap = max(int(len(bases)), 1)
        hashes = np.zeros(cap, np.uint64)
        pos = np.zeros(cap, np.uint32)
        N.check(N.lib().dcn_minimizer_hashes_batch(self._h, _ptr(bases) if len(bases) else None, _ptr(offsets),
                                                   n_reads, pl, _ptr(out_off), _ptr(hashes), _ptr(pos), cap))
        n = int(out_off[-1])
        return out_off, hashes[:n], pos[:n]

    def should_keep_hashes(self, hashes, hash_offsets):
        hashes = np.ascontiguousarray(hashes, dtype=np.uint64)
        hash_offsets = np.ascontiguousarray(hash_offsets, dtype=np.uint64)
        n_units = len(hash_offsets) - 1
        keep = np.zeros(max(n_units, 1), np.uint8)
        hits = np.zeros(max(n_units, 1), np.uint32)
        total = np.zeros(max(n_units, 1), np.uint32)
        p = self._params()
        N.check(N.lib().dcn_should_keep_hashes(self._h, _ptr(hashes) if len(hashes) else None, _ptr(hash_offsets),
                                               n_units, C.byref(p), _ptr(keep), _ptr(hits), _ptr(total)))
        return keep[:n_units].astype(bool), hits[:n_units], total[:n_units]


def stats_allreduce(processors):
    arr = (C.c_void_p * len(processors))(*[p._h for p in processors])
    c = (C.c_uint64 * N.N_STATS)()
    N.check(N.lib().dcn_stats_allreduce(arr, len(processors), c))
    return dict(zip(N.STAT_NAMES, (int(x) for x in c)))


def get_minimizer_hashes_and_positions(processor, seq, prefix_length=0):
    bases, offsets = concat_reads([seq])
    _, h, p = processor.minimizer_hashes_batch(bases, offsets, prefix_length)
    return h, p


def _should_keep(processor, per_unit_hashes, abs_threshold, rel_threshold, deplete):
    lens = np.fromiter((len(h) for h in per_unit_hashes), dtype=np.uint64, count=len(per_unit_hashes))
    off = np.zeros(len(per_unit_hashes) + 1, np.uint64)
    np.cumsum(lens, out=off[1:])
    flat = (np.concatenate([np.asarray(h, dtype=np.uint64) for h in per_unit_hashes])
            if len(per_unit_hashes) and off[-1] else np.zeros(0, np.uint64))
    saved = (processor.abs_threshold, processor.rel_threshold, processor.deplete)
    processor.abs_threshold, processor.rel_threshold, processor.deplete = int(abs_threshold), float(rel_threshold), bool(deplete)
    try:
        keep, hits, total = processor.should_keep_hashes(flat, off)
    finally:
        processor.abs_threshold, processor.rel_threshold, processor.deplete = saved
    return [(bool(k), int(h), int(t)) for k, h, t in zip(keep, hits, total)]


def unpaired_should_keep(processor, input_minimizers, abs_threshold, rel_threshold, deplete):
    return _should_keep(processor, input_minimizers, abs_threshold, rel_threshold, deplete)


def paired_should_keep(processor, input_minimizers, abs_threshold, rel_threshold, deplete):
    return _should_keep(processor, input_minimizers, abs_threshold, rel_threshold, deplete)
```

### include/deacon_hip.h

```cpp
#ifndef DEACON_HIP_H
#define DEACON_HIP_H

#include <stddef.h>
#include <stdint.h>

#ifdef __cplusplus
extern "C" {
#endif

#define DCN_OK 0
#define DCN_ERR_ARG (-1)
#define DCN_ERR_HIP (-2)
#define DCN_ERR_NOMEM (-3)
#define DCN_ERR_IO (-4)
#define DCN_ERR_FORMAT (-5)
#define DCN_ERR_CAPACITY (-6)
#define DCN_ERR_INTERNAL (-7)

typedef struct dcn_index dcn_index;
typedef struct dcn_ctx dcn_ctx;

typedef struct dcn_params {
    uint64_t abs_threshold;
    double rel_threshold;
    uint64_t prefix_length;
    uint32_t deplete;
    uint32_t reserved;
} dcn_params;

enum {
    DCN_STAT_TOTAL_SEQS = 0,
    DCN_STAT_FILTERED_SEQS = 1,
    DCN_STAT_TOTAL_BP = 2,
    DCN_STAT_OUTPUT_BP = 3,
    DCN_STAT_FILTERED_BP = 4,
    DCN_STAT_OUTPUT_SEQ_COUNTER = 5,
    DCN_N_STATS = 6
};

#define DCN_ABI_MAJOR 1
#define DCN_ABI_MINOR 11
int dcn_abi_version(uint32_t *major, uint32_t *minor);
const char *dcn_version(void);
const char *dcn_last_error(void);
int dcn_device_count(int *count);

int dcn_set_minimizer_variant(uint32_t nt_rot, uint32_t cmp_bits, uint32_t combine );
int dcn_get_minimizer_variant(uint32_t *nt_rot, uint32_t *cmp_bits, uint32_t *combine);


int dcn_index_from_keys(const uint64_t *keys, uint64_t n, uint8_t k, uint8_t w, int device, dcn_index **out);

int dcn_index_from_file(const char *path, int device, dcn_index **out);

int dcn_index_build(const uint8_t *bases, const uint64_t *offsets, uint32_t n_seqs, uint8_t k, uint8_t w,
                    float entropy_threshold, uint64_t capacity_keys, int device, dcn_index **out);

int dcn_index_keys(const dcn_index *index, uint64_t *out, uint64_t capacity, uint64_t *n);

int dcn_index_write_file(const dcn_index *index, const char *path);

int dcn_index_union(const dcn_index *const *inputs, uint32_t n, dcn_index **out);

int dcn_index_diff(const dcn_index *first, const dcn_index *second, dcn_index **out);

int dcn_index_intersect(const dcn_index *const *inputs, uint32_t n, dcn_index **out);

int dcn_index_header(const dcn_index *index, uint8_t *k, uint8_t *w, uint64_t *n_keys);

int dcn_index_device(const dcn_index *index, int *device);

int dcn_index_memory(const dcn_index *index, uint64_t *table_bytes);

int dcn_index_contains(const dcn_index *index, const uint64_t *keys, uint64_t n, uint8_t *out);

int dcn_index_contains_device(const dcn_index *index, const uint64_t *d_keys, uint64_t n, uint8_t *d_out,
                              void *stream);

int dcn_index_probe_ceiling(const dcn_index *index, const uint64_t *d_keys, uint64_t n, uint32_t reps,
                            double *probes_per_s);

int dcn_index_clone(const dcn_index *index, int device, dcn_index **out);

void dcn_index_destroy(dcn_index *index);


int dcn_ctx_create(const dcn_index *index, uint64_t max_batch_bases, uint32_t max_batch_reads, dcn_ctx **out);
void dcn_ctx_destroy(dcn_ctx *ctx);


int dcn_filter_batch(dcn_ctx *ctx, const uint8_t *bases, const uint64_t *offsets, const uint32_t *unit_id,
                     uint32_t n_reads, const dcn_params *params, uint8_t *keep, uint32_t *hits,
                     uint32_t *total);

int dcn_filter_batch_submit(dcn_ctx *ctx, const uint8_t *bases, const uint64_t *offsets, const uint32_t *unit_id,
                            uint32_t n_reads, const dcn_params *params, uint8_t *keep, uint32_t *hits,
                            uint32_t *total, uint64_t *ticket);
int dcn_filter_batch_wait(dcn_ctx *ctx, uint64_t ticket);

int dcn_filter_batch_packed(dcn_ctx *ctx, const uint32_t *packed, const uint32_t *invmask, const uint64_t *offsets,
                            const uint32_t *unit_id, uint32_t n_reads, const dcn_params *params, uint8_t *keep,
                            uint32_t *hits, uint32_t *total);
int dcn_filter_batch_packed_submit(dcn_ctx *ctx, const uint32_t *packed, const uint32_t *invmask,
                                   const uint64_t *offsets, const uint32_t *unit_id, uint32_t n_reads,
                                   const dcn_params *params, uint8_t *keep, uint32_t *hits, uint32_t *total,
                                   uint64_t *ticket);

int dcn_pack_ascii(const uint8_t *bases, uint64_t n_bases, uint32_t *packed, uint32_t *invmask, uint32_t *saw_newline);

int dcn_filter_batch_device(dcn_ctx *ctx, const uint8_t *d_bases, const uint64_t *d_offsets,
                            const uint32_t *d_unit_id, uint32_t n_reads, uint64_t n_bases, uint32_t n_units,
                            const dcn_params *params, uint8_t *d_keep, uint32_t *d_hits, uint32_t *d_total);

int dcn_ctx_synchronize(dcn_ctx *ctx);

int dcn_ctx_reserve_records(dcn_ctx *ctx, uint64_t n_records);

void *dcn_ctx_stream(dcn_ctx *ctx);

int dcn_host_alloc(uint64_t bytes, void **out);
void dcn_host_free(void *p);

int dcn_minimizer_hashes_batch(dcn_ctx *ctx, const uint8_t *bases, const uint64_t *offsets, uint32_t n_reads,
                               uint64_t prefix_length, uint64_t *out_offsets, uint64_t *out_hashes,
                               uint32_t *out_positions, uint64_t capacity);

int dcn_should_keep_hashes(dcn_ctx *ctx, const uint64_t *hashes, const uint64_t *hash_offsets, uint32_t n_units,
                           const dcn_params *params, uint8_t *keep, uint32_t *hits, uint32_t *total);

int dcn_index_set_create(const dcn_index *const *members, uint32_t n, dcn_index **out);
void dcn_index_set_destroy(dcn_index *set);
int dcn_index_set_info(const dcn_index *set, uint32_t *n_members, uint8_t *k, uint8_t *w, uint64_t *n_keys,
                       uint64_t *table_bytes);

int dcn_index_set_select(const dcn_index *set, uint32_t all_of, uint32_t any_of, uint32_t none_of, uint32_t min_members,
                         uint32_t max_members, uint64_t *n_selected, dcn_index **out);
int dcn_index_set_overlap(const dcn_index *set, uint64_t *shared, uint64_t *exclusive, uint64_t *by_count);

int dcn_classify_batch(dcn_ctx *ctx, const dcn_index *set, const uint8_t *bases, const uint64_t *offsets,
                       const uint32_t *unit_id, uint32_t n_reads, const dcn_params *params, uint32_t *match,
                       uint32_t *hits, uint32_t *total);
int dcn_classify_batch_device(dcn_ctx *ctx, const dcn_index *set, const uint8_t *d_bases, const uint64_t *d_offsets,
                              const uint32_t *d_unit_id, uint32_t n_reads, uint64_t n_bases, uint32_t n_units,
                              const dcn_params *params, uint32_t *d_match, uint32_t *d_hits, uint32_t *d_total);

int dcn_index_set_coverage_enable(dcn_index *set, int enable);
int dcn_index_set_coverage_reset(dcn_index *set);
int dcn_index_set_coverage(const dcn_index *set, uint64_t *observed, uint64_t *keys);
int dcn_index_set_coverage_keys(const dcn_index *set, uint32_t member, uint64_t *out, uint64_t capacity, uint64_t *n);

int dcn_index_set_depth_enable(dcn_index *set, int enable);
int dcn_index_set_depth_reset(dcn_index *set);
int dcn_index_set_depth_stats(const dcn_index *set, uint64_t *observed, uint64_t *sum, uint64_t *saturated);
int dcn_index_set_depth_hist(const dcn_index *set, uint32_t member, uint32_t n_bins, uint64_t *hist);
int dcn_index_set_depth_keys(const dcn_index *set, uint32_t member, uint64_t *keys, uint32_t *depths, uint64_t capacity,
                             uint64_t *n);

typedef struct dcn_index_builder dcn_index_builder;
int dcn_index_builder_create(uint8_t k, uint8_t w, float entropy_threshold, uint64_t capacity_keys, int device, void **out);
int dcn_index_builder_add(void *builder, const uint8_t *bases, const uint64_t *offsets, uint32_t n_seqs);
int dcn_index_builder_info(const void *builder, uint64_t *n_keys, uint64_t *n_occurrences, uint64_t *n_bases,
                           uint64_t *device_bytes);
int dcn_index_builder_hist(const void *builder, uint32_t n_bins, uint64_t *hist);
int dcn_index_builder_counts(const void *builder, uint64_t *keys, uint32_t *counts, uint64_t capacity, uint64_t *n);
int dcn_index_builder_finish(const void *builder, uint32_t min_count, uint32_t max_count, uint64_t *n_selected,
                             dcn_index **out);
void dcn_index_builder_destroy(void *builder);

typedef struct dcn_locate_params {
    uint32_t max_gap;
    uint32_t min_hits;
    uint32_t member_mask;
    uint32_t reserved;
    uint64_t prefix_length;
} dcn_locate_params;
typedef struct dcn_segment {
    uint32_t start, end, n_hits, members;
} dcn_segment;

int dcn_locate_batch(dcn_ctx *ctx, const dcn_index *index, const uint8_t *bases, const uint64_t *offsets,
                     uint32_t n_reads, const void *params, uint64_t *seg_offsets, void *segs, uint64_t capacity);

typedef struct dcn_track_params {
    uint32_t bin_bases;
    uint32_t member_mask;
    uint32_t depth_cap;
    uint32_t reserved;
    uint64_t prefix_length;
} dcn_track_params;
typedef struct dcn_track_bin {
    uint32_t n_positions, n_keys, n_observed, max_depth;
    uint64_t sum_depth;
} dcn_track_bin;

int dcn_depth_track_batch(dcn_ctx *ctx, const dcn_index *set, const uint8_t *bases, const uint64_t *offsets,
                          uint32_t n_reads, const void *params, uint64_t *bin_offsets, void *bins, uint64_t capacity);

int dcn_anchor_map_create(const dcn_index *index, dcn_index **out);
int dcn_anchor_map_add(dcn_index *map, dcn_ctx *ctx, const uint8_t *bases, const uint64_t *offsets,
                       uint32_t n_records, uint32_t *first_record);
int dcn_anchor_map_info(const dcn_index *map, uint32_t *n_records, uint64_t *n_keys, uint64_t *n_anchors,
                        uint64_t *n_repeats);
int dcn_anchor_map_anchors(const dcn_index *map, uint64_t *keys, uint32_t *records, uint32_t *positions,
                           uint64_t capacity, uint64_t *n);

typedef struct dcn_place_params {
    uint32_t band_bases;
    uint32_t min_votes;
    uint64_t prefix_length;
    uint32_t reserved[2];
} dcn_place_params;
typedef struct dcn_placement {
    uint32_t record;
    uint32_t reverse;
    uint32_t votes, n_anchors, n_positions;
    uint32_t read_start, read_end;
    uint32_t reserved;
    uint64_t ref_start, ref_end;
} dcn_placement;

int dcn_place_batch(dcn_ctx *ctx, const dcn_index *map, const uint8_t *bases, const uint64_t *offsets,
                    uint32_t n_reads, const void *params, void *placements);

#define DCN_PLACE_SPLIT_MAX 8
typedef struct dcn_place_split_params {
    uint32_t band_bases, min_votes;
    uint64_t prefix_length;
    uint32_t max_placements;
    uint32_t reserved[3];
} dcn_place_split_params;
typedef struct dcn_split_placement {
    uint32_t record;
    uint32_t reverse;
    uint32_t votes, n_anchors, n_positions;
    uint32_t read_start, read_end;
    uint32_t reserved;
    uint64_t ref_start, ref_end;
    uint32_t rank, n_placed, rival_votes, mapq;
} dcn_split_placement;

int dcn_place_split_batch(dcn_ctx *ctx, const dcn_index *map, const uint8_t *bases, const uint64_t *offsets,
                          uint32_t n_reads, const void *params, uint64_t *place_offsets, void *placements,
                          uint64_t capacity, uint32_t *read_counts);

#define DCN_PAIR_HIST_BINS 256
#define DCN_PAIR_PROPER 1u
#define DCN_PAIR_RESCUED 2u
#define DCN_PAIR_MATE_PLACED 4u
typedef struct dcn_place_pair_params {
    uint32_t band_bases, min_votes;
    uint64_t prefix_length;
    uint32_t max_placements;
    uint32_t max_insert;
    uint32_t hist_bin_bases;
    uint32_t reserved[3];
} dcn_place_pair_params;
typedef struct dcn_pair_placement {
    uint32_t record;
    uint32_t reverse;
    uint32_t votes, n_anchors, n_positions;
    uint32_t read_start, read_end;
    uint32_t reserved;
    uint64_t ref_start, ref_end;
    uint32_t rank, n_placed, rival_votes, mapq;
    uint32_t flags;
    uint32_t pair_votes;
    int64_t tlen;
// ... 38 lines not shown
```

Measured before the change: 401,600.

## Fuse ASCII packing into scan kernel for short-read batches

Adds a shape-check kernel that flags a batch as short when every read fits within a fixed maximum length. For such batches the pack kernel exits early and a dedicated scan kernel loads ASCII directly, packs it into LDS staging per wave, and runs the shared scan body. This is meant to remove the global packed/invmask round trip and the separate pack pass. The cost is an extra shape kernel launch, an extra scan launch that early-exits otherwise, and more code paths. It is disabled for decisions-only calls that use early-out, which may be exactly the benchmark path.

```diff
diff --git a/deacon-server_amd/_native.py b/deacon-server_amd/_native.py
--- a/deacon-server_amd/_native.py
+++ b/deacon-server_amd/_native.py
@@ -197,6 +197,7 @@
     "dcn_filter_batch_device": (C.c_int, [_vp, _vp, _vp, _vp, C.c_uint32, C.c_uint64, C.c_uint32,
                                           C.POINTER(Params), _vp, _vp, _vp]),
     "dcn_ctx_synchronize": (C.c_int, [_vp]),
+    "dcn_ctx_last_batch_short": (C.c_int, [_vp, _u32p]),
     "dcn_ctx_reserve_records": (C.c_int, [_vp, C.c_uint64]),
     "dcn_ctx_stream": (_vp, [_vp]),
     "dcn_host_alloc": (C.c_int, [C.c_uint64, C.POINTER(_vp)]),
@@ -244,7 +245,7 @@
 }
 
 _lib = None
-ABI = (1, 11)
+ABI = (1, 12)
 
 
 def lib():
diff --git a/deacon-server_amd/csrc/ctx.hip b/deacon-server_amd/csrc/ctx.hip
--- a/deacon-server_amd/csrc/ctx.hip
+++ b/deacon-server_amd/csrc/ctx.hip
@@ -181,6 +181,9 @@
     uint32_t *packed = v.d_packed + DCN_FRONT_PAD, *invmask = v.d_invmask + DCN_FRONT_PAD;
     int ahead_buf = -1;
     const uint32_t *newline_flag = nullptr;
+    bool short_fused = false;
+    static const bool no_early_out = getenv("DCN_NO_EARLY_OUT") != nullptr, no_early_out_pairs = getenv("DCN_NO_EARLY_OUT_PAIRS") != nullptr;
+    const bool decisions_only_call = !v.d_hits && !v.d_total && params->abs_threshold >= 1 && params->abs_threshold <= 4 && !no_early_out;
     if (v.d_ascii && pack_ahead && c->profiling != 1 && ensure_pack_ahead(c)) {
         ahead_buf = c->pack_buf;
         c->pack_buf ^= 1;
@@ -197,6 +200,10 @@
         DCN_HIP(hipStreamWaitEvent(st, c->pack_done[ahead_buf], 0));
         newline_flag = &ps->any_newline;
     } else if (v.d_ascii) {
+        short_fused = c->short_fused && !v.d_unit_id && params->prefix_length == 0 && v.b0 == 0 && v.b1 == v.stream_bases &&
+                      v.n_reads == v.n_units && c->tile_windows >= dcn_short_lmax() && idx->variant == DCN_VARIANT_DEFAULT &&
+                      dcn_scan_has_short_path(idx->k, idx->w) && !decisions_only_call;
+        if (short_fused) DCN_TRY(dcn_launch_shape(v.d_offsets, v.n_reads, v.stream_bases, dcn_short_lmax(), c->d_status, st));
         DCN_TRY(dcn_launch_pack(v.d_ascii, v.b0, v.b1, packed, invmask, c->d_status, st));
     }
     DCN_PROF_MARK(DCN_STAGE_PACK);
@@ -223,8 +230,7 @@
     sa.rel_threshold = params->rel_threshold;
     sa.deplete = params->deplete;
     sa.early_out_max_items = 0;
-    static const bool no_early_out = getenv("DCN_NO_EARLY_OUT") != nullptr, no_early_out_pairs = getenv("DCN_NO_EARLY_OUT_PAIRS") != nullptr;
-    if (!v.d_hits && !v.d_total && params->abs_threshold >= 1 && params->abs_threshold <= 4 && !no_early_out) {
+    if (decisions_only_call) {
         uint32_t lo = 0, hi = 65535;
         while (lo < hi) {
             uint32_t mid = (lo + hi + 1) / 2;
@@ -247,6 +253,7 @@
     sa.tile_hits = c->d_tile_hits;
     sa.pending = c->d_pending;
     sa.status = c->d_status;
+    sa.ascii = short_fused ? v.d_ascii : nullptr;
     DCN_TRY(dcn_launch_scan(sa, tile_bound(c, n_reads, v.b1 - v.b0), false, st));
     DCN_PROF_MARK(DCN_STAGE_SCAN);
 
@@ -299,6 +306,7 @@
     if (!c->batch_pending) return DCN_OK;
     c->batch_pending = false;
     DCN_HIP(hipMemcpy(c->h_report, c->d_report, sizeof(dcn_batch_report), hipMemcpyDeviceToHost));
+    c->last_batch_short = c->h_report->short_batch != 0;
     if (c->h_report->bounds) {
         DCN_HIP(hipMemsetAsync(c->d_report, 0, offsetof(dcn_batch_report, stats), c->stream));
         return dcn_fail(DCN_ERR_INTERNAL, "scan kernel: index out of range in phase B (DCN_DEBUG_BOUNDS build)");
@@ -669,6 +677,7 @@
     if (!ok) return fail(dcn_fail(DCN_ERR_HIP, "stream/event creation failed"));
     c->rec_shift = 2;
     if (index->w <= 7) c->rec_shift = 0;
+    c->short_fused = getenv("DCN_NO_SHORT_FUSED") == nullptr;
     if (const char *rs = getenv("DCN_REC_SHIFT")) c->rec_shift = (uint32_t)std::min(3, std::max(0, atoi(rs)));
     uint64_t MR = max_batch_reads;
     const bool slab = getenv("DCN_CTX_SLAB") != nullptr;
@@ -754,6 +763,12 @@
     return alloc_records(ctx, n_records);
 }
 
+extern "C" int dcn_ctx_last_batch_short(dcn_ctx *ctx, uint32_t *was_short) {
+    if (!ctx || !was_short) return dcn_fail(DCN_ERR_ARG, "ctx/was_short is NULL");
+    *was_short = ctx->last_batch_short ? 1u : 0u;
+    return DCN_OK;
+}
+
 extern "C" int dcn_ctx_synchronize(dcn_ctx *ctx) {
     if (!ctx) return dcn_fail(DCN_ERR_ARG, "ctx is NULL");
     DCN_HIP(hipSetDevice(ctx->device));
diff --git a/deacon-server_amd/csrc/dcn_ctx.h b/deacon-server_amd/csrc/dcn_ctx.h
--- a/deacon-server_amd/csrc/dcn_ctx.h
+++ b/deacon-server_amd/csrc/dcn_ctx.h
@@ -92,6 +92,8 @@
     uint64_t rec_capacity = 0;
     uint64_t *d_set_slots = nullptr;
     dcn_status *d_status = nullptr;
+    bool short_fused = true;
+    bool last_batch_short = false;
     dcn_batch_report *d_report = nullptr;
     dcn_batch_report *h_report = nullptr;
     uint64_t host_stats[DCN_N_STATS] = {};
diff --git a/deacon-server_amd/csrc/dcn_internal.h b/deacon-server_amd/csrc/dcn_internal.h
--- a/deacon-server_amd/csrc/dcn_internal.h
+++ b/deacon-server_amd/csrc/dcn_internal.h
@@ -120,6 +120,10 @@
     uint32_t bounds;
     uint32_t run_overflow;
     uint32_t bad_offsets;
+    uint32_t short_batch;
+    uint32_t shape_bad;
+    uint32_t shape_done;
+    uint32_t reserved_;
     unsigned long long set_cursor;
 };
 
@@ -127,7 +131,7 @@
     uint32_t overflow;
     uint32_t bounds;
     uint32_t bad_offsets;
-    uint32_t reserved_;
+    uint32_t short_batch;
     unsigned long long need;
     unsigned long long stats[DCN_N_STATS];
 };
@@ -169,6 +173,7 @@
     uint32_t nt_rot;
     uint32_t cmp_mask;
     uint32_t nt_combine_xor;
+    const uint8_t *ascii;
 };
 
 int dcn_launch_pack(const uint8_t *d_ascii, uint64_t base_begin, uint64_t base_end, uint32_t *d_packed,
@@ -177,6 +182,10 @@
 int dcn_launch_pack_beside(const uint8_t *d_ascii, uint64_t base_begin, uint64_t base_end, uint32_t *d_packed, uint32_t *d_invmask,
                            dcn_status *status, hipStream_t stream);
 int dcn_launch_scan(const dcn_scan_args &args, uint32_t max_tiles, bool dump, hipStream_t stream);
+bool dcn_scan_has_short_path(uint32_t k, uint32_t w);
+uint32_t dcn_short_lmax();
+int dcn_launch_shape(const uint64_t *d_offsets, uint32_t n_reads, uint64_t stream_bases, uint32_t lmax, dcn_status *status,
+                     hipStream_t stream);
 
 int dcn_table_build(dcn_index *idx, const uint64_t *host_keys, uint64_t n);
 int dcn_table_contains(const dcn_index *idx, const uint64_t *host_keys, uint64_t n, uint8_t *out);
diff --git a/deacon-server_amd/csrc/dcn_pack.h b/deacon-server_amd/csrc/dcn_pack.h
--- /dev/null
+++ b/deacon-server_amd/csrc/dcn_pack.h
@@ -0,0 +1,23 @@
+#pragma once
+
+#include <stdint.h>
+
+#if defined(__HIPCC__) || defined(__CUDACC__)
+#define DCN_PACK_FN __host__ __device__ inline
+#else
+#define DCN_PACK_FN inline
+#endif
+
+DCN_PACK_FN uint32_t dcn_pack4(uint32_t x) {
+    uint32_t y = (x >> 1) & 0x03030303u;
+    return (y * ((1u << 24) | (1u << 18) | (1u << 12) | (1u << 6))) >> 24;
+}
+
+DCN_PACK_FN uint32_t dcn_invalid4(uint32_t x) {
+    const uint32_t y = x | 0x20202020u;
+    const uint32_t T = (y >> 2) & ~(y >> 1) & 0x01010101u;
+    const uint32_t expect = 0x60606060u | (T << 4) | (T ^ 0x01010101u);
+    const uint32_t diff = (y & 0xF9F9F9F9u) ^ expect;
+    const uint32_t nz = ((diff & 0x7F7F7F7Fu) + 0x7F7F7F7Fu) | diff;
+    return (((nz >> 7) & 0x01010101u) * 0x01020408u) >> 24;
+}
diff --git a/deacon-server_amd/csrc/pack.hip b/deacon-server_amd/csrc/pack.hip
--- a/deacon-server_amd/csrc/pack.hip
+++ b/deacon-server_amd/csrc/pack.hip
@@ -1,13 +1,9 @@
 #include "dcn_internal.h"
+#include "dcn_pack.h"
 
 #include <algorithm>
 
 namespace {
-
-__device__ inline uint32_t pack4(uint32_t x) {
-    uint32_t y = (x >> 1) & 0x03030303u;
-    return (y * ((1u << 24) | (1u << 18) | (1u << 12) | (1u << 6))) >> 24;
-}
 
 __device__ inline uint32_t pack4_index_side(uint32_t x) {
     uint32_t out = 0;
@@ -23,20 +19,12 @@
     return out;
 }
 
-__device__ inline uint32_t invalid4(uint32_t x) {
-    const uint32_t y = x | 0x20202020u;
-    const uint32_t T = (y >> 2) & ~(y >> 1) & 0x01010101u;
-    const uint32_t expect = 0x60606060u | (T << 4) | (T ^ 0x01010101u);
-    const uint32_t diff = (y & 0xF9F9F9F9u) ^ expect;
-    const uint32_t nz = ((diff & 0x7F7F7F7Fu) + 0x7F7F7F7Fu) | diff;
-    return (((nz >> 7) & 0x01010101u) * 0x01020408u) >> 24;
-}
-
 template <bool ALIGNED, bool INDEX_SIDE>
 __global__ __launch_bounds__(256) void pack_kernel(const uint8_t *__restrict__ ascii, uint64_t n_bases,
                                                    uint32_t *__restrict__ packed,
                                                    uint32_t *__restrict__ invmask, uint64_t g_first, uint64_t n_chunks,
                                                    dcn_status *status) {
+    if (!INDEX_SIDE && status && status->short_batch) return;
     uint64_t stride = (uint64_t)gridDim.x * blockDim.x;
     uint32_t nl = 0;
     for (uint64_t t = g_first + (uint64_t)blockIdx.x * blockDim.x + threadIdx.x; t < g_first + n_chunks; t += stride) {
@@ -63,11 +51,11 @@
         uint32_t p0 = 0, p1 = 0, m = 0;
 #pragma unroll
         for (int q = 0; q < 4; ++q) {
-            p0 |= (INDEX_SIDE ? pack4_index_side(w[q]) : pack4(w[q])) << (8 * q);
-            p1 |= (INDEX_SIDE ? pack4_index_side(w[q + 4]) : pack4(w[q + 4])) << (8 * q);
+            p0 |= (INDEX_SIDE ? pack4_index_side(w[q]) : dcn_pack4(w[q])) << (8 * q);
+            p1 |= (INDEX_SIDE ? pack4_index_side(w[q + 4]) : dcn_pack4(w[q + 4])) << (8 * q);
         }
 #pragma unroll
-        for (int q = 0; q < 8; ++q) m |= invalid4(w[q]) << (4 * q);
+        for (int q = 0; q < 8; ++q) m |= dcn_invalid4(w[q]) << (4 * q);
         if (!INDEX_SIDE && m) {
 #pragma unroll
             for (int q = 0; q < 8; ++q) {
@@ -91,8 +79,8 @@
     uint16_t *mask16 = reinterpret_cast<uint16_t *>(invmask);
     for (uint32_t t = h_first + blockIdx.x * 64u + threadIdx.x; t < h_end; t += stride) {
         const uint4 a = *reinterpret_cast<const uint4 *>(ascii + (uint64_t)t * 16);
-        const uint32_t p = pack4(a.x) | (pack4(a.y) << 8) | (pack4(a.z) << 16) | (pack4(a.w) << 24);
-        const uint32_t m = invalid4(a.x) | (invalid4(a.y) << 4) | (invalid4(a.z) << 8) | (invalid4(a.w) << 12);
+        const uint32_t p = dcn_pack4(a.x) | (dcn_pack4(a.y) << 8) | (dcn_pack4(a.z) << 16) | (dcn_pack4(a.w) << 24);
+        const uint32_t m = dcn_invalid4(a.x) | (dcn_invalid4(a.y) << 4) | (dcn_invalid4(a.z) << 8) | (dcn_invalid4(a.w) << 12);
         if (m) {
             uint32_t z = a.x ^ 0x0A0A0A0Au;
             nl |= (z - 0x01010101u) & ~z & 0x80808080u;
diff --git a/deacon-server_amd/csrc/plan.hip b/deacon-server_amd/csrc/plan.hip
--- a/deacon-server_amd/csrc/plan.hip
+++ b/deacon-server_amd/csrc/plan.hip
@@ -162,6 +162,33 @@
     }
 }
 
+__global__ __launch_bounds__(256) void shape_kernel(const uint64_t *__restrict__ offsets, uint32_t n_reads, uint64_t stream_bases,
+                                                    uint32_t lmax, dcn_status *status) {
+    bool bad = false;
+    const uint32_t stride = gridDim.x * blockDim.x;
+    for (uint32_t r0 = blockIdx.x * blockDim.x + threadIdx.x; r0 < n_reads; r0 += 4 * stride) {
+        uint64_t off[4], end[4];
+#pragma unroll
+        for (int q = 0; q < 4; ++q) {
+            const uint32_t r = r0 + q * stride;
+            off[q] = end[q] = 0;
+            if (r < n_reads && r >= r0) {
+                off[q] = offsets[r];
+                end[q] = offsets[r + 1];
+            }
+        }
+#pragma unroll
+        for (int q = 0; q < 4; ++q) bad |= end[q] < off[q] || end[q] > stream_bases || end[q] - off[q] > lmax;
+    }
+    const int any_bad = __syncthreads_or(bad ? 1 : 0);
+    if (threadIdx.x == 0) {
+        if (any_bad) atomicOr(&status->shape_bad, 1u);
+        __threadfence();
+        const bool last = atomicAdd(&status->shape_done, 1u) == gridDim.x - 1;
+        if (last && atomicOr(&status->shape_bad, 0u) == 0u) status->short_batch = 1;
+    }
+}
+
 #ifndef DCN_LDS_SET_LOG2
 #define DCN_LDS_SET_LOG2 11
 #endif
@@ -439,6 +466,7 @@
         }
     }
     if (a.status->bounds && blockIdx.x == 0 && threadIdx.x == 0) a.report->bounds = a.status->bounds;
+    if (blockIdx.x == 0 && threadIdx.x == 0) a.report->short_batch = a.status->short_batch;
     if (a.status->bad_offsets) {
         if (blockIdx.x == 0 && threadIdx.x == 0) a.report->bad_offsets = 1;
         return;
@@ -529,6 +557,14 @@
     return DCN_OK;
 }
 
+int dcn_launch_shape(const uint64_t *d_offsets, uint32_t n_reads, uint64_t stream_bases, uint32_t lmax, dcn_status *status,
+                     hipStream_t stream) {
+    hipLaunchKernelGGL(shape_kernel, dim3(blocks_for((n_reads + 3) / 4, 2048)), dim3(256), 0, stream, d_offsets, n_reads, stream_bases,
+                       lmax, status);
+    DCN_HIP(hipGetLastError());
+    return DCN_OK;
+}
+
 int dcn_launch_distinct(const dcn_distinct_args &a, hipStream_t stream) {
     hipLaunchKernelGGL(unit_distinct_kernel, dim3(std::max(1u, std::min(a.n_units, 256u * 10u))), dim3(64), 0, stream, a);
     hipLaunchKernelGGL(distinct_clear_kernel, dim3(1024), dim3(256), 0, stream, a.set_slots, a.set_capacity, a.status);
diff --git a/deacon-server_amd/csrc/scan.hip b/deacon-server_amd/csrc/scan.hip
--- a/deacon-server_amd/csrc/scan.hip
+++ b/deacon-server_amd/csrc/scan.hip
@@ -1,7 +1,10 @@
 #include "dcn_internal.h"
 #include "dcn_probe.h"
 
+#include "dcn_pack.h"
+
 #include <atomic>
+#include <type_traits>
 
 namespace {
 
@@ -89,6 +92,44 @@
     uint8_t lok[DCN_WAVE];
 };
 
+constexpr int DCN_SHORT_LMAX = 152;
+constexpr int DCN_STAGE_WORDS = 612;
+constexpr int DCN_LSTRIDE8 = 44;
+static_assert(DCN_LSTRIDE8 >= DCN_LCAP + 2 && (DCN_LSTRIDE8 / 4) % 2 == 1 && DCN_LSTRIDE8 % 4 == 0, "odd dword stride");
+static_assert(DCN_STAGE_WORDS % 2 == 0 && 16 * DCN_STAGE_WORDS >= 64 * DCN_SHORT_LMAX + 14 + 30, "one pass per full wave");
+
+struct WaveSharedShort {
+    uint4 tab[16];
+    uint32_t stage_p[DCN_STAGE_WORDS];
+    union {
+        uint32_t stage_m[DCN_STAGE_WORDS / 2 + 2];
+        uint16_t stage_m16[DCN_STAGE_WORDS + 4];
+    };
+#if DCN_LIST_BY_LANE
+    uint8_t list[DCN_WAVE][DCN_LSTRIDE8];
+#else
+    uint8_t list[DCN_LCAP + 2][DCN_WAVE];
+#endif
+    uint64_t ring_hash[DCN_RCAP];
+    uint32_t total[DCN_WAVE];
+    uint32_t hits[DCN_WAVE];
+    uint32_t items[DCN_WAVE];
+    uint32_t unit_of[DCN_WAVE];
+    uint16_t start[DCN_WAVE + 2];
+    uint8_t hraw[DCN_WAVE];
+    uint8_t uhits[DCN_WAVE];
+    uint8_t local[DCN_WAVE];
+    uint8_t lok[DCN_WAVE];
+};
+static_assert(sizeof(WaveSharedShort) <= 10240 && sizeof(WaveShared) <= 10240, "16 one-wave workgroups per CU of 160 KB");
+
+struct ShortLane {
+    int lane;
+    bool have;
+    dcn_tile t;
+    uint32_t s_local;
+};
+
 #ifndef DCN_EXP
 #define DCN_EXP 0
 #endif
@@ -120,13 +161,13 @@
 #define DCN_U_FINAL 1
 #endif
 
-template <int W, bool K128, bool DUMP, bool FAST, bool VAR = false>
-__global__ __launch_bounds__(DCN_WAVE, FAST ? DCN_MIN_WAVES_FAST : DCN_MIN_WAVES) void scan_kernel(dcn_scan_args a) {
+template <int W, bool K128, bool DUMP, bool FAST, bool VAR, bool SHORT, class SH>
+__device__ __forceinline__ void scan_body(const dcn_scan_args &a, SH &sh, const ShortLane &sl) {
     static_assert(!VAR || (W == 0 && !FAST), "the variant path is the generic-w counting / dump kernel");
-    __shared__ WaveShared sh;
+    static_assert(!SHORT || (W > 0 && !K128 && !DUMP && !FAST && !VAR), "the short path is a counting kernel of fixed w, k <= 32");
     extern __shared__ __align__(16) uint2 dyn_ring[];
 
-    const int lane = threadIdx.x;
+    const int lane = SHORT ? sl.lane : (int)threadIdx.x;
     const uint32_t NT = a.status->bad_offsets ? 0u : *a.n_tiles;
     const uint32_t wave_first = blockIdx.x * DCN_WAVE;
     if (wave_first >= NT) return;
@@ -135,27 +176,29 @@
     const uint32_t l = k + w - 1;
 
     const uint32_t tile_idx = wave_first + lane;
-    const bool have_tile = tile_idx < NT;
-    dcn_tile t = a.tiles[have_tile ? tile_idx : NT - 1];
+    const bool have_tile = SHORT ? sl.have : tile_idx < NT;
+    dcn_tile t;
+    if constexpr (SHORT) t = sl.t;
+    else t = a.tiles[have_tile ? tile_idx : NT - 1];
     if (!have_tile) t.nwf = 0;
     const uint32_t carry = t.carry();
     const uint32_t nwc = t.n_windows() ? t.n_windows() + carry : 0;
     const uint32_t tile_read_pos = (DUMP && have_tile && a.tile_read_pos) ? a.tile_read_pos[tile_idx] : 0u;
     const uint32_t unit_prev = __shfl_up(t.unit, 1, 64);
     const uint64_t start_prev = (uint64_t)__shfl_up((long long)t.scan_start, 1, 64);
-    const bool head = lane == 0 || t.unit != unit_prev || t.scan_start < start_prev;
+    const bool head = SHORT ? have_tile : (lane == 0 || t.unit != unit_prev || t.scan_start < start_prev);
     const unsigned long long head_mask = __ballot(head);
-    const uint32_t uslot = (uint32_t)__popcll(head_mask & ((2ull << lane) - 1)) - 1;
+    const uint32_t uslot = SHORT ? (uint32_t)lane : (uint32_t)__popcll(head_mask & ((2ull << lane) - 1)) - 1;
     sh.total[lane] = 0;
     sh.hits[lane] = 0;
     sh.items[lane] = 0;
     sh.hraw[lane] = 0;
     sh.lok[lane] = 0;
     sh.uhits[lane] = 0;
-    sh.ucap[lane] = 0;
+    if constexpr (!SHORT) sh.ucap[lane] = 0;
     if (head) {
         sh.unit_of[uslot] = t.unit;
-        sh.run_base[uslot] = (t.scan_start + carry) >> a.rec_shift;
+        if constexpr (!SHORT) sh.run_base[uslot] = (t.scan_start + carry) >> a.rec_shift;
         bool loc = false;
         if (!DUMP) {
             if (t.whole_unit()) {
@@ -179,7 +222,7 @@
         sh.tab[lane] = e;
     }
     __syncthreads();
-    if (!DUMP) {
+    if constexpr (!DUMP && !SHORT) {
         const uint32_t head_lane = 63u - (uint32_t)__clzll(head_mask & ((2ull << lane) - 1));
         const uint64_t first_win = (uint64_t)__shfl((long long)(t.scan_start + carry), head_lane, 64);
         const uint32_t slack = t.n_windows() < a.tile_windows ? l - 1 : 0u;
@@ -189,8 +232,28 @@
         __syncthreads();
     }
 
-    const uint32_t *packed = a.packed;
-    const int64_t s = (int64_t)t.scan_start;
+    auto PK = [&](int64_t i) -> uint32_t {
+        if constexpr (SHORT) return sh.stage_p[(uint32_t)i];
+        else return a.packed[i];
+    };
+    auto MK = [&](uint64_t i) -> uint32_t {
+        if constexpr (SHORT) return sh.stage_m[(uint32_t)i];
+        else return a.invmask[i];
+    };
+    const int64_t s = SHORT ? (int64_t)sl.s_local : (int64_t)t.scan_start;
+    auto run_cap = [&](uint32_t us, uint32_t us_windows) -> uint32_t {
+        if constexpr (SHORT) {
+            const uint64_t first_win = a.tiles[wave_first + us].scan_start;
+            return (uint32_t)(((first_win + us_windows + l - 1) >> a.rec_shift) - (first_win >> a.rec_shift));
+        } else {
+            return sh.ucap[us];
+        }
+    };
+    auto run_slot0 = [&](uint32_t us) -> uint64_t {
+        if constexpr (SHORT) return a.tiles[wave_first + us].scan_start >> a.rec_shift;
+        else return sh.run_base[us];
+    };
+    [[maybe_unused]] const uint64_t p_limit = SHORT ? (uint64_t)16 * DCN_STAGE_WORDS : a.stream_bases;
 
     uint32_t fw = 0, rc = 0, tg = 0;
     {
@@ -198,7 +261,7 @@
         const uint32_t sh_in = (uint32_t)(s & 15) * 2;
         uint32_t cur = 0;
         for (uint32_t tt = 0; tt + 1 < k; ++tt) {
-            if ((tt & 15) == 0) cur = __funnelshift_r(packed[q_in + (tt >> 4)], packed[q_in + (tt >> 4) + 1], sh_in);
+            if ((tt & 15) == 0) cur = __funnelshift_r(PK(q_in + (tt >> 4)), PK(q_in + (tt >> 4) + 1), sh_in);
             uint32_t c = (cur >> (2 * (tt & 15))) & 3;
             uint4 e = sh.tab[c];
             fw = rotl32(fw, VAR ? ROT : 1u) ^ e.x;
@@ -274,19 +337,17 @@
             it.o_uslot = o_pk & 0xFFu;
             it.p = (uint64_t)(o_s + it.rel);
 #ifdef DCN_DEBUG_BOUNDS
-            if (it.act && it.p + k > a.stream_bases) {
+            if (it.act && it.p + k > p_limit) {
                 a.status->bounds = 2;
                 it.act = false;
                 it.p = 0;
             }
 #endif
             if (it.act) {
-                const uint32_t *mp = a.invmask + (it.p >> 5);
-                const uint32_t *pp = packed + (it.p >> 4);
-#pragma unroll
-                for (int q = 0; q < NMW; ++q) it.mw[q] = mp[q];
-#pragma unroll
-                for (int q = 0; q < NPW; ++q) it.pw[q] = pp[q];
+#pragma unroll
+                for (int q = 0; q < NMW; ++q) it.mw[q] = MK((it.p >> 5) + q);
+#pragma unroll
+                for (int q = 0; q < NPW; ++q) it.pw[q] = PK((int64_t)(it.p >> 4) + q);
             }
         };
         Item cur, nxt;
@@ -346,7 +407,7 @@
                 o_uslot[u] = o_pk & 0xFFu;
                 p[u] = (uint64_t)(o_s + rel[u]);
 #ifdef DCN_DEBUG_BOUNDS
-                if (act[u] && p[u] + k > a.stream_bases) {
+                if (act[u] && p[u] + k > p_limit) {
                     a.status->bounds = 2;
                     act[u] = false;
                     p[u] = 0;
@@ -356,12 +417,10 @@
 #pragma unroll
             for (int u = 0; u < (PIPE ? 0 : U); ++u) {
                 if (act[u]) {
-                    const uint32_t *mp = a.invmask + (p[u] >> 5);
-                    const uint32_t *pp = packed + (p[u] >> 4);
-#pragma unroll
-                    for (int q = 0; q < NMW; ++q) mw[u][q] = (DCN_EXP & 16) ? 0u : mp[q];
-#pragma unroll
-                    for (int q = 0; q < NPW; ++q) pw[u][q] = pp[q];
+#pragma unroll
+                    for (int q = 0; q < NMW; ++q) mw[u][q] = (DCN_EXP & 16) ? 0u : MK((p[u] >> 5) + q);
+#pragma unroll
+                    for (int q = 0; q < NPW; ++q) pw[u][q] = PK((int64_t)(p[u] >> 4) + q);
                 }
             }
             bool valid[U];
@@ -513,10 +572,11 @@
                         const uint32_t head_lane = hm ? 63u - (uint32_t)__clzll(hm) : 0u;
                         const uint32_t rank = (uint32_t)__popcll(below) - (uint32_t)__popcll(rb & ((1ull << head_lane) - 1));
                         any_rec = true;
+                        const uint32_t o_windows = SHORT ? __shfl(nwc, lo[u], 64) : 0u;
                         if (rec) {
                             const uint32_t at = sh.uhits[o_uslot[u]] + rank;
-                            if (at < sh.ucap[o_uslot[u]]) {
-                                if (!(DCN_EXP & 512)) a.rec_hash[sh.run_base[o_uslot[u]] + at] = hash[u];
+                            if (at < run_cap(o_uslot[u], o_windows)) {
+                                if (!(DCN_EXP & 512)) a.rec_hash[run_slot0(o_uslot[u]) + at] = hash[u];
                             } else {
                                 a.status->run_overflow = 1;
                             }
@@ -566,9 +626,9 @@
     int64_t b_in = 2 * (s + (int64_t)(k - 1)), b_k = 2 * s, b_l = 2 * (s - (int64_t)(w - 1));
     int64_t wi_in = b_in >> 5, wi_k = b_k >> 5, wi_l = b_l >> 5;
     uint32_t so_in = (uint32_t)(b_in & 31), so_k = (uint32_t)(b_k & 31), so_l = (uint32_t)(b_l & 31);
-    uint32_t ra_in = packed[wi_in], rb_in = packed[wi_in + 1];
-    uint32_t ra_k = packed[wi_k], rb_k = packed[wi_k + 1];
-    uint32_t ra_l = packed[wi_l], rb_l = packed[wi_l + 1];
+    uint32_t ra_in = PK(wi_in), rb_in = PK(wi_in + 1);
+    uint32_t ra_k = PK(wi_k), rb_k = PK(wi_k + 1);
+    uint32_t ra_l = PK(wi_l), rb_l = PK(wi_l + 1);
     uint32_t w_in = __funnelshift_r(ra_in, rb_in, so_in);
     uint32_t w_k = __funnelshift_r(ra_k, rb_k, so_k);
     uint32_t w_l = __funnelshift_r(ra_l, rb_l, so_l);
@@ -580,12 +640,12 @@
             ra_in = rb_in ^ 0x5A5A5A5Au; rb_in = ra_k + 0x1234567u; ra_k = rb_l; rb_k = ra_l ^ ra_in; ra_l = rb_k; rb_l = rb_in;
             return;
         }
-        ra_in = packed[wi_in]; rb_in = packed[wi_in + 1];
+        ra_in = PK(wi_in); rb_in = PK(wi_in + 1);
         if (DCN_EXP & 64) {
             ra_k = ra_in; rb_k = rb_in; ra_l = ra_in; rb_l = rb_in;
         } else {
-            ra_k = packed[wi_k]; rb_k = packed[wi_k + 1];
-            ra_l = packed[wi_l]; rb_l = packed[wi_l + 1];
+            ra_k = PK(wi_k); rb_k = PK(wi_k + 1);
+            ra_l = PK(wi_l); rb_l = PK(wi_l + 1);
         }
     };
     advance_streams();
@@ -596,7 +656,7 @@
         } else {
             for (uint32_t b = 1; b < w; ++b) {
                 int64_t p = s - (int64_t)b;
-                tg += (packed[p >> 4] >> (2 * (uint32_t)(p & 15) + 1)) & 1u;
+                tg += (PK(p >> 4) >> (2 * (uint32_t)(p & 15) + 1)) & 1u;
             }
         }
     }
@@ -682,7 +742,7 @@
                 if (!FIRST || r == STEP - 1) {
                     const uint32_t sel = ((tg > lhalf) ? lmin : rmax) & 0xFFFFu;
                     const bool emit = FIRST ? (nwc > 0) : ((j - (w - 1) < nwc) && sel != prev);
-                    if (!(DCN_EXP & 4)) sh.DCN_LIST_AT(lane, cnt) = (uint16_t)sel;
+                    if (!(DCN_EXP & 4)) sh.DCN_LIST_AT(lane, cnt) = (std::remove_reference_t<decltype(sh.list[0][0])>)sel;
                     cnt += emit ? 1u : 0u;
                     prev = sel;
                 }
@@ -731,7 +791,7 @@
                 hash = 0;
                 if (actv) {
                     const uint32_t *mp = a.invmask + (p >> 5);
-                    const uint32_t *pp = packed + (p >> 4);
+                    const uint32_t *pp = a.packed + (p >> 4);
                     const uint32_t m0 = mp[0], m1 = mp[1], m2 = K128 ? mp[2] : 0u;
                     uint32_t pw[K128 ? 5 : 3];
 #pragma unroll
@@ -880,6 +940,115 @@
     }
 }
 
+template <int W>
+__device__ __forceinline__ void scan_short(const dcn_scan_args &a, WaveSharedShort &sh) {
+    const uint32_t NT = a.status->bad_offsets ? 0u : *a.n_tiles;
+    const uint32_t wave_first = blockIdx.x * DCN_WAVE;
+    if (wave_first >= NT) return;
+    const uint32_t n_have = min(NT - wave_first, (uint32_t)DCN_WAVE);
+    const uint32_t l = a.k + W - 1;
+    const uint64_t n_bases = a.stream_bases;
+    const uint64_t a16 = reinterpret_cast<uintptr_t>(a.ascii) & 15;
+    const uint8_t *abase = a.ascii - a16;
+
+    auto load_chunk = [&](int64_t c) -> uint4 {
+        const int64_t b0 = 16 * c - (int64_t)a16;
+        if (b0 >= 0 && (uint64_t)b0 + 16 <= n_bases) return *reinterpret_cast<const uint4 *>(abase + 16 * c);
+        uint32_t v[4] = {0, 0, 0, 0};
+        for (int j = 0; j < 16; ++j) {
+            const int64_t p = b0 + j;
+            const uint32_t byte = p < 0 ? 0u : ((uint64_t)p < n_bases ? (uint32_t)a.ascii[p] : (uint32_t)'A');
+            v[j >> 2] |= byte << (8 * (j & 3));
+        }
+        return make_uint4(v[0], v[1], v[2], v[3]);
+    };
+
+    constexpr int64_t GAP_CHUNKS = 2;
+    for (uint32_t lo = 0; lo < n_have;) {
+        int lane = threadIdx.x;
+        asm volatile("" : "+v"(lane));
+        const bool have = (uint32_t)lane < n_have;
+        const dcn_tile t = a.tiles[wave_first + (have ? (uint32_t)lane : n_have - 1)];
+        const uint64_t start = t.scan_start, end = start + t.n_windows() + l - 1;
+        uint32_t nw = t.n_windows();
+        if (have && nw && end <= n_bases && a.ascii[end - 1] == '\n') nw -= 1;
+        const int64_t cf = ((int64_t)(a16 + start) - (int64_t)(W - 1)) >> 4;
+        const int64_t cl = (int64_t)(a16 + end - 1) >> 4;
+        const int64_t cl_prev = __shfl_up((long long)cl, 1, 64);
+        const uint64_t start_prev = (uint64_t)__shfl_up((long long)start, 1, 64);
+        const bool in = (uint32_t)lane >= lo && have;
+        const bool newrun = (uint32_t)lane == lo || start < start_prev || cf > cl_prev + 1 + GAP_CHUNKS;
+        const int64_t cost64 = newrun ? cl - cf + 1 : cl - cl_prev;
+        const uint32_t cost = in ? (uint32_t)(cost64 > 0 ? cost64 : 0) : 0u;
+        const uint32_t incl = wave_inclusive_scan_u32(cost, lane);
+        const uint32_t hi = max((uint32_t)__popcll(__ballot(have && incl <= (uint32_t)DCN_STAGE_WORDS)), lo + 1);
+        const bool act = in && (uint32_t)lane < hi && incl <= (uint32_t)DCN_STAGE_WORDS;
+        const unsigned long long heads = __ballot(act && newrun);
+        const unsigned long long mine = heads & ((2ull << lane) - 1);
+        const uint32_t head_lane = mine ? 63u - (uint32_t)__clzll(mine) : lo;
+        const uint32_t excl = incl - cost;
+        const uint32_t wb_h = __shfl(excl, head_lane, 64);
+        const int64_t cf_h = __shfl((long long)cf, head_lane, 64);
+        const uint32_t total_words = __shfl(incl, hi - 1, 64);
+        __syncthreads();
+        for (unsigned long long rest = heads; rest;) {
+            const int h = __ffsll((long long)rest) - 1;
+            rest &= rest - 1;
+            const uint32_t wb = __shfl(excl, h, 64);
+            const int64_t c0 = __shfl((long long)cf, h, 64);
+            const uint32_t we = rest ? __shfl(excl, __ffsll((long long)rest) - 1, 64) : total_words;
+            for (uint32_t i0 = 0; i0 < we - wb; i0 += 4 * DCN_WAVE) {
+                uint4 v[4];
+#pragma unroll
+                for (int q = 0; q < 4; ++q) {
+                    const uint32_t i = i0 + q * DCN_WAVE + lane;
+                    v[q] = make_uint4(0, 0, 0, 0);
+                    if (i < we - wb) v[q] = load_chunk(c0 + i);
+                }
+#pragma unroll
+                for (int q = 0; q < 4; ++q) {
+                    const uint32_t i = i0 + q * DCN_WAVE + lane;
+                    if (i < we - wb && wb + i < (uint32_t)DCN_STAGE_WORDS) {
+                        sh.stage_p[wb + i] = dcn_pack4(v[q].x) | (dcn_pack4(v[q].y) << 8) | (dcn_pack4(v[q].z) << 16) | (dcn_pack4(v[q].w) << 24);
+                        sh.stage_m16[wb + i] = (uint16_t)(dcn_invalid4(v[q].x) | (dcn_invalid4(v[q].y) << 4) | (dcn_invalid4(v[q].z) << 8) |
+                                                          (dcn_invalid4(v[q].w) << 12));
+                    }
+                }
+            }
+        }
+        ShortLane sl;
+        sl.lane = lane;
+        sl.have = act;
+        sl.t = t;
+        sl.t.nwf = act ? ((t.nwf & 0xC0000000u) | nw) : 0u;
+        sl.s_local = act ? (uint32_t)((int64_t)(a16 + start) - 16 * cf_h + 16 * (int64_t)wb_h) : 16u;
+        __syncthreads();
+        scan_body<W, false, false, false, false, true>(a, sh, sl);
+        lo = hi;
+    }
+}
+
+#ifndef DCN_SHORT_FUSED
+#define DCN_SHORT_FUSED 1
+#endif
+template <int W>
+constexpr bool dcn_scan_has_short = DCN_SHORT_FUSED && DCN_LIST_BY_LANE && !DCN_EXPORT_UNIFORM && W == 15;
+
+template <int W, bool K128, bool DUMP, bool FAST, bool VAR = false, bool SHORTK = false>
+__global__ __launch_bounds__(DCN_WAVE, FAST ? DCN_MIN_WAVES_FAST : DCN_MIN_WAVES) void scan_kernel(dcn_scan_args a) {
+    if constexpr (SHORTK) {
+        static_assert(dcn_scan_has_short<W> && !K128 && !DUMP && !FAST && !VAR, "the short path is a counting kernel of fixed w, k <= 32");
+        __shared__ WaveSharedShort sh;
+        if (a.status->short_batch) scan_short<W>(a, sh);
+    } else {
+        __shared__ WaveShared sh;
+        if constexpr (dcn_scan_has_short<W> && !K128 && !DUMP && !FAST && !VAR) {
+            if (a.ascii && a.status->short_batch) return;
+        }
+        scan_body<W, K128, DUMP, FAST, VAR, false>(a, sh, ShortLane{});
+    }
+}
+
 template <int W, bool VAR = false>
 int launch_w(const dcn_scan_args &args, uint32_t blocks, bool dump, bool k128, size_t dyn, hipStream_t stream) {
 #define DCN_LAUNCH(K128_, DUMP_, FAST_)                                                               \
@@ -893,6 +1062,10 @@
         hipLaunchKernelGGL(kern, dim3(blocks), dim3(DCN_WAVE), dyn, stream, args);                    \
     } while (0)
     const bool fast = !dump && args.early_out_max_items != 0;
+    if constexpr (dcn_scan_has_short<W> && !VAR) {
+        if (args.ascii && !k128 && !dump && !fast)
+            hipLaunchKernelGGL((scan_kernel<W, false, false, false, false, true>), dim3(blocks), dim3(DCN_WAVE), 0, stream, args);
+    }
     if (k128) {
         if (dump) DCN_LAUNCH(true, true, false);
         else if (fast) DCN_LAUNCH(true, false, true);
@@ -930,6 +1103,9 @@
     if (combine) *combine = v & 0xFF;
     return DCN_OK;
 }
+
+bool dcn_scan_has_short_path(uint32_t k, uint32_t w) { return k <= 32 && w == 15 && dcn_scan_has_short<15>; }
+uint32_t dcn_short_lmax() { return DCN_SHORT_LMAX; }
 
 int dcn_launch_scan(const dcn_scan_args &args_in, uint32_t max_tiles, bool dump, hipStream_t stream) {
     if (max_tiles == 0) return DCN_OK;
diff --git a/deacon-server_amd/filter.py b/deacon-server_amd/filter.py
--- a/deacon-server_amd/filter.py
+++ b/deacon-server_amd/filter.py
@@ -762,6 +762,11 @@
         N.check(N.lib().dcn_filter_batch_device(self._h, d_bases, d_offsets, d_unit_id, n_reads, n_bases, n_units,
                                                 C.byref(p), d_keep, d_hits, d_total))
 
+    def last_batch_short(self):
+        v = C.c_uint32()
+        N.check(N.lib().dcn_ctx_last_batch_short(self._h, C.byref(v)))
+        return bool(v.value)
+
     def reserve_records(self, n_records):
         N.check(N.lib().dcn_ctx_reserve_records(self._h, int(n_records)))
 
diff --git a/include/deacon_hip.h b/include/deacon_hip.h
--- a/include/deacon_hip.h
+++ b/include/deacon_hip.h
@@ -39,7 +39,7 @@
 };
 
 #define DCN_ABI_MAJOR 1
-#define DCN_ABI_MINOR 11
+#define DCN_ABI_MINOR 12
 int dcn_abi_version(uint32_t *major, uint32_t *minor);
 const char *dcn_version(void);
 const char *dcn_last_error(void);
@@ -113,6 +113,8 @@
                             const dcn_params *params, uint8_t *d_keep, uint32_t *d_hits, uint32_t *d_total);
 
 int dcn_ctx_synchronize(dcn_ctx *ctx);
+
+int dcn_ctx_last_batch_short(dcn_ctx *ctx, uint32_t *was_short);
 
 int dcn_ctx_reserve_records(dcn_ctx *ctx, uint64_t n_records);
 
```

After: 435,200, median of 6. +8.4%, better.
